# mmetcalf14/qml-cutensornet

Measured on AMD Instinct MI355X. Metric: Gram kernel entries/sec @ 60 qubits x 6 layers, higher is better.
Workload: dtype f64 (complex128)

## Files before the change

lab/qk_quad.h:

```cpp
#pragma once

__device__ __forceinline__ int qkq_qinv(const int d) {
  static constexpr int T[17] = {0, 1048576, 524288, 349526, 262144, 209716, 174763, 149797, 131072, 116509, 104858, 95326, 87382, 80660, 74899, 69906, 65536};
  return T[d];
}

struct QkqUnit {
  bool mine, a1, b1;
  int ta, tb, p;
};

template <bool A1, bool B1, typename XPtr>
__device__ __forceinline__ void qkq_p1(QkfTile (&T)[2][2], v2d (&fr)[4], v2d (&fs)[4], const bool primed, QkfStream cur, XPtr xp, unsigned x0, unsigned x1, const int nks,
                                       const QkfStream n0, const unsigned n1off) {
  v4d P[2][2][3];
  v2d fx[4], fy[4];
  if (!primed) qkf_load4(fr, cur);
  if (B1) {
#pragma unroll
    for (int i = 0; i < 4; ++i) fs[i] = qkf_ldg(cur.base + i * cur.step, cur.off + TILE);
  }
#pragma unroll
  for (int i = 0; i < 4; ++i) {
    fx[i] = qkf_ldx(xp + i * QKF_XSTEP, x0);
// ... 93 lines not shown
        p1 = __builtin_amdgcn_mfma_f64_16x16x4f64(S[1][0][i], fs[i].x, p1, 0, 0, 0);
        p2 = __builtin_amdgcn_mfma_f64_16x16x4f64(T[1][0].re[i], sp, p2, 0, 0, 0);
        p3 = __builtin_amdgcn_mfma_f64_16x16x4f64(T[1][0].im[i], sm, p3, 0, 0, 0);
        if (B1) {
          r1 = __builtin_amdgcn_mfma_f64_16x16x4f64(S[1][1][i], fs[i].x, r1, 0, 0, 0);
          r2 = __builtin_amdgcn_mfma_f64_16x16x4f64(T[1][1].re[i], sp, r2, 0, 0, 0);
          r3 = __builtin_amdgcn_mfma_f64_16x16x4f64(T[1][1].im[i], sm, r3, 0, 0, 0);
        }
      }
      if (!LAST) fs[i] = qkf_ldg(i == 0 ? b0 : i == 1 ? b1 : i == 2 ? b2 : b3, o1);
      __builtin_amdgcn_sched_barrier(0);
    }
  }
  QKF_PRIO_HI();
  {
    const v4d re = p1 - p3, im = p1 - p2;
#pragma unroll
    for (int r = 0; r < 4; ++r) {
      __hip_atomic_fetch_add(d + r * rs, re[r], __ATOMIC_RELAXED, __HIP_MEMORY_SCOPE_WORKGROUP);
      __hip_atomic_fetch_add(d + r * rs + 1, im[r], __ATOMIC_RELAXED, __HIP_MEMORY_SCOPE_WORKGROUP);
    }
  }
  if (B1) {
    const v4d re = r1 - r3, im = r1 - r2;
#pragma unroll
    for (int r = 0; r < 4; ++r) {
      __hip_atomic_fetch_add(d1 + r * rs, re[r], __ATOMIC_RELAXED, __HIP_MEMORY_SCOPE_WORKGROUP);
      __hip_atomic_fetch_add(d1 + r * rs + 1, im[r], __ATOMIC_RELAXED, __HIP_MEMORY_SCOPE_WORKGROUP);
    }
  }
}

template <bool FULL, bool A1, bool B1>
__device__ __forceinline__ void qkq_p2(const QkfTile (&T)[2][2], v2d (&fr)[4], v2d (&fs)[4], const QkfStream cur, const unsigned a1off, const int ps, const int nn, const int kmax, lds_v2d* xo,
                                       const int q, const int j, const QkfStream nxt) {
  lds_double* d = (lds_double*)(xo + q * TILE + j);
  lds_double* d1 = d + 2 * QKF_XBLOCK;
  constexpr long rs = 2 * QKF_XSTEP;
  v4d S[2][2];
#pragma unroll
  for (int u = 0; u < 2; ++u)
#pragma unroll
    for (int v = 0; v < 2; ++v) S[u][v] = ((u == 0 || A1) && (v == 0 || B1)) ? T[u][v].re + T[u][v].im : (v4d){0, 0, 0, 0};
  const v2d *const c0 = cur.base, *const c1 = cur.base + cur.step, *const c2 = cur.base + 2 * cur.step, *const c3 = cur.base + 3 * cur.step;
  unsigned o0 = cur.off, o1 = cur.off + a1off;
#pragma unroll 1
  for (int tn = 0; tn + 1 < nn; ++tn) {
    o0 += TILE, o1 += TILE;
    qkq_p2_block<FULL, A1, B1, false>(T, S, fr, fs, kmax, c0, c1, c2, c3, o0, o1, d, d1, rs);
    d += 2 * ps, d1 += 2 * ps;
  }
  qkq_p2_block<FULL, A1, B1, true>(T, S, fr, fs, kmax, nxt.base, nxt.base + nxt.step, nxt.base + 2 * nxt.step, nxt.base + 3 * nxt.step, nxt.off, 0u, d, d1, rs);
}

template <int NW, int XCAP, int WPS>
__global__ __launch_bounds__(64 * NW, WPS) void qk_sweep_fused_quad_kernel(const SweepArgs g) {
  constexpr int NT = 64 * NW;
  extern __shared__ __attribute__((aligned(16))) double lds_raw[];
  lds_v2d* const XL = (lds_v2d*)lds_raw;
  long long* const slot = reinterpret_cast<long long*>(lds_raw + 2 * XCAP);
  const v2d* const xdata = reinterpret_cast<const v2d*>(g.xdata);
  const v2d* const ydata = reinterpret_cast<const v2d*>(g.ydata);
  v2d* const G0 = reinterpret_cast<v2d*>(g.scratch) + (long long)blockIdx.x * 2 * g.x_plane;
  const int tid = threadIdx.x, lane = tid & 63;
  const int wave = __builtin_amdgcn_readfirstlane(tid >> 6);
  const int j = lane & 15, q = lane >> 4;
  const int ns = g.n_sites;
  __attribute__((address_space(3))) double* const zacc = (__attribute__((address_space(3))) double*)(slot + 2);
  lds_v4i* const rec = (lds_v4i*)(slot + 2 + 32);
  long long* const m_off = reinterpret_cast<long long*>(slot + 2 + 32) + 6 * (long long)ns;
  auto rfl = [&](const int v) __attribute__((always_inline)) { return __builtin_amdgcn_readfirstlane(v); };
  auto ldl = [&](const long long* p_) __attribute__((always_inline)) {
    const long long v = *p_;
    const unsigned lo = __builtin_amdgcn_readfirstlane((unsigned)v);
    const unsigned hi = __builtin_amdgcn_readfirstlane((unsigned)((unsigned long long)v >> 32));
    return (long long)(((unsigned long long)hi << 32) | lo);
  };
  auto site = [&](const int k) __attribute__((always_inline)) {
    const v4i r0 = rec[3 * k], r1 = rec[3 * k + 1], r2 = rec[3 * k + 2];
    QkfSite s;
    s.a = rfl(r0.x), s.a2 = rfl(r0.y), s.b = rfl(r0.z), s.b2 = rfl(r0.w);
    s.at = rfl(r1.x), s.nks = rfl(r1.y), s.W = rfl(r1.z), s.small = rfl(r1.w) != 0;
    s.inv = rfl(r2.x);
    s.ps = rfl(r2.y), s.pd = 1 << s.ps, s.next = rfl(r2.z);
    s.mt = s.a / TILE, s.nt = s.b2 / TILE, s.nn = s.a2 / TILE;
    s.Ak = xdata + ldl(m_off + 2 * k);
    s.Bk = ydata + ldl(m_off + 2 * k + 1);
    return s;
  };
  struct Pieces {
    int qa_f, qb_f, ra, rb, nA, kq, n2a, nB, nC, nD, L, qinv;
  };
  auto pieces_of = [&](const QkfSite& s, const int w) __attribute__((always_inline)) {
    Pieces pc;
    pc.qa_f = s.mt >> 1, pc.qb_f = w >> 1, pc.ra = s.mt & 1, pc.rb = w & 1;
    pc.nA = s.pd * pc.qa_f * pc.qb_f;
#if defined(QKF_QUAD_MODE) && QKF_QUAD_MODE == 0
    pc.kq = 0;
#else
    pc.kq = pc.nA - pc.nA % NW;
#endif
    pc.n2a = 2 * (pc.nA - pc.kq);
    pc.nB = s.pd * pc.ra * pc.qb_f, pc.nC = s.pd * pc.qa_f * pc.rb, pc.nD = s.pd * pc.ra * pc.rb;
    pc.L = pc.kq + pc.n2a + pc.nB + pc.nC + pc.nD;
    pc.qinv = qkq_qinv(pc.qa_f);
    return pc;
  };
  auto unit_of = [&](const QkfSite& s, const int w, const Pieces& pc, const int r0) __attribute__((always_inline)) {
    QkqUnit un;
    const int left = pc.L - r0;
    const bool cut = 2 * left <= NW;
    const int sub = cut && wave >= left ? 1 : 0;
    int i = r0 + wave - sub * left;
    un.mine = cut ? wave < 2 * left : i < pc.L;
    un.a1 = un.b1 = false, un.ta = un.tb = un.p = 0;
    auto quad = [&](const int vq) __attribute__((always_inline)) {
      const int u = vq >> s.ps, qb = (u * pc.qinv) >> 20, qa = u - qb * pc.qa_f;
      un.p = vq & (s.pd - 1), un.ta = 2 * qa, un.tb = 2 * qb;
    };
    if (i < pc.kq) {
      quad(i), un.a1 = un.b1 = true;
    } else if ((i -= pc.kq) < pc.n2a) {
      quad(pc.kq + (i >> 1)), un.ta += i & 1, un.b1 = true;
    } else if ((i -= pc.n2a) < pc.nB) {
      un.p = i & (s.pd - 1), un.ta = s.mt - 1, un.tb = 2 * (i >> s.ps), un.b1 = true;
    } else if ((i -= pc.nB) < pc.nC) {
      un.p = i & (s.pd - 1), un.ta = 2 * (i >> s.ps), un.tb = w - 1, un.a1 = true;
    } else {
      i -= pc.nC;
      un.p = i & (s.pd - 1), un.ta = s.mt - 1, un.tb = w - 1;
    }
    if (cut) {
      if (un.b1) un.tb += sub, un.b1 = false;
      else if (un.a1) un.ta += sub, un.a1 = false;
      else un.mine = un.mine && sub == 0;
    }
    return un;
  };
  auto b_stream = [&](const QkfSite& s, const int s0, const QkqUnit& un) __attribute__((always_inline)) {
    return QkfStream{s.Bk + un.p * s.b2, (unsigned)((q * s.pd) * s.b2 + (s0 + un.tb) * TILE + j), 4 * s.pd * s.b2};
  };
  auto a_stream = [&](const QkfSite& s, const QkqUnit& un) __attribute__((always_inline)) {
    return QkfStream{s.Ak + un.p * s.a2, (unsigned)(((un.ta * TILE + q) * s.pd) * s.a2 + j), 4 * s.pd * s.a2};
  };
  const int xcc = qk_xcc_id();
  if (tid == 0) qk_tail_start(g);
  for (;;) {
    if (tid == 0) *slot = qk_pull(g, xcc);
    __syncthreads();
    const long long p = *slot;
    __syncthreads();
    if (p < 0) break;
    const int xi = g.pairs[2 * p], yj = g.pairs[2 * p + 1];
    qkf_step_table<XCAP, NT>(g, xi, yj, rec, m_off, tid, [](const int pmt, const int nt) { return pmt * ((nt + 1) / 2) <= NW; });
    const int ek = g.edge_k, k_hi = ns - ek;
    const bool edges = ek > 0;
    if (!edges)
      for (int e = tid; e < TILE * TILE; e += NT) XL[e] = (v2d){e == 0 ? 1.0 : 0.0, 0.0};
    __syncthreads();
    bool xg = false;
    int cur = 0, xb = 0;
    if (edges) {
      const v4i r0 = rec[3 * ek];
      const int a_e = rfl(r0.x), b_e = rfl(r0.z);
      xg = a_e * b_e > XCAP;
      qkf_edge_prefix<NW, QKF_EDGE_PAIRS(WPS), QKF_EDGE_SETS(WPS)>(g, xi, yj, a_e, b_e, XL, G0, xg, wave, q, j);
      __syncthreads();
    }
    v2d fr[4], fs[4];
    bool primed = false;
    QkfSite sn = site(ek);
    for (int k = ek; k < k_hi;) {
      const QkfSite sc = sn;
      k = sc.next;
      if (k < k_hi) sn = site(k);
      const int a = sc.a, a2 = sc.a2, b = sc.b, nt = sc.nt, W = sc.W;
      const bool small = sc.small;
      v2d* const Gc = G0 + (long long)cur * g.x_plane;
      v2d* const Gn = G0 + (long long)(cur ^ 1) * g.x_plane;
      if (small && xg) {
        for (int e = tid; e < a * b; e += NT) XL[e] = Gc[e];
        __syncthreads();
        xg = false, xb = 0;
      } else if (!small && !xg) {
        for (int e = tid; e < a * b; e += NT) Gc[e] = XL[xb + e];
        __syncthreads();
        xg = true;
      }
      const int n_out = sc.b2 * a2;
      const bool pingpong = small && a * b + n_out <= XCAP;
      const int ob = !small ? 0 : pingpong ? (xb == 0 ? XCAP - n_out : 0) : 0;
      if (pingpong)
        for (int e = tid; e < n_out; e += NT) XL[ob + e] = (v2d){0.0, 0.0};
      for (int s0 = 0; s0 < nt; s0 += W) {
        const int w = min(W, nt - s0);
        const Pieces pc = pieces_of(sc, w);
        const int quads = pc.L;
        if (!small) {
          for (int e = tid; e < w * TILE * a2; e += NT) XL[e] = (v2d){0.0, 0.0};
          qk_lds_barrier();
        }
        for (int r0 = 0; r0 < quads; r0 += NW) {
          const QkqUnit un = unit_of(sc, w, pc, r0);
          const QkfStream as = a_stream(sc, un);
          const unsigned a1off = (unsigned)(TILE * sc.pd * a2);
          auto between = [&]() __attribute__((always_inline)) {
            if (small && r0 == 0) {
              qk_lds_barrier();
              if (!pingpong) {
                for (int e = tid; e < n_out; e += NT) XL[e] = (v2d){0.0, 0.0};
                qk_lds_barrier();
              }
            }
          };
          if (un.mine) {
            QkfTile T[2][2];
            const QkfStream bs = b_stream(sc, s0, un);
            const unsigned x0 = (unsigned)(un.ta * (b * TILE) + q * TILE + j), x1 = x0 + (unsigned)(b * TILE);
            auto go = [&](auto xbase) __attribute__((always_inline)) {
              if (un.a1) {
                if (un.b1) qkq_p1<true, true>(T, fr, fs, primed, bs, xbase, x0, x1, sc.nks, as, as.off + a1off);
                else qkq_p1<true, false>(T, fr, fs, primed, bs, xbase, x0, x1, sc.nks, as, as.off + a1off);
              } else {
                if (un.b1) qkq_p1<false, true>(T, fr, fs, primed, bs, xbase, x0, x1, sc.nks, as, as.off + a1off);
                else qkq_p1<false, false>(T, fr, fs, primed, bs, xbase, x0, x1, sc.nks, as, as.off + a1off);
              }
            };
            if (xg) go((const v2d*)Gc);
            else go((const lds_v2d*)(XL + xb));
            between();
            const int kmax = min(4, (sc.at - (un.ta + (un.a1 ? 1 : 0)) * TILE + 3) >> 2);
            QkfStream nxt = as;
            bool np1 = false;
            if (r0 + NW < quads) {
              const QkqUnit nu = unit_of(sc, w, pc, r0 + NW);
              if (nu.mine) nxt = b_stream(sc, s0, nu), np1 = true;
            } else if (s0 + W < nt) {
              const int w2 = min(W, nt - s0 - W);
              const QkqUnit nu = unit_of(sc, w2, pieces_of(sc, w2), 0);
              if (nu.mine) nxt = b_stream(sc, s0 + W, nu), np1 = true;
            } else if (k < k_hi) {
              const int w2 = min(sn.W, sn.nt);
              const QkqUnit nu = unit_of(sn, w2, pieces_of(sn, w2), 0);
              if (nu.mine) nxt = b_stream(sn, 0, nu), np1 = true;
            }
            lds_v2d* const xo = XL + ob + un.tb * QKF_XBLOCK;
            const int ps = w * QKF_XBLOCK;
            auto p2 = [&](auto a1_, auto b1_) __attribute__((always_inline)) {
              constexpr bool A1_ = decltype(a1_)::value, B1_ = decltype(b1_)::value;
              if (kmax == 4) qkq_p2<true, A1_, B1_>(T, fr, fs, as, a1off, ps, sc.nn, 4, xo, q, j, nxt);
              else qkq_p2<false, A1_, B1_>(T, fr, fs, as, a1off, ps, sc.nn, kmax, xo, q, j, nxt);
            };
            if (un.a1) {
              if (un.b1) p2(std::true_type{}, std::true_type{});
              else p2(std::true_type{}, std::false_type{});
            } else {
              if (un.b1) p2(std::false_type{}, std::true_type{});
              else p2(std::false_type{}, std::false_type{});
            }
            primed = np1;
          } else {
            between();
          }
        }
        qk_lds_barrier();
        if (!small && nt > W) {
          for (int tn = 0; tn < sc.nn; ++tn)
            for (int e = tid; e < w * QKF_XBLOCK; e += NT) Gn[(long long)tn * (sc.b2 * TILE) + s0 * QKF_XBLOCK + e] = XL[tn * w * QKF_XBLOCK + e];
          __syncthreads();
        }
      }
      if (!small) {
        if (nt > W) cur ^= 1;
        else xg = false, xb = 0;
      } else {
        xb = ob;
      }
    }
    if (edges) {
      const v4i r0 = rec[3 * (k_hi - 1)];
      const int a_e = rfl(r0.y), b_e = rfl(r0.w);
      qkf_edge_suffix<NW, QKF_EDGE_PAIRS(WPS), QKF_EDGE_SETS(WPS)>(g, xi, yj, a_e, b_e, (const lds_v2d*)(XL + xb), (const v2d*)(G0 + (long long)cur * g.x_plane), xg, zacc, wave, q, j);
      __syncthreads();
    }
    if (tid == 0) {
      v2d zz = {0.0, 0.0};
      if (edges)
        for (int w_ = 0; w_ < NW; ++w_) zz.x += zacc[2 * w_], zz.y += zacc[2 * w_ + 1];
      else zz = xg ? G0[(long long)cur * g.x_plane] : (v2d)XL[xb];
      g.values[p] = zz.x * zz.x + zz.y * zz.y;
      if (g.z) {
        g.z[2 * p] = zz.x;
        g.z[2 * p + 1] = zz.y;
      }
    }
    __syncthreads();
  }
  if (tid == 0) qk_tail_exit(g);
}
```

qml-cutensornet_amd/csrc/qk_device.h:

```cpp
#pragma once
#include <hip/hip_runtime.h>

#include <cstdint>
#include <type_traits>

static constexpr int TILE = 16;
typedef double v4d __attribute__((ext_vector_type(4)));
typedef float v4f __attribute__((ext_vector_type(4)));

struct SweepArgs {
  const double* xdata;
  const int32_t* xdims;
  const int32_t* xtrue;
  const int64_t* xoffs;
  const double* ydata;
  const int32_t* ydims;
  const int32_t* ytrue;
  const int64_t* yoffs;
  int n_sites;
  const int32_t* pairs;
  long long npairs;
  const int32_t* groups;
  long long ngroups;
  double* values;
  double* z;
  double* scratch;
  long long x_plane;
  long long t_plane;
  unsigned long long* counter;
  int nq;
  long long qstart[17];
  const double* xedge;
  const long long* xedge_offs;
  const double* yedge;
  const long long* yedge_offs;
  int edge_k;
  const double* xmg;
  const double* ymg;
  const int64_t* xmg_offs;
  const int64_t* ymg_offs;
  int merge_steps;
  int turn_ints;
  unsigned long long* tail;
  unsigned long long* err;
  unsigned long long* prof;
  unsigned long long* gang;
  int gang_n;
  int debug_flags;
  int prio_mode;
};

static constexpr int QK_QSTRIDE = 16;
static constexpr int QK_NQ_MAX = 16;

__device__ __forceinline__ int qk_xcc_id() { return __builtin_amdgcn_s_getreg((3 << 11) | 20) & 7; }

__device__ __forceinline__ long long qk_pull(const SweepArgs& g, const int xcc) {
  if (g.nq <= 1) {
    const long long p = (long long)atomicAdd(g.counter, 1ull);
    return p < g.npairs ? p : -1;
  }
  for (int s = 0; s < g.nq; ++s) {
    const int qd = ((xcc + s) & 7) + (s & 8);
    const long long n = g.qstart[qd + 1] - g.qstart[qd];
    if (n <= 0) continue;
    const long long t = (long long)atomicAdd(g.counter + QK_QSTRIDE * qd, 1ull);
    if (t < n) return g.qstart[qd] + t;
  }
  return -1;
}

__device__ __forceinline__ void qk_gang_sync(const SweepArgs& g, const int xcc, const bool have_pair, int& round) {
  if (g.gang_n <= 1) return;
  unsigned long long* const a = g.gang + QK_QSTRIDE * xcc;
  if (!have_pair) {
    __hip_atomic_store(a + 1, 1ull, __ATOMIC_RELAXED, __HIP_MEMORY_SCOPE_AGENT);
    return;
  }
  const unsigned long long target = (unsigned long long)g.gang_n * (unsigned long long)(++round);
  __hip_atomic_fetch_add(a, 1ull, __ATOMIC_RELAXED, __HIP_MEMORY_SCOPE_AGENT);
  for (int spins = 0;; ++spins) {
    if (__hip_atomic_load(a, __ATOMIC_RELAXED, __HIP_MEMORY_SCOPE_AGENT) >= target) return;
    if (__hip_atomic_load(a + 1, __ATOMIC_RELAXED, __HIP_MEMORY_SCOPE_AGENT) != 0) return;
    if (spins > 4000) {
      __hip_atomic_store(a + 1, 1ull, __ATOMIC_RELAXED, __HIP_MEMORY_SCOPE_AGENT);
      return;
    }
    __builtin_amdgcn_s_sleep(8);
  }
}

__device__ __forceinline__ void qk_tail_start(const SweepArgs& g) {
  if (g.tail) atomicMin(g.tail, (unsigned long long)__builtin_amdgcn_s_memrealtime());
}
__device__ __forceinline__ void qk_tail_exit(const SweepArgs& g) {
  if (g.tail) {
    const unsigned long long t = __builtin_amdgcn_s_memrealtime();
    atomicMin(g.tail + 1, t);
    atomicMax(g.tail + 4, t);
  }
}

__device__ __forceinline__ void qk_lds_barrier() { asm volatile("s_waitcnt lgkmcnt(0)\n\ts_barrier" ::: "memory"); }
```

qml-cutensornet_amd/csrc/qk_fused.h:

```cpp
#pragma once
#include "qk_device.h"
#include "qk_plan.h"

#define QKF_PRIO_LO() __builtin_amdgcn_s_setprio(0)
#define QKF_PRIO_HI() __builtin_amdgcn_s_setprio(2)
typedef double v2d __attribute__((ext_vector_type(2)));
typedef __attribute__((address_space(3))) v2d lds_v2d;
static constexpr int QKF_XSTEP = 4 * TILE;
static constexpr int QKF_XBLOCK = TILE * TILE;


#ifndef QKF_LDS3M
#define QKF_LDS3M 0
#endif
#ifndef QKF_P2_PROBE
#define QKF_P2_PROBE 0
#endif
#ifndef QKF_ABL
#define QKF_ABL 0
#endif
#define QKF_STEP_BARRIER()                            \
  do {                                                \
    if (QKF_ABL & 4) asm volatile("s_waitcnt lgkmcnt(0)" ::: "memory"); \
    else qk_lds_barrier();                            \
// ... 258 lines not shown
#else
#define QKF_EDGE_SETS(WPS) ((WPS) <= 3 ? 2 : 1)
#endif
__device__ __forceinline__ v2d qkf_lde(const v2d* __restrict__ base, const unsigned boff, const int col = 0) {
  return reinterpret_cast<const v2d*>(reinterpret_cast<const char*>(base) + (size_t)boff)[col];
}
template <bool HAS1, bool MORE>
__device__ __forceinline__ void qkf_edge_group(v4d (&acc)[6], v2d (&fy)[4], v2d (&fz)[4], v2d (&fx)[4], const v2d* const* const by, const v2d* const* const bx, const unsigned boy,
                                               const unsigned box) {
#pragma unroll
  for (int i = 0; i < 4; ++i) {
    const double sb = QKF_DIF(fx[i].x, fx[i].y);
    acc[0] = __builtin_amdgcn_mfma_f64_16x16x4f64(fy[i].x, fx[i].x, acc[0], 0, 0, 0);
    acc[1] = __builtin_amdgcn_mfma_f64_16x16x4f64(fy[i].y, fx[i].y, acc[1], 0, 0, 0);
    acc[2] = __builtin_amdgcn_mfma_f64_16x16x4f64(QKF_SUM(fy[i].x, fy[i].y), sb, acc[2], 0, 0, 0);
    if (HAS1) {
      acc[3] = __builtin_amdgcn_mfma_f64_16x16x4f64(fz[i].x, fx[i].x, acc[3], 0, 0, 0);
      acc[4] = __builtin_amdgcn_mfma_f64_16x16x4f64(fz[i].y, fx[i].y, acc[4], 0, 0, 0);
      acc[5] = __builtin_amdgcn_mfma_f64_16x16x4f64(QKF_SUM(fz[i].x, fz[i].y), sb, acc[5], 0, 0, 0);
    }
    if (MORE) {
      fy[i] = qkf_lde(by[i], boy);
      if (HAS1) fz[i] = qkf_lde(by[i], boy, TILE);
      fx[i] = qkf_lde(bx[i], box);
    }
    __builtin_amdgcn_sched_barrier(0);
  }
}
template <bool HAS1, int SETS>
__device__ __forceinline__ void qkf_edge_unit(QkfTile& t0, QkfTile& t1, const v2d* __restrict__ Ay, const unsigned oy, const int ldy, const v2d* __restrict__ Ax, const unsigned ox, const int ldx,
                                              const int ng) {
  static_assert(SETS == 1 || SETS == 2, "one or two groups of k-steps in flight");
  v4d acc[6];
#pragma unroll
  for (int e = 0; e < 6; ++e) acc[e] = (v4d){0, 0, 0, 0};
  v2d fy[SETS][4], fz[SETS][4], fx[SETS][4];
  const v2d *by[4 * SETS], *bx[4 * SETS];
#pragma unroll
  for (int i = 0; i < 4 * SETS; ++i) by[i] = Ay + 4 * i * ldy, bx[i] = Ax + 4 * i * ldx;
  unsigned boy = oy * 16u, box = ox * 16u;
  const unsigned sy = (unsigned)(SETS * TILE * ldy) * 16u, sx = (unsigned)(SETS * TILE * ldx) * 16u;
  const bool two = SETS == 2 && ng > 1;
#pragma unroll
  for (int s = 0; s < SETS; ++s) {
    if (s == 0 || two) {
#pragma unroll
      for (int i = 0; i < 4; ++i) {
        fy[s][i] = qkf_lde(by[4 * s + i], boy);
        if (HAS1) fz[s][i] = qkf_lde(by[4 * s + i], boy, TILE);
        fx[s][i] = qkf_lde(bx[4 * s + i], box);
      }
    }
  }
  QKF_PRIO_LO();
#pragma unroll 1
  for (int g = SETS; g < ng; g += SETS) {
    boy += sy, box += sx;
#pragma unroll
    for (int s = 0; s < SETS; ++s) qkf_edge_group<HAS1, true>(acc, fy[s], fz[s], fx[s], by + 4 * s, bx + 4 * s, boy, box);
  }
  qkf_edge_group<HAS1, false>(acc, fy[0], fz[0], fx[0], by, bx, boy, box);
  if constexpr (SETS == 2) {
    if (two) qkf_edge_group<HAS1, false>(acc, fy[1], fz[1], fx[1], by + 4, bx + 4, boy, box);
  }
  QKF_PRIO_HI();
  t0.re = acc[0] + acc[1], t0.im = acc[2] - acc[0] + acc[1];
  if (HAS1) t1.re = acc[3] + acc[4], t1.im = acc[5] - acc[3] + acc[4];
}
__device__ __forceinline__ long long qkf_uniform(const long long v) {
  const unsigned lo = __builtin_amdgcn_readfirstlane((unsigned)v);
  const unsigned hi = __builtin_amdgcn_readfirstlane((unsigned)((unsigned long long)v >> 32));
  return (long long)(((unsigned long long)hi << 32) | lo);
}

template <int NW, bool PAIRS>
__device__ __forceinline__ QkEdgeUnit qkf_edge_unit_of(const int u, const int mt, const int nt, const int inv) {
  if constexpr (PAIRS) return qk_edge_unit(u, mt, nt, NW, inv);
  const int tb = (u * inv) >> 20;
  return QkEdgeUnit{u - tb * mt, tb, false, true};
}
template <int NW, bool PAIRS, int SETS>
__device__ __forceinline__ void qkf_edge_prefix(const SweepArgs& g, const int xi, const int yj, const int a, const int b, lds_v2d* const xl, v2d* const xg, const bool to_global, const int wave,
                                                const int q, const int j) {
  const v2d* const Lx = reinterpret_cast<const v2d*>(g.xedge) + qkf_uniform(g.xedge_offs[2 * (long long)xi]);
  const v2d* const Ly = reinterpret_cast<const v2d*>(g.yedge) + qkf_uniform(g.yedge_offs[2 * (long long)yj]);
  const int mt = a / TILE, nt = b / TILE, ng = (1 << g.edge_k) >> 4, inv = qk_recip20(mt), units = PAIRS ? qk_edge_units(mt, nt, NW) : mt * nt;
  for (int u = wave; u < units; u += NW) {
    const QkEdgeUnit un = qkf_edge_unit_of<NW, PAIRS>(u, mt, nt, inv);
    if (!un.mine) continue;
    QkfTile T0, T1;
    const unsigned oy = (unsigned)(q * b + un.tb0 * TILE + j), ox = (unsigned)(q * a + un.ta * TILE + j);
    if (un.has1) qkf_edge_unit<true, 1>(T0, T1, Ly, oy, b, Lx, ox, a, ng);
    else qkf_edge_unit<false, SETS>(T0, T1, Ly, oy, b, Lx, ox, a, ng);
    const int at = un.ta * (b * TILE) + (un.tb0 * TILE + q) * TILE + j;
    if (to_global) {
#pragma unroll
      for (int r = 0; r < 4; ++r) xg[at + r * QKF_XSTEP] = (v2d){T0.re[r], T0.im[r]};
      if (un.has1) {
#pragma unroll
        for (int r = 0; r < 4; ++r) xg[at + QKF_XBLOCK + r * QKF_XSTEP] = (v2d){T1.re[r], T1.im[r]};
      }
    } else {
#pragma unroll
      for (int r = 0; r < 4; ++r) xl[at + r * QKF_XSTEP] = (v2d){T0.re[r], T0.im[r]};
      if (un.has1) {
#pragma unroll
        for (int r = 0; r < 4; ++r) xl[at + QKF_XBLOCK + r * QKF_XSTEP] = (v2d){T1.re[r], T1.im[r]};
      }
    }
  }
}

template <int NW, bool PAIRS, int SETS>
__device__ __forceinline__ void qkf_edge_suffix(const SweepArgs& g, const int xi, const int yj, const int a, const int b, const lds_v2d* const xl, const v2d* const xg, const bool from_global,
                                                __attribute__((address_space(3))) double* zacc, const int wave, const int q, const int j) {
  const v2d* const Rx = reinterpret_cast<const v2d*>(g.xedge) + qkf_uniform(g.xedge_offs[2 * (long long)xi + 1]);
  const v2d* const Ry = reinterpret_cast<const v2d*>(g.yedge) + qkf_uniform(g.yedge_offs[2 * (long long)yj + 1]);
  const int mt = a / TILE, nt = b / TILE, ng = (1 << g.edge_k) >> 4, inv = qk_recip20(mt), units = PAIRS ? qk_edge_units(mt, nt, NW) : mt * nt;
  double zr = 0, zi = 0;
  for (int u = wave; u < units; u += NW) {
    const QkEdgeUnit un = qkf_edge_unit_of<NW, PAIRS>(u, mt, nt, inv);
    if (!un.mine) continue;
    QkfTile T0, T1;
    const unsigned oy = (unsigned)(q * b + un.tb0 * TILE + j), ox = (unsigned)(q * a + un.ta * TILE + j);
    if (un.has1) qkf_edge_unit<true, 1>(T0, T1, Ry, oy, b, Rx, ox, a, ng);
    else qkf_edge_unit<false, SETS>(T0, T1, Ry, oy, b, Rx, ox, a, ng);
    const int at = un.ta * (b * TILE) + (un.tb0 * TILE + q) * TILE + j;
#pragma unroll
    for (int r = 0; r < 4; ++r) {
      const v2d x = from_global ? xg[at + r * QKF_XSTEP] : (v2d)xl[at + r * QKF_XSTEP];
      zr += x.x * T0.re[r] - x.y * T0.im[r], zi += x.x * T0.im[r] + x.y * T0.re[r];
    }
    if (un.has1) {
#pragma unroll
      for (int r = 0; r < 4; ++r) {
        const v2d x = from_global ? xg[at + QKF_XBLOCK + r * QKF_XSTEP] : (v2d)xl[at + QKF_XBLOCK + r * QKF_XSTEP];
        zr += x.x * T1.re[r] - x.y * T1.im[r], zi += x.x * T1.im[r] + x.y * T1.re[r];
      }
    }
  }
#pragma unroll
  for (int o = 32; o > 0; o >>= 1) zr += __shfl_xor(zr, o), zi += __shfl_xor(zi, o);
  if ((q | j) == 0) zacc[2 * wave] = zr, zacc[2 * wave + 1] = zi;
}

struct QkfSite {
  int a, a2, b, b2, at, nks, mt, nt, nn, W, inv, inv2, pd, ps, next;
  bool small;
  const v2d *Ak, *Bk;
};
typedef int v4i __attribute__((ext_vector_type(4)));
typedef __attribute__((address_space(3))) v4i lds_v4i;

template <int XCAP, int NT, bool ITEM_RECIPS = false, typename OneRound>
__device__ __forceinline__ void qkf_step_table(const SweepArgs& g, const int xi, const int yj, lds_v4i* const rec, long long* const m_off, const int tid, const OneRound one_round) {
  const int ns = g.n_sites, n1 = ns + 1;
  const int32_t* const xd = g.xdims + (long long)xi * n1;
  const int32_t* const yd = g.ydims + (long long)yj * n1;
  const int32_t* const xt = g.xtrue + (long long)xi * n1;
  const int32_t* const yt = g.ytrue + (long long)yj * n1;
  const v2d* const xdata = reinterpret_cast<const v2d*>(g.xdata);
  const v2d* const ydata = reinterpret_cast<const v2d*>(g.ydata);
  auto is_small = [&](const int a, const int a2, const int b, const int b2, const int pd) __attribute__((always_inline)) {
    return a * b <= XCAP && a2 * b2 <= XCAP && (one_round(pd * (a / TILE), b2 / TILE) || a * b + a2 * b2 <= XCAP);
  };
  auto put = [&](const int e, const int a, const int a2, const int b, const int b2, const int ps, const int next, const bool small, const v2d* const A, const v2d* const B)
                 __attribute__((always_inline)) {
    const int mt = a / TILE, nt = b2 / TILE;
    const int W = small ? nt : max(1, min(nt, XCAP / (TILE * a2)));
    rec[3 * e] = (v4i){a, a2, b, b2};
    rec[3 * e + 1] = (v4i){xt[e], (yt[e] + 3) >> 2, W, small ? 1 : 0};
    rec[3 * e + 2] = (v4i){qk_recip20(mt), ps, next, ITEM_RECIPS ? qk_unit_recips(nt, W, false) : 0};
    m_off[2 * e] = (long long)(((const char*)A - (const char*)xdata) / 16);
    m_off[2 * e + 1] = (long long)(((const char*)B - (const char*)ydata) / 16);
  };
  auto plain = [&](const int e, const int next) __attribute__((always_inline)) {
    const int a = xd[e], a2 = xd[e + 1], b = yd[e], b2 = yd[e + 1];
    put(e, a, a2, b, b2, 1, next, is_small(a, a2, b, b2, 2), xdata + (g.xoffs[(long long)xi * ns + e] >> 1), ydata + (g.yoffs[(long long)yj * ns + e] >> 1));
  };
  if (g.merge_steps == 0) {
    for (int e = tid; e < ns; e += NT) plain(e, e + 1);
    return;
  }
  const int ek = g.edge_k, k_hi = ns - ek;
  for (int t = tid; 2 * t < k_hi - ek; t += NT) {
    const int e = ek + 2 * t;
    if (e + 1 >= k_hi) {
      plain(e, e + 1);
      continue;
    }
    const int a = xd[e], am = xd[e + 1], a2 = xd[e + 2], b = yd[e], bm = yd[e + 1], b2 = yd[e + 2];
    const bool sm = is_small(a, a2, b, b2, 4);
    const long long work_m = 4ll * a * b2 * (b + a2), work_p = 2ll * a * bm * (b + am) + 2ll * am * b2 * (bm + a2);
    const bool merged = (sm || (!is_small(a, am, b, bm, 2) && !is_small(am, a2, bm, b2, 2))) && work_m <= work_p;
    plain(e + 1, e + 2);
    if (merged)
      put(e, a, a2, b, b2, 2, e + 2, sm, reinterpret_cast<const v2d*>(g.xmg) + (g.xmg_offs[(long long)xi * g.merge_steps + t] >> 1),
          reinterpret_cast<const v2d*>(g.ymg) + (g.ymg_offs[(long long)yj * g.merge_steps + t] >> 1));
    else plain(e, e + 1);
  }
}

#ifdef QKF_PROF
#define QKF_PROF_DECL() \
  unsigned long long pf[8] = {0, 0, 0, 0, 0, 0, 0, 0}, pt = __builtin_amdgcn_s_memtime(); \
  const unsigned long long pt0 = pt
#define QKF_STAMP(i)                                              \
  do {                                                            \
    const unsigned long long now_ = __builtin_amdgcn_s_memtime(); \
    pf[i] += now_ - pt;                                           \
    pt = now_;                                                    \
  } while (0)
#define QKF_PROF_FLUSH()                                             \
  do {                                                               \
    if (lane == 0) {                                                 \
      pf[7] = __builtin_amdgcn_s_memtime() - pt0;                    \
      for (int i_ = 0; i_ < 8; ++i_) atomicAdd(g.prof + i_, pf[i_]); \
    }                                                                \
  } while (0)
#else
#define QKF_PROF_DECL()
#define QKF_STAMP(i)
#define QKF_PROF_FLUSH()
#endif

#define QKF_PULLER(NT) ((NT) - 64)
__device__ __forceinline__ void qkf_pull_next(const SweepArgs& g, const int xcc, int& gang_round, long long* const word) {
  const long long pp = qk_pull(g, xcc);
  qk_gang_sync(g, xcc, pp >= 0, gang_round);
  *word = pp;
}

template <int NW, int S, int XCAP, int WPS, bool DET = false>
__global__ __launch_bounds__(64 * NW, WPS) void qk_sweep_fused_kernel(const SweepArgs g) {
  constexpr int NT = 64 * NW;
  extern __shared__ __attribute__((aligned(16))) double lds_raw[];
  lds_v2d* const XL = (lds_v2d*)lds_raw;
  long long* const slot = reinterpret_cast<long long*>(lds_raw + 2 * XCAP);
  const v2d* const xdata = reinterpret_cast<const v2d*>(g.xdata);
  const v2d* const ydata = reinterpret_cast<const v2d*>(g.ydata);
  v2d* const G0 = reinterpret_cast<v2d*>(g.scratch) + (long long)blockIdx.x * 2 * g.x_plane;
  const int tid = threadIdx.x, lane = tid & 63;
  const int wave = __builtin_amdgcn_readfirstlane(tid >> 6);
  const int j = lane & 15, q = lane >> 4;
  const int ns = g.n_sites;
  __attribute__((address_space(3))) double* const zacc = (__attribute__((address_space(3))) double*)(slot + 2);
  lds_v4i* const rec = (lds_v4i*)(slot + 2 + 32);
  long long* const m_off = reinterpret_cast<long long*>(slot + 2 + 32) + 6 * (long long)ns;
  lds_int* const tbroken = (lds_int*)(m_off + 2 * (long long)ns);
  lds_int* const turn0 = tbroken + 2;
  auto rfl = [&](const int v) __attribute__((always_inline)) { return __builtin_amdgcn_readfirstlane(v); };
  auto ldl = [&](const long long* p_) __attribute__((always_inline)) {
    const long long v = *p_;
    const unsigned lo = __builtin_amdgcn_readfirstlane((unsigned)v);
    const unsigned hi = __builtin_amdgcn_readfirstlane((unsigned)((unsigned long long)v >> 32));
    return (long long)(((unsigned long long)hi << 32) | lo);
  };
  auto site = [&](const int k) __attribute__((always_inline)) {
    const v4i r0 = rec[3 * k], r1 = rec[3 * k + 1], r2 = rec[3 * k + 2];
    QkfSite s;
    s.a = rfl(r0.x), s.a2 = rfl(r0.y), s.b = rfl(r0.z), s.b2 = rfl(r0.w);
    s.at = rfl(r1.x), s.nks = rfl(r1.y), s.W = rfl(r1.z), s.small = rfl(r1.w) != 0;
    s.inv = rfl(r2.x), s.inv2 = rfl(r2.w);
    s.ps = rfl(r2.y), s.pd = 1 << s.ps, s.next = rfl(r2.z);
    s.mt = s.a / TILE, s.nt = s.b2 / TILE, s.nn = s.a2 / TILE;
    s.Ak = xdata + ldl(m_off + 2 * k);
    s.Bk = ydata + ldl(m_off + 2 * k + 1);
    return s;
  };
  auto item_of = [&](const QkfSite& s, const int w, const int it) __attribute__((always_inline)) {
    return DET ? qk_unit_decode_ordered(it, s.ps, s.mt, s.inv) : qk_unit_decode(it, s.mt, w, s.inv, qk_unit_recip_of(s.inv2, w == s.W));
  };
  auto b_stream = [&](const QkfSite& s, const int s0, const int w, const int it) __attribute__((always_inline)) {
    const QkUnit un = item_of(s, w, it);
    return QkfStream{s.Bk + un.p * s.b2, (unsigned)((q * s.pd) * s.b2 + (s0 + un.tc) * TILE + j), 4 * s.pd * s.b2, min(4, s.nks)};
  };
  auto a_stream = [&](const QkfSite& s, const int w, const int it) __attribute__((always_inline)) {
    const QkUnit un = item_of(s, w, it);
    return QkfStream{s.Ak + un.p * s.a2, (unsigned)(((un.ta * TILE + q) * s.pd) * s.a2 + j), 4 * s.pd * s.a2, min(4, (s.at - un.ta * TILE + 3) >> 2)};
  };
  QKF_PROF_DECL();
  const int xcc = qk_xcc_id();
  int gang_round = 0;
  if (tid == 0) qk_tail_start(g);
  for (;;) {
    if (tid == 0) {
      const long long pp_ = qk_pull(g, xcc);
      qk_gang_sync(g, xcc, pp_ >= 0, gang_round);
      *slot = pp_;
    }
    __syncthreads();
    const long long p = *slot;
    __syncthreads();
    if (p < 0) break;
    const int xi = g.pairs[2 * p], yj = g.pairs[2 * p + 1];
    qkf_step_table<XCAP, NT, true>(g, xi, yj, rec, m_off, tid, [](const int pmt, const int nt) { return pmt * nt <= NW * S; });
    const int ek = g.edge_k, k_hi = ns - ek;
    const bool edges = ek > 0;
    if (!edges)
      for (int e = tid; e < TILE * TILE; e += NT) XL[e] = (v2d){e == 0 ? 1.0 : 0.0, 0.0};
    if constexpr (DET)
      for (int e = tid; e < 2 * g.turn_ints + 2; e += NT) tbroken[e] = 0;
    int tsel = 0;
    __syncthreads();
    bool xg = false;
    int cur = 0, xb = 0;
    if (edges) {
      const v4i r0 = rec[3 * ek];
      const int a_e = rfl(r0.x), b_e = rfl(r0.z);
      xg = a_e * b_e > XCAP;
      qkf_edge_prefix<NW, QKF_EDGE_PAIRS(WPS), QKF_EDGE_SETS(WPS)>(g, xi, yj, a_e, b_e, XL, G0, xg, wave, q, j);
      __syncthreads();
    }
    QKF_STAMP(0);
    QkfTile T[S];
    v2d fr[4];
    bool primed = false;
    QkfSite sn = site(ek);
    for (int k = ek; k < k_hi;) {
      const QkfSite sc = sn;
      k = sc.next;
      if (k < k_hi) sn = site(k);
      const int a = sc.a, a2 = sc.a2, b = sc.b, mt = sc.mt, nt = sc.nt, W = sc.W;
      const bool small = sc.small;
      v2d* const Gc = G0 + (long long)cur * g.x_plane;
      v2d* const Gn = G0 + (long long)(cur ^ 1) * g.x_plane;
      if (small && xg) {
        for (int e = tid; e < a * b; e += NT) XL[e] = Gc[e];
        __syncthreads();
        xg = false, xb = 0;
      } else if (!small && !xg) {
        for (int e = tid; e < a * b; e += NT) Gc[e] = XL[xb + e];
        __syncthreads();
        xg = true;
      }
      const int n_out = sc.b2 * a2;
      const bool pingpong = small && a * b + n_out <= XCAP;
      const int ob = !small ? 0 : pingpong ? (xb == 0 ? XCAP - n_out : 0) : 0;
      if (pingpong && !DET)
        for (int e = tid; e < n_out; e += NT) XL[ob + e] = (v2d){0.0, 0.0};
      QKF_STAMP(1);
      for (int s0 = 0; s0 < nt; s0 += W) {
        const int w = min(W, nt - s0), items = sc.pd * mt * w;
        lds_int* const tcur = turn0 + tsel * g.turn_ints;
        if constexpr (DET) {
          for (int e = tid; e < g.turn_ints; e += NT) turn0[(tsel ^ 1) * g.turn_ints + e] = 0;
        } else if (!small) {
          for (int e = tid; e < w * TILE * a2; e += NT) XL[e] = (v2d){0.0, 0.0};
          QKF_STEP_BARRIER();
        }
        QKF_STAMP(6);
        for (int r0 = 0; r0 < items; r0 += NW * S) {
          const int L = min(S, (items - r0 + NW - 1) / NW);
          const bool multi = L > 1;
          const int it0 = r0 + wave;
          auto phase1 = [&](auto xbase) __attribute__((always_inline)) {
#pragma unroll 1
            for (int s = 0; s < L; ++s) {
              if (multi) qkf_rotate<S>(T, L);
              const int it = it0 + NW * s;
              if (it < items) {
                const int ta = item_of(sc, w, it).ta;
                const bool more = s + 1 < L && it + NW < items;
                const QkfStream nxt = more ? b_stream(sc, s0, w, it + NW) : a_stream(sc, w, it0);
                qkf_p1_tile(T[S - 1], fr, primed, b_stream(sc, s0, w, it), xbase, (unsigned)(ta * (b * TILE) + q * TILE + j), sc.nks, nxt);
                primed = true;
              }
            }
          };
          if (xg) phase1((const v2d*)Gc);
          else phase1((const lds_v2d*)(XL + xb));
          QKF_STAMP(2);
          if (small && r0 == 0 && !(DET && pingpong)) {
            QKF_STEP_BARRIER();
            if (!pingpong && !DET) {
              for (int e = tid; e < n_out; e += NT) XL[e] = (v2d){0.0, 0.0};
              QKF_STEP_BARRIER();
            }
          }
          QKF_STAMP(3);
          const bool last_round = s0 + W >= nt && r0 + NW * S >= items;
#pragma unroll 1
          for (int s = 0; s < S; ++s) {
            const int it = it0 + NW * s;
            if (it >= items) break;
            if (multi) qkf_rotate<S>(T, L);
            const QkUnit un = item_of(sc, w, it);
            const int ta = un.ta, tbl = un.tc;
            const int kmax = min(4, (sc.at - ta * TILE + 3) >> 2);
            const bool more = s + 1 < S && it + NW < items;
            const int wn = min(sn.W, sn.nt);
            const bool chain = !more && last_round && k < k_hi && wave < sn.pd * sn.mt * wn;
            const QkfStream nxt = more ? a_stream(sc, w, it + NW) : chain ? b_stream(sn, 0, wn, wave) : a_stream(sc, w, it);
            const int tix = sc.pd * ta + un.p;
            const QkfTurn turn{tcur + tbl * sc.nn, tix, tbroken, g.err};
            if (kmax == 4) qkf_p2_item<true, DET>(T[S - 1], fr, primed, a_stream(sc, w, it), w * QKF_XBLOCK, sc.nn, 4, XL + ob + tbl * QKF_XBLOCK, q, j, nxt, turn);
            else qkf_p2_item<false, DET>(T[S - 1], fr, primed, a_stream(sc, w, it), w * QKF_XBLOCK, sc.nn, kmax, XL + ob + tbl * QKF_XBLOCK, q, j, nxt, turn);
            primed = more || chain;
          }
          QKF_STAMP(4);
        }
        QKF_STEP_BARRIER();
        tsel ^= 1;
        QKF_STAMP(5);
        if (!small && nt > W) {
          for (int tn = 0; tn < sc.nn; ++tn)
            for (int e = tid; e < w * QKF_XBLOCK; e += NT) Gn[(long long)tn * (sc.b2 * TILE) + s0 * QKF_XBLOCK + e] = XL[tn * w * QKF_XBLOCK + e];
          __syncthreads();
          QKF_STAMP(1);
        }
      }
      if (!small) {
        if (nt > W) cur ^= 1;
        else xg = false, xb = 0;
      } else {
        xb = ob;
      }
    }
    if (edges) {
      const v4i r0 = rec[3 * (k_hi - 1)];
      const int a_e = rfl(r0.y), b_e = rfl(r0.w);
      qkf_edge_suffix<NW, QKF_EDGE_PAIRS(WPS), QKF_EDGE_SETS(WPS)>(g, xi, yj, a_e, b_e, (const lds_v2d*)(XL + xb), (const v2d*)(G0 + (long long)cur * g.x_plane), xg, zacc, wave, q, j);
      __syncthreads();
    }
    if (tid == 0) {
      v2d zz = {0.0, 0.0};
      if (edges)
        for (int w_ = 0; w_ < NW; ++w_) zz.x += zacc[2 * w_], zz.y += zacc[2 * w_ + 1];
      else zz = xg ? G0[(long long)cur * g.x_plane] : (v2d)XL[xb];
      g.values[p] = zz.x * zz.x + zz.y * zz.y;
      if (g.z) {
        g.z[2 * p] = zz.x;
        g.z[2 * p + 1] = zz.y;
      }
    }
    __syncthreads();
  }
  if (tid == 0) qk_tail_exit(g);
  QKF_PROF_FLUSH();
}

template <bool HAS1, typename XPtr>
__device__ __forceinline__ void qkf_p1_dual(QkfTile& t0, QkfTile& t1, v2d (&fr)[4], v2d (&fs)[4], const bool primed, QkfStream cur, XPtr xp, unsigned xoff, const int nks,
                                            const QkfStream nxt) {
  v4d p1 = {0, 0, 0, 0}, p2 = {0, 0, 0, 0}, p3 = {0, 0, 0, 0}, r1 = {0, 0, 0, 0}, r2 = {0, 0, 0, 0}, r3 = {0, 0, 0, 0};
  v2d fx[4];
  if (!primed) qkf_load4(fr, cur);
  if (HAS1) {
#pragma unroll
// ... 95 lines not shown
  }
  if (HAS1) {
#pragma unroll
    for (int r = 0; r < 4; ++r) {
      __hip_atomic_fetch_add(d1 + r * rs, re1[r], __ATOMIC_RELAXED, __HIP_MEMORY_SCOPE_WORKGROUP);
      __hip_atomic_fetch_add(d1 + r * rs + 1, im1[r], __ATOMIC_RELAXED, __HIP_MEMORY_SCOPE_WORKGROUP);
    }
  }
}
template <bool FULL, bool HAS1, bool DET>
__device__ __forceinline__ void qkf_p2_dual_turn(const QkfTile& t0, const QkfTile& t1, v2d (&fr)[4], v2d (&fs)[4], QkfStream cur, const int ps, const int nn, const int kmax, lds_v2d* xo, const int q,
                                            const int j, const QkfStream nxt, const bool nxt_p1, const unsigned n1, const QkfTurn turn = QkfTurn{nullptr, 0, nullptr, nullptr}) {
  __attribute__((address_space(3))) double* d = (__attribute__((address_space(3))) double*)(xo + q * TILE + j);
#pragma unroll 1
  for (int tn = 0; tn < nn; ++tn) {
    v4d p1 = {0, 0, 0, 0}, p2 = {0, 0, 0, 0}, p3 = {0, 0, 0, 0}, r1 = {0, 0, 0, 0}, r2 = {0, 0, 0, 0}, r3 = {0, 0, 0, 0};
    const bool fin = tn + 1 == nn;
    const v2d* const rb = fin ? nxt.base : cur.base;
    const int rs = fin ? nxt.step : cur.step;
    cur.off = fin ? nxt.off : cur.off + TILE;
    QKF_PRIO_LO();
#pragma unroll
    for (int i = 0; i < 4; ++i) {
      if (FULL || i < kmax) {
        qkf_kstep<true>(p1, p2, p3, t0.re[i], t0.im[i], fr[i].x, fr[i].y);
        if (HAS1) qkf_kstep<true>(r1, r2, r3, t1.re[i], t1.im[i], fr[i].x, fr[i].y);
      }
      fr[i] = qkf_ldg_a(rb + i * rs, cur.off);
      __builtin_amdgcn_sched_barrier(0);
    }
    QKF_PRIO_HI();
    {
      const v4d re = p1 + p2, im = p3 - p1 + p2;
      if constexpr (DET) qkf_turn_add(d, (long)2 * QKF_XSTEP, re, im, turn, tn);
      else {
#pragma unroll
        for (int r = 0; r < 4; ++r) {
          __hip_atomic_fetch_add(d + r * 2 * QKF_XSTEP, re[r], __ATOMIC_RELAXED, __HIP_MEMORY_SCOPE_WORKGROUP);
          __hip_atomic_fetch_add(d + r * 2 * QKF_XSTEP + 1, im[r], __ATOMIC_RELAXED, __HIP_MEMORY_SCOPE_WORKGROUP);
        }
      }
    }
    if (HAS1) {
      const v4d re = r1 + r2, im = r3 - r1 + r2;
      __attribute__((address_space(3))) double* const d1 = d + 2 * QKF_XBLOCK;
      if constexpr (DET) qkf_turn_add(d1, (long)2 * QKF_XSTEP, re, im, QkfTurn{turn.at + nn, turn.idx, turn.broken, turn.gerr}, tn);
      else {
#pragma unroll
        for (int r = 0; r < 4; ++r) {
          __hip_atomic_fetch_add(d1 + r * 2 * QKF_XSTEP, re[r], __ATOMIC_RELAXED, __HIP_MEMORY_SCOPE_WORKGROUP);
          __hip_atomic_fetch_add(d1 + r * 2 * QKF_XSTEP + 1, im[r], __ATOMIC_RELAXED, __HIP_MEMORY_SCOPE_WORKGROUP);
        }
      }
    }
    d += 2 * ps;
  }
}

template <bool FULL, bool HAS1, bool DET = false>
__device__ __forceinline__ void qkf_p2_dual(const QkfTile& t0, const QkfTile& t1, v2d (&fr)[4], v2d (&fs)[4], QkfStream cur, const int ps, const int nn, const int kmax, lds_v2d* xo, const int q,
                                            const int j, const QkfStream nxt, const bool nxt_p1, const unsigned n1, const QkfTurn turn = QkfTurn{nullptr, 0, nullptr, nullptr}) {
  if constexpr (DET) {
    qkf_p2_dual_turn<FULL, HAS1, DET>(t0, t1, fr, fs, cur, ps, nn, kmax, xo, q, j, nxt, nxt_p1, n1, turn);
    return;
  }
  lds_double* d = (lds_double*)(xo + q * TILE + j);
  lds_double* d1 = d + 2 * QKF_XBLOCK;
  constexpr long rs = 2 * QKF_XSTEP;
  const v4d s0 = t0.re + t0.im, s1 = HAS1 ? t1.re + t1.im : s0;
  const v2d *const c0 = cur.base, *const c1 = cur.base + cur.step, *const c2 = cur.base + 2 * cur.step, *const c3 = cur.base + 3 * cur.step;
  unsigned off = cur.off;
#pragma unroll 1
  for (int tn = 0; tn + 1 < nn; ++tn) {
    off += TILE;
    qkf_p2_block<FULL, HAS1>(t0, t1, s0, s1, fr, kmax, c0, c1, c2, c3, off, d, d1, rs);
    d += 2 * ps, d1 += 2 * ps;
  }
  qkf_p2_block<FULL, HAS1>(t0, t1, s0, s1, fr, kmax, nxt.base, nxt.base + nxt.step, nxt.base + 2 * nxt.step, nxt.base + 3 * nxt.step, nxt.off, d, d1, rs);
}

template <int NW, int XCAP, int WPS, bool DET = false>
__global__ __launch_bounds__(64 * NW, WPS) void qk_sweep_fused_dual_kernel(const SweepArgs g) {
  constexpr int NT = 64 * NW;
  extern __shared__ __attribute__((aligned(16))) double lds_raw[];
  lds_v2d* const XL = (lds_v2d*)lds_raw;
  long long* const slot = reinterpret_cast<long long*>(lds_raw + 2 * XCAP);
  const v2d* const xdata = reinterpret_cast<const v2d*>(g.xdata);
  const v2d* const ydata = reinterpret_cast<const v2d*>(g.ydata);
  v2d* const G0 = reinterpret_cast<v2d*>(g.scratch) + (long long)blockIdx.x * 2 * g.x_plane;
  const int tid = threadIdx.x, lane = tid & 63;
  const int wave = __builtin_amdgcn_readfirstlane(tid >> 6);
  const int j = lane & 15, q = lane >> 4;
  const int ns = g.n_sites;
  __attribute__((address_space(3))) double* const zacc = (__attribute__((address_space(3))) double*)(slot + 2);
  lds_v4i* const rec = (lds_v4i*)(slot + 2 + 32);
  long long* const m_off = reinterpret_cast<long long*>(slot + 2 + 32) + 6 * (long long)ns;
  lds_int* const tbroken = (lds_int*)(m_off + 2 * (long long)ns);
  lds_int* const turn0 = tbroken + 2;
  auto rfl = [&](const int v) __attribute__((always_inline)) { return __builtin_amdgcn_readfirstlane(v); };
  auto ldl = [&](const long long* p_) __attribute__((always_inline)) {
    const long long v = *p_;
    const unsigned lo = __builtin_amdgcn_readfirstlane((unsigned)v);
    const unsigned hi = __builtin_amdgcn_readfirstlane((unsigned)((unsigned long long)v >> 32));
    return (long long)(((unsigned long long)hi << 32) | lo);
  };
  auto site = [&](const int k) __attribute__((always_inline)) {
    const v4i r0 = rec[3 * k], r1 = rec[3 * k + 1], r2 = rec[3 * k + 2];
    QkfSite s;
    s.a = rfl(r0.x), s.a2 = rfl(r0.y), s.b = rfl(r0.z), s.b2 = rfl(r0.w);
    s.at = rfl(r1.x), s.nks = rfl(r1.y), s.W = rfl(r1.z), s.small = rfl(r1.w) != 0;
    s.inv = rfl(r2.x);
    s.ps = rfl(r2.y), s.pd = 1 << s.ps, s.next = rfl(r2.z);
    s.mt = s.a / TILE, s.nt = s.b2 / TILE, s.nn = s.a2 / TILE;
    s.Ak = xdata + ldl(m_off + 2 * k);
    s.Bk = ydata + ldl(m_off + 2 * k + 1);
    return s;
  };
  auto pair_of = [&](const QkfSite& s, const int v) __attribute__((always_inline)) { return qk_unit_decode_ordered(v, s.ps, s.mt, s.inv); };
  auto b_stream = [&](const QkfSite& s, const int s0, const int v, const int half) __attribute__((always_inline)) {
    const QkUnit un = pair_of(s, v);
    return QkfStream{s.Bk + un.p * s.b2, (unsigned)((q * s.pd) * s.b2 + (s0 + 2 * un.tc + half) * TILE + j), 4 * s.pd * s.b2};
  };
  struct Unit {
    bool mine, has1;
    int v, half;
  };
  auto unit_of = [&](const QkfSite& s, const int w, const int units, const int r0) __attribute__((always_inline)) {
    Unit un;
    const int left = units - r0;
    const bool halves = 2 * left <= NW;
    un.half = (halves && wave >= left) ? 1 : 0;
    un.v = r0 + wave - (un.half ? left : 0);
    const int tp = pair_of(s, un.v).tc;
    const bool second = 2 * tp + 1 < w;
    un.mine = un.v < units && (un.half == 0 || second);
    un.has1 = !halves && second;
    return un;
  };
  auto a_stream = [&](const QkfSite& s, const int v) __attribute__((always_inline)) {
    const QkUnit un = pair_of(s, v);
    return QkfStream{s.Ak + un.p * s.a2, (unsigned)(((un.ta * TILE + q) * s.pd) * s.a2 + j), 4 * s.pd * s.a2};
  };
  QKF_PROF_DECL();
  const int xcc = qk_xcc_id();
  int gang_round = 0;
  if (tid == 0) qk_tail_start(g);
  if (tid == QKF_PULLER(NT)) qkf_pull_next(g, xcc, gang_round, slot);
  __syncthreads();
  long long p = slot[0];
  int psel = 0;
  auto table_of = [&](const long long pp) __attribute__((always_inline)) {
    if (pp < 0) return;
    const int xi_ = g.pairs[2 * pp], yj_ = g.pairs[2 * pp + 1];
    qkf_step_table<XCAP, NT>(g, xi_, yj_, rec, m_off, tid, [](const int pmt, const int nt) { return pmt * ((nt + 1) / 2) <= NW; });
  };
  table_of(p);
  while (p >= 0) {
    const int xi = g.pairs[2 * p], yj = g.pairs[2 * p + 1];
    const int ek = g.edge_k, k_hi = ns - ek;
    const bool edges = ek > 0;
    if (!edges)
      for (int e = tid; e < TILE * TILE; e += NT) XL[e] = (v2d){e == 0 ? 1.0 : 0.0, 0.0};
    if constexpr (DET)
      for (int e = tid; e < 2 * g.turn_ints + 2; e += NT) tbroken[e] = 0;
    int tsel = 0;
    __syncthreads();
    bool xg = false;
    int cur = 0, xb = 0;
    if (edges) {
      const v4i r0 = rec[3 * ek];
      const int a_e = rfl(r0.x), b_e = rfl(r0.z);
      xg = a_e * b_e > XCAP;
      qkf_edge_prefix<NW, QKF_EDGE_PAIRS(WPS), QKF_EDGE_SETS(WPS)>(g, xi, yj, a_e, b_e, XL, G0, xg, wave, q, j);
      __syncthreads();
    }
    QKF_STAMP(0);
    QkfTile T0, T1;
    v2d fr[4], fs[4];
    bool primed = false;
    QkfSite sn = site(ek);
    for (int k = ek; k < k_hi;) {
      const QkfSite sc = sn;
      k = sc.next;
      if (k < k_hi) sn = site(k);
      const int a = sc.a, a2 = sc.a2, b = sc.b, mt = sc.mt, nt = sc.nt, W = sc.W;
      const bool small = sc.small;
      v2d* const Gc = G0 + (long long)cur * g.x_plane;
      v2d* const Gn = G0 + (long long)(cur ^ 1) * g.x_plane;
      if (small && xg) {
        for (int e = tid; e < a * b; e += NT) XL[e] = Gc[e];
        __syncthreads();
        xg = false, xb = 0;
      } else if (!small && !xg) {
        for (int e = tid; e < a * b; e += NT) Gc[e] = XL[xb + e];
        __syncthreads();
        xg = true;
      }
      const int n_out = sc.b2 * a2;
      const bool pingpong = small && a * b + n_out <= XCAP;
      const int ob = !small ? 0 : pingpong ? (xb == 0 ? XCAP - n_out : 0) : 0;
      if (pingpong && !DET)
        for (int e = tid; e < n_out; e += NT) XL[ob + e] = (v2d){0.0, 0.0};
      QKF_STAMP(1);
      for (int s0 = 0; s0 < nt; s0 += W) {
        const int w = min(W, nt - s0), units = sc.pd * mt * ((w + 1) >> 1);
        lds_int* const tcur = turn0 + tsel * g.turn_ints;
        if constexpr (DET) {
          for (int e = tid; e < g.turn_ints; e += NT) turn0[(tsel ^ 1) * g.turn_ints + e] = 0;
        } else if (!small) {
          for (int e = tid; e < w * TILE * a2; e += NT) XL[e] = (v2d){0.0, 0.0};
          QKF_STEP_BARRIER();
        }
        for (int r0 = 0; r0 < units; r0 += NW) {
          const Unit un = unit_of(sc, w, units, r0);
          const int v = un.v;
          const bool mine = un.mine, has1 = un.has1;
          const QkUnit pr = pair_of(sc, v);
          const int tp = pr.tc, ta = pr.ta;
          if (mine) {
            const QkfStream bs = b_stream(sc, s0, v, un.half), as = a_stream(sc, v);
            const unsigned xoff = (unsigned)(ta * (b * TILE) + q * TILE + j);
            if (xg) {
              if (has1) qkf_p1_dual<true>(T0, T1, fr, fs, primed, bs, (const v2d*)Gc, xoff, sc.nks, as);
              else qkf_p1_dual<false>(T0, T1, fr, fs, primed, bs, (const v2d*)Gc, xoff, sc.nks, as);
            } else {
              if (has1) qkf_p1_dual<true>(T0, T1, fr, fs, primed, bs, (const lds_v2d*)(XL + xb), xoff, sc.nks, as);
              else qkf_p1_dual<false>(T0, T1, fr, fs, primed, bs, (const lds_v2d*)(XL + xb), xoff, sc.nks, as);
            }
          }
          QKF_STAMP(2);
          if (small && r0 == 0 && !(DET && pingpong)) {
            QKF_STEP_BARRIER();
            if (!pingpong && !DET) {
              for (int e = tid; e < n_out; e += NT) XL[e] = (v2d){0.0, 0.0};
              QKF_STEP_BARRIER();
            }
          }
          QKF_STAMP(3);
          if (mine) {
            const int kmax = min(4, (sc.at - ta * TILE + 3) >> 2);
            QkfStream nxt = a_stream(sc, v);
            bool np1 = false;
            if (r0 + NW < units) {
              const Unit nu = unit_of(sc, w, units, r0 + NW);
              if (nu.mine) nxt = b_stream(sc, s0, nu.v, nu.half), np1 = true;
            } else if (s0 + W < nt) {
              const int w2 = min(W, nt - s0 - W);
              const Unit nu = unit_of(sc, w2, sc.pd * mt * ((w2 + 1) >> 1), 0);
              if (nu.mine) nxt = b_stream(sc, s0 + W, nu.v, nu.half), np1 = true;
            } else if (k < k_hi) {
              const int w2 = min(sn.W, sn.nt);
              const Unit nu = unit_of(sn, w2, sn.pd * sn.mt * ((w2 + 1) >> 1), 0);
              if (nu.mine) nxt = b_stream(sn, 0, nu.v, nu.half), np1 = true;
            }
            const unsigned nd1 = 0;
            lds_v2d* const xo = XL + ob + (2 * tp + un.half) * QKF_XBLOCK;
            const QkfTurn tp_turn{tcur + (2 * tp + un.half) * sc.nn, sc.pd * ta + pr.p, tbroken, g.err};
            if (has1) {
              if (kmax == 4) qkf_p2_dual<true, true, DET>(T0, T1, fr, fs, a_stream(sc, v), w * QKF_XBLOCK, sc.nn, 4, xo, q, j, nxt, np1, nd1, tp_turn);
              else qkf_p2_dual<false, true, DET>(T0, T1, fr, fs, a_stream(sc, v), w * QKF_XBLOCK, sc.nn, kmax, xo, q, j, nxt, np1, nd1, tp_turn);
            } else {
              if (kmax == 4) qkf_p2_dual<true, false, DET>(T0, T1, fr, fs, a_stream(sc, v), w * QKF_XBLOCK, sc.nn, 4, xo, q, j, nxt, np1, nd1, tp_turn);
              else qkf_p2_dual<false, false, DET>(T0, T1, fr, fs, a_stream(sc, v), w * QKF_XBLOCK, sc.nn, kmax, xo, q, j, nxt, np1, nd1, tp_turn);
            }
            primed = np1;
          }
          QKF_STAMP(4);
        }
        QKF_STEP_BARRIER();
        tsel ^= 1;
        QKF_STAMP(5);
        if (!small && nt > W) {
          for (int tn = 0; tn < sc.nn; ++tn)
            for (int e = tid; e < w * QKF_XBLOCK; e += NT) Gn[(long long)tn * (sc.b2 * TILE) + s0 * QKF_XBLOCK + e] = XL[tn * w * QKF_XBLOCK + e];
          __syncthreads();
        }
      }
      if (!small) {
        if (nt > W) cur ^= 1;
        else xg = false, xb = 0;
      } else {
        xb = ob;
      }
    }
    if (tid == QKF_PULLER(NT)) qkf_pull_next(g, xcc, gang_round, slot + (psel ^ 1));
    if (edges) {
      const v4i r0 = rec[3 * (k_hi - 1)];
      const int a_e = rfl(r0.y), b_e = rfl(r0.w);
      qkf_edge_suffix<NW, QKF_EDGE_PAIRS(WPS), QKF_EDGE_SETS(WPS)>(g, xi, yj, a_e, b_e, (const lds_v2d*)(XL + xb), (const v2d*)(G0 + (long long)cur * g.x_plane), xg, zacc, wave, q, j);
    }
    __syncthreads();
    const long long pn = slot[psel ^ 1];
    if (tid == 0) {
      v2d zz = {0.0, 0.0};
      if (edges)
        for (int w_ = 0; w_ < NW; ++w_) zz.x += zacc[2 * w_], zz.y += zacc[2 * w_ + 1];
      else zz = xg ? G0[(long long)cur * g.x_plane] : (v2d)XL[xb];
      g.values[p] = zz.x * zz.x + zz.y * zz.y;
      if (g.z) {
        g.z[2 * p] = zz.x;
        g.z[2 * p + 1] = zz.y;
      }
    }
    table_of(pn);
    if (!edges) __syncthreads();
    p = pn, psel ^= 1;
    QKF_STAMP(6);
// ... 227 lines not shown
```

qml-cutensornet_amd/csrc/qk_host.h:

```cpp
#pragma once
#include "../../include/qkgram.h"
#include "qk_plan.h"

#include <hip/hip_runtime.h>

#include "qk_devmem.h"

#include <cstdint>
#include <vector>

struct QkRangeGuard {
  explicit QkRangeGuard(const char* n) { qk_range_push(n); }
  ~QkRangeGuard() { qk_range_pop(); }
};

#define HIP_TRY(expr)                                                                                 \
  do {                                                                                                \
    hipError_t e_ = (expr);                                                                           \
    if (e_ != hipSuccess) return qk_fail(QK_EDEVICE, "%s failed: %s", #expr, hipGetErrorString(e_));  \
  } while (0)
#define HIP_TRY_AS(what, expr)                              \
  do {                                                                                                          \
    hipError_t e_ = (expr);                                                                                     \
    if (e_ != hipSuccess) return qk_fail(QK_EDEVICE, "%s: %s failed: %s", what, #expr, hipGetErrorString(e_));  \
  } while (0)

struct qk_ctx {
  int device = 0;
  int num_cus = 0;
  hipStream_t own_stream = nullptr;
  hipStream_t stream = nullptr;
  bool split_pending = false;
  hipEvent_t ev0 = nullptr, ev1 = nullptr, ev_mid = nullptr;
  hipEvent_t ev_d = nullptr;
  bool ev_pending = false;
  QkGrowBuf scratch;
  QkDevBuf counter;
  bool tail_pending = false;
  QkDevBuf prof;
  QkSweepPolicy policy;
  qk_stats last{};
  QkGrowBuf build_arena, build_work;
  QkGrowBuf derive_tmp;
  QkGrowBuf local_scratch;
};

uint64_t qk_next_uid();

struct qk_mps_set {
  qk_ctx* ctx = nullptr;
  uint64_t uid = qk_next_uid();
  int n_states = 0, n_sites = 0, max_pad = 0;
  int precision = 64;
  QkDevBuf d_data;
  QkDevBuf d_il;
  QkDevBuf d_dims;
  QkDevBuf d_true;
  QkDevBuf d_offs;
  std::vector<int32_t> dims_true;
  int64_t bytes = 0;
  QkDevBuf d_edge;
  QkDevBuf d_edge_offs;
  int edge_k = 0;
  int64_t edge_bytes = 0;
  QkDevBuf d_mg;
  QkDevBuf d_mg_offs;
  QkDevBuf d_mg_units;
  std::vector<long long> h_edge_offs, h_mg_units;
  std::vector<int64_t> h_mg_offs;
  int mg_k = -1, mg_steps = 0;
  int64_t mg_bytes = 0;
};

int qk_mps_set_alloc(qk_ctx* c, int n_states, int n_sites, int64_t data_bytes, int precision, qk_mps_set** out, const char* who);

struct QkSpectraArgs {
  const double* env;
  const int32_t* dims;
  const int32_t* tru;
  const int32_t* states;
  const int32_t* pmax;
  const int64_t* sbase;
  const int64_t* roff;
  const int64_t* loff;
  const int2* tasks;
  int n_tasks;
  char* work;
  long long work_bytes;
  int qmax;
  double* out;
  int n_sites, max_values, rmul;
  int* error;
};
size_t qk_bond_spectra_work_bytes(int qmax);
int qk_bond_spectra_launch(qk_ctx* c, QkSpectraArgs a, int grid, const char* what);

struct QkCompressArgs {
  const double* planes;
  const int32_t* pad;
  const int32_t* tru;
  const int64_t* offs;
  int s0, n_batch, n_sites;
  double* stage;
  const long long* stage_offs;
  int32_t* dims_new;
  double* fidelity;
  double* discarded;
  int cap;
  double budget, zero;
  char* work;
  long long work_bytes;
  int qmax;
  int* error;
};
size_t qk_compress_work_bytes(int qmax);
int qk_compress_launch(qk_ctx* c, QkCompressArgs a, int grid, const char* what);

struct SweepArgs;
int qk_lab_init(qk_ctx* c);
int qk_lab_launch(qk_ctx* c, int variant, const SweepArgs& a, int grid, int n_sites);
int qk_lab_launch_quad(qk_ctx* c, const SweepArgs& a, int grid, int n_sites, bool f32);
```

qml-cutensornet_amd/csrc/qk_plan.h:

```cpp
#pragma once
#include "../../include/qkgram.h"

#include <algorithm>
#include <cstdint>
#include <cstdio>
#include <vector>

int qk_fail(int code, const char* fmt, ...) __attribute__((format(printf, 2, 3)));

#ifndef QKF_XCAP_ONE_V
#define QKF_XCAP_ONE_V 8192
#endif
#ifndef QKF_XCAP_TWO_V
#define QKF_XCAP_TWO_V 4608
#endif
#ifndef QKF_TWO_WGS
#define QKF_TWO_WGS 2
#endif
static constexpr int QKF_XCAP_ONE = QKF_XCAP_ONE_V, QKF_XCAP_TWO = QKF_XCAP_TWO_V;
static constexpr int QK_TILE = 16;
static inline int qk_pad16(int x) { return (x + QK_TILE - 1) / QK_TILE * QK_TILE; }
static constexpr int GMAX = 4;

#if defined(__HIPCC__)
#define QK_HD __host__ __device__
#else
#define QK_HD
#endif
struct QkUnit {
  int ta, tc, p;
};
QK_HD static inline int qk_unit_cols(const int w, const bool dual) { return dual ? (w + 1) >> 1 : w; }
QK_HD static inline int qk_recip20(const int d) { return ((1 << 20) + d - 1) / d; }
QK_HD static inline int qk_recip15(const int d) { return ((1 << 15) + d - 1) / d; }
QK_HD static inline int qk_unit_recips(const int nt, const int W, const bool dual) {
  const int wl = nt - (nt - 1) / W * W;
  return qk_recip15(qk_unit_cols(W, dual)) | (qk_recip15(qk_unit_cols(wl, dual)) << 16);
}
QK_HD static inline int qk_unit_recip_of(const int recips, const bool full_strip) { return full_strip ? (recips & 0xffff) : (int)((unsigned)recips >> 16); }
QK_HD static inline QkUnit qk_unit_decode(const int v, const int mt, const int wc, const int inv_mt, const int inv_wc) {
  const int c = (v * inv_mt) >> 20, p = (c * inv_wc) >> 15;
  return QkUnit{v - c * mt, c - p * wc, p};
}
QK_HD static inline QkUnit qk_unit_decode_ordered(const int v, const int ps, const int mt, const int inv_mt) {
  const int u = v >> ps, tc = (u * inv_mt) >> 20;
  return QkUnit{u - tc * mt, tc, v & ((1 << ps) - 1)};
}

struct QkEdgeUnit {
  int ta, tb0;
  bool has1, mine;
};
QK_HD static inline int qk_edge_units(const int mt, const int nt, const int NW) {
  const int pairs = mt * ((nt + 1) >> 1), r0 = (pairs - 1) / NW * NW, left = pairs - r0;
  return 2 * left <= NW ? r0 + 2 * left : pairs;
}
QK_HD static inline QkEdgeUnit qk_edge_unit(const int u, const int mt, const int nt, const int NW, const int inv_mt) {
  const int pairs = mt * ((nt + 1) >> 1), r0 = (pairs - 1) / NW * NW, left = pairs - r0;
  const bool halves = 2 * left <= NW, single = halves && u >= r0, half = halves && u >= r0 + left;
  const int v = u - (half ? left : 0), tp = (v * inv_mt) >> 20;
  const bool second = 2 * tp + 1 < nt;
  return QkEdgeUnit{v - tp * mt, 2 * tp + (half ? 1 : 0), !single && second, u < (halves ? r0 + 2 * left : pairs) && (!half || second)};
}

struct qk_ctx;

struct qk_plan {
  int n_sites = 0, nx = 0, ny = 0;
  bool symmetric = false;
  bool quad = false;
  int world = 1, rank = 0;
  int64_t total_pairs = 0, max_per_rank = 0;
  std::vector<int32_t> pairs;
  std::vector<int32_t> groups;
  int group = 1;
  qk_stats stats{};
  qk_stats second{};
  int64_t n_first = 0;
  int nq = 1;
  int64_t qstart[17] = {0};
  int edge_k = 0;
  bool second_wave2 = false;
  double fit_two = 1.0;
  double fit_narrow = 1.0;
  double tile_reuse_bytes = 0;
  double plan_ms = 0;
  int plan_threads = 1;
  qk_ctx* up_ctx = nullptr;
  int32_t* d_pairs = nullptr;
  int32_t* d_groups = nullptr;
};

struct QkSweepPolicy {
  int variant = 20;
  int wgs_per_cu = 2;
  bool wave_path = true;
  bool wave2_ring = true;
  bool wave2_path = true;
  bool small_path = true;
  int fused_path = 1;
  int fused_split = 1;
  int fused_wgs = 0;
  bool deterministic = false;
  bool merge_sites = true;
  bool fused_dual = true;
  bool gang = false;
};

struct QkSetShape {
  int max_pad = 0, precision = 64, n_sites = 0;
};

struct QkSweepRun {
  int kernel = QK_KERNEL_NONE;
  long long grid = 0;
  size_t lds = 0;
  long long first = 0, count = 0;
  int nq = 1, gang_n = 0;
  bool gang2 = false;
};

struct QkSweepChoice {
  int rc = QK_OK;
  char err[192] = {};
  int n_runs = 0;
  QkSweepRun run[2];
  long long launched_grid = 0;
  long long x_plane = 0, t_plane = 0;
  int turn_ints = 0;
  size_t scratch_bytes = 0;
  bool interleaved = false;
  bool fused_images = false;
  int queues = 1;
  bool tails = false;
};

static inline QkSweepChoice qk_choose_sweep(const QkSweepPolicy& p, const qk_plan& plan, const QkSetShape& x, const QkSetShape& y, const int num_cus) {
  QkSweepChoice ch;
  const long long np = (long long)plan.pairs.size() / 2;
  const bool f32 = x.precision == 32, quad = plan.quad, det = p.deterministic;
  const int n = x.n_sites, max_pad = std::max(x.max_pad, y.max_pad);
  const bool grouped = p.variant == 14 && !f32 && !quad, duo = p.variant == 16 && !f32 && !quad;
  const long long chains = quad ? 4 : (duo ? 2 : 1);
  const long long units = quad ? np / 4 : grouped ? (long long)plan.groups.size() / 2 : (duo ? (np + 1) / 2 : np);
  ch.x_plane = (grouped ? GMAX : 1) * (long long)x.max_pad * y.max_pad, ch.t_plane = 2 * ch.x_plane;
  ch.turn_ints = det ? (y.max_pad / QK_TILE) * (x.max_pad / QK_TILE) : 0;
  const size_t lds_meta = 16 + 256 + (size_t)n * (48 + 16) + (det ? (size_t)(2 * ch.turn_ints + 2) * sizeof(int) : 0);
  const bool can_one = max_pad <= QKF_XCAP_ONE / QK_TILE && (size_t)QKF_XCAP_ONE * 16 + lds_meta <= 160 * 1024;
  const bool can_two = max_pad <= QKF_XCAP_TWO / QK_TILE && (size_t)QKF_XCAP_TWO * 16 + lds_meta <= 160 * 1024 / QKF_TWO_WGS;
  const bool fused = p.variant == 20 && !f32 && !quad && p.fused_path != 0 && max_pad > (p.fused_path >= 2 ? 16 : 32) && (can_one || can_two);
  const bool second_class = fused && plan.n_first > 0 && plan.n_first < np;
  const bool split = second_class && can_one && can_two && p.fused_wgs == 0 && p.fused_split != 0 && !plan.second_wave2 && (p.fused_split == 2 || np >= 100ll * num_cus);
  const bool mixed = second_class && plan.second_wave2 && p.wave2_path && p.wave2_ring;
  const bool fused_two = fused && can_two && !split && (!can_one || p.fused_wgs == 2 || (p.fused_wgs == 0 && plan.fit_two >= 0.75 && plan.fit_narrow >= 0.5));
  const bool dual = fused && !fused_two && p.fused_dual;
  const int wgs = fused ? (fused_two ? QKF_TWO_WGS : 1) : p.wgs_per_cu;
  const long long grid = std::min(units, (long long)wgs * num_cus);
  ch.scratch_bytes = (size_t)(split ? 2ll * num_cus : grid) * (size_t)chains * 2 * (size_t)(ch.x_plane + ch.t_plane) * sizeof(double);
  const size_t site_meta = 16 + (size_t)(4 * (n + 1) + 2) * sizeof(int) + (size_t)2 * n * sizeof(long long);
  const size_t lds_ring = 3 * 16 * 1024 + site_meta;
  const size_t esz = f32 ? sizeof(float) : sizeof(double), lds_small = (size_t)(3 * 2 * (64 / esz) * 64 + 6 * 32 * 32) * esz + site_meta;
  if (lds_ring > 80 * 1024)
    return ch.rc = QK_EINVAL, snprintf(ch.err, sizeof ch.err, "qk_gram_values: %d sites need %zu bytes of LDS per workgroup (limit 80 KiB for 2 workgroups per CU)", n, lds_ring), ch;
  QkSweepRun& r = ch.run[0];
  ch.n_runs = 1, ch.launched_grid = r.grid = grid, r.count = np;
  if (quad) {
#ifdef QK_LAB
    r.kernel = QK_KERNEL_LAB;
#else
    ch.rc = QK_EINVAL, snprintf(ch.err, sizeof ch.err, "qk_gram_values: QK_PLAN_QUADS plans are swept by an experimental kernel that only libqklab.so contains");
#endif
  } else if (p.variant == 20 && p.wave_path && !f32 && max_pad <= 16) {
    r.kernel = QK_KERNEL_WAVE, ch.launched_grid = r.grid = std::min(np, 16ll * num_cus);
  } else if (!fused && p.variant == 20 && p.wave2_path && (!f32 || p.wave2_ring) && max_pad <= 32) {
    r.kernel = (f32 || p.wave2_ring) ? QK_KERNEL_WAVE2 : QK_KERNEL_WAVE2_PLAIN, ch.launched_grid = r.grid = std::min(np, 8ll * num_cus);
    ch.interleaved = ch.tails = true, ch.queues = plan.nq > 1 ? 8 : 1, r.nq = plan.nq;
  } else if (!fused && p.variant == 20 && p.small_path && max_pad <= 32 && lds_small <= 80 * 1024) {
    r.kernel = QK_KERNEL_SMALL, r.lds = lds_small;
  } else if (fused) {
    ch.interleaved = ch.fused_images = ch.tails = true, ch.queues = plan.nq > 1 ? 8 : 1, r.nq = plan.nq;
    r.kernel = fused_two ? (det ? QK_KERNEL_FUSED2_DET : QK_KERNEL_FUSED2) : dual ? (det ? QK_KERNEL_FUSED_DUAL_DET : QK_KERNEL_FUSED_DUAL) : (det ? QK_KERNEL_FUSED1_DET : QK_KERNEL_FUSED1);
    r.lds = (size_t)(fused_two ? QKF_XCAP_TWO : QKF_XCAP_ONE) * 16 + lds_meta;
    auto gang_of = [&](const long long g) { return p.gang && plan.nq > 1 && g >= 16 && g % 8 == 0 ? (int)(g / 8) : 0; };
    if (split || mixed) {
      QkSweepRun& r2 = ch.run[1];
      ch.n_runs = 2;
      r.count = plan.n_first, r2.first = plan.n_first, r2.count = np - plan.n_first;
      r.nq = r2.nq = plan.nq > 1 ? 8 : plan.nq;
      r.grid = std::min(r.count, (long long)wgs * num_cus);
      if (split) {
        r2.kernel = det ? QK_KERNEL_FUSED2_DET : QK_KERNEL_FUSED2, r2.grid = std::min(r2.count, (long long)QKF_TWO_WGS * num_cus);
        r2.lds = (size_t)QKF_XCAP_TWO * 16 + lds_meta, r2.gang_n = gang_of(r2.grid), r2.gang2 = true;
      } else {
        r2.kernel = QK_KERNEL_WAVE2, r2.grid = std::min(r2.count, 8ll * num_cus);
      }
    }
    r.gang_n = gang_of(r.grid);
  } else if (f32 || p.variant == 20) {
    r.kernel = QK_KERNEL_RING, r.lds = lds_ring;
  } else {
#ifdef QK_LAB
    r.kernel = QK_KERNEL_LAB;
#else
    ch.rc = QK_EINVAL, snprintf(ch.err, sizeof ch.err, "qk_gram_values: no kernel for this call");
#endif
  }
  return ch;
}
```

qml-cutensornet_amd/csrc/qk_planner.cpp:

```cpp
#include "qk_plan.h"

#include <sched.h>

#include <algorithm>
#include <chrono>
#include <cmath>
#include <cstdio>
#include <cstdlib>
#include <cstring>
#include <new>
#include <numeric>
#include <thread>
#include <vector>

static inline int pad16(int x) { return qk_pad16(x); }

static int plan_threads() {
  if (const char* e = std::getenv("QK_PLAN_THREADS")) return std::max(1, std::min(64, std::atoi(e)));
  cpu_set_t set;
  int n = 1;
  if (sched_getaffinity(0, sizeof set, &set) == 0) n = CPU_COUNT(&set);
  return std::max(1, std::min(16, n));
}

template <typename F>
static void par_ranges(const int threads, const int64_t n, const F& f) {
  const int t = (int)std::max<int64_t>(1, std::min<int64_t>(threads, n));
  if (t == 1) {
    f((int64_t)0, n);
    return;
  }
  std::vector<std::thread> pool;
  pool.reserve((size_t)t - 1);
  for (int w = 1; w < t; ++w) pool.emplace_back([&, w] { f(n * w / t, n * (w + 1) / t); });
  f((int64_t)0, n / t);
  for (std::thread& th : pool) th.join();
}

struct SiteTab {
  int n = 0;
  std::vector<double> t0, t1, t01, P0, P1, P01, T0, T1, TK;
  std::vector<double> bytes, weight;
  std::vector<int> max_pad;
  void build(const int n_states, const int n_sites, const int32_t* dims) {
    n = n_sites;
    const size_t tot = (size_t)n_states * n_sites;
    for (std::vector<double>* v : {&t0, &t1, &t01, &P0, &P1, &P01, &T0, &T1, &TK}) v->assign(tot, 0.0);
    bytes.assign((size_t)n_states, 0.0), weight.assign((size_t)n_states, 0.0), max_pad.assign((size_t)n_states, 0);
    for (int s = 0; s < n_states; ++s) {
      const int32_t* d = dims + (int64_t)s * (n_sites + 1);
      double by = 0, w = 0;
      int mp = 0;
      for (int k = 0; k < n_sites; ++k) {
        const size_t e = (size_t)s * n_sites + k;
        const int a0 = d[k], a1 = d[k + 1], A0 = pad16(a0), A1 = pad16(a1);
        t0[e] = a0, t1[e] = a1, t01[e] = (double)a0 * a1;
        P0[e] = A0, P1[e] = A1, P01[e] = (double)A0 * A1;
        T0[e] = A0 / 16, T1[e] = A1 / 16, TK[e] = (double)(A1 / 16) * ((a0 + 3) / 4);
        by += 16.0 * 2 * ((double)a0 * a1);
        w += (double)A0 * A1 * ((double)A0 + A1);
        mp = std::max(mp, std::max(A0, A1));
      }
      bytes[(size_t)s] = by, weight[(size_t)s] = w, max_pad[(size_t)s] = mp;
    }
  }
};

struct Pass1 {
  double c_xy, c_yx, fp_xy, fp_yx;
};
#if defined(__x86_64__)
#define QK_SIMD_CLONES __attribute__((target_clones("avx2,fma", "default")))
#else
#define QK_SIMD_CLONES
#endif
QK_SIMD_CLONES static Pass1 pair_pass1(const int n, const double* __restrict__ xT0, const double* __restrict__ xT1, const double* __restrict__ xTK, const double* __restrict__ xP0,
                                       const double* __restrict__ xP1, const double* __restrict__ xP01, const double* __restrict__ yT0, const double* __restrict__ yT1,
                                       const double* __restrict__ yTK, const double* __restrict__ yP0, const double* __restrict__ yP1, const double* __restrict__ yP01) {
  double cxy = 0, cyx = 0, fxy = 0, fyx = 0;
#pragma omp simd reduction(+ : cxy, cyx, fxy, fyx)
  for (int k = 0; k < n; ++k) {
    cxy += xT0[k] * yTK[k] + yT1[k] * xTK[k];
    cyx += yT0[k] * xTK[k] + xT1[k] * yTK[k];
    fxy += xP0[k] * yP01[k] + xP01[k] * yP1[k];
    fyx += yP0[k] * xP01[k] + yP01[k] * xP1[k];
  }
  return Pass1{6 * cxy, 6 * cyx, 16 * fxy, 16 * fyx};
}

struct Pass2 {
  double f, ft, fn;
};
QK_SIMD_CLONES static Pass2 pair_pass2(const int n, const double* __restrict__ a0, const double* __restrict__ a1, const double* __restrict__ a01, const double* __restrict__ A0,
                                       const double* __restrict__ A1, const double* __restrict__ A01, const double* __restrict__ b0, const double* __restrict__ b1,
                                       const double* __restrict__ b01, const double* __restrict__ B0, const double* __restrict__ B1, const double* __restrict__ B01, const double cap_two,
                                       const double cap_fit) {
  double f = 0, ft = 0, fn = 0;
#pragma omp simd reduction(+ : f, ft, fn)
  for (int k = 0; k < n; ++k) {
    const double f1 = a0[k] * b01[k] + a01[k] * b1[k];
    const double f2 = b0[k] * a01[k] + b01[k] * a1[k];
    f += f1 < f2 ? f1 : f2;
    const double w = A0[k] * B01[k] + A01[k] * B1[k];
    const double x0 = A0[k] * B0[k], x1 = A1[k] * B1[k];
    ft += (x0 <= cap_two && x1 <= cap_two) ? w : 0.0;
    fn += (x0 <= cap_fit && x1 <= cap_fit) ? w : 0.0;
  }
  return Pass2{16 * f, 16 * ft, 16 * fn};
}

static void pair_work(int n, const int32_t* a, const int32_t* b, const double plan_fit, double* flops, double* padded, double* bytes, double* fit_two = nullptr, double* fit_narrow = nullptr) {
  double f = 0, fp = 0, by = 0, ft = 0, fn = 0;
  for (int k = 0; k < n; ++k) {
    const double a0 = a[k], a1 = a[k + 1], b0 = b[k], b1 = b[k + 1];
    const double f1 = a0 * b0 * 2 * b1 + 2 * a0 * a1 * b1;
    const double f2 = a0 * b0 * 2 * a1 + 2 * b0 * a1 * b1;
    f += 8 * std::min(f1, f2);
    const double A0 = pad16(a[k]), A1 = pad16(a[k + 1]), B0 = pad16(b[k]), B1 = pad16(b[k + 1]);
    fp += 8 * (A0 * B0 * 2 * B1 + 2 * A0 * A1 * B1);
    if (A0 * B0 <= QKF_XCAP_TWO && A1 * B1 <= QKF_XCAP_TWO) ft += 8 * (A0 * B0 * 2 * B1 + 2 * A0 * A1 * B1);
    if (A0 * B0 <= plan_fit && A1 * B1 <= plan_fit) fn += 8 * (A0 * B0 * 2 * B1 + 2 * A0 * A1 * B1);
    by += 16.0 * 2 * (a0 * a1 + b0 * b1);
  }
  if (fit_two) *fit_two = ft;
  if (fit_narrow) *fit_narrow = fn;
  *flops = f;
  *padded = fp;
  *bytes = by + 8;
}
static double fused_cost(int n, const int32_t* a, const int32_t* b) {
  double c = 0;
  for (int k = 0; k < n; ++k) {
    const double A0 = pad16(a[k]) / 16, A1 = pad16(a[k + 1]) / 16, B1 = pad16(b[k + 1]) / 16;
    const double kb = (b[k] + 3) / 4, ka = (a[k] + 3) / 4;
    c += 6 * A0 * B1 * kb + 6 * B1 * A1 * ka;
  }
  return c;
}

static int choose_edge_k(const int n_sites, const int32_t* x_dims, const int32_t* y_dims, const std::vector<int32_t>& pairs) {
  constexpr int KMIN = 4, KMAX = 9;
  if (const char* e = std::getenv("QK_EDGE")) {
    const int v = std::atoi(e);
    if (v <= 0) return 0;
    return (v >= KMIN && v <= KMAX && n_sites >= 2 * v + 2) ? v : 0;
  }
  const int64_t np = (int64_t)pairs.size() / 2;
  if (np == 0 || n_sites < 2 * KMIN + 2) return 0;
  const int stride = n_sites + 1;
  const int64_t step = std::max<int64_t>(1, np / 512);
  const double over = 375.0;
  auto t16 = [](const int v) { return (double)((v + 15) / 16); };
  std::vector<double> total((size_t)KMAX + 1, 0.0);
  std::vector<double> site((size_t)n_sites);
  for (int64_t t = 0; t < np; t += step) {
    const int32_t* a = x_dims + (int64_t)pairs[2 * t] * stride;
    const int32_t* b = y_dims + (int64_t)pairs[2 * t + 1] * stride;
    for (int k = 0; k < n_sites; ++k)
      site[(size_t)k] = 6 * t16(a[k]) * t16(b[k + 1]) * ((b[k] + 3) / 4) + 6 * t16(b[k + 1]) * t16(a[k + 1]) * ((a[k] + 3) / 4) + over;
    double chain = 0;
    for (double v : site) chain += v;
    total[0] += chain;
    double ends = 0;
    for (int k = 1; k <= KMAX && n_sites >= 2 * k + 2; ++k) {
      ends += site[(size_t)k - 1] + site[(size_t)(n_sites - k)];
      if (k < KMIN) continue;
      const double blocks = 2.0 * 3.0 * ((1 << k) / 4) * (t16(a[k]) * t16(b[k]) + t16(a[n_sites - k]) * t16(b[n_sites - k])) + 2 * over;
      total[(size_t)k] += chain - ends + blocks;
    }
  }
  int best = 0;
  for (int k = KMIN; k <= KMAX && n_sites >= 2 * k + 2; ++k)
    if (total[(size_t)k] > 0 && total[(size_t)k] < total[(size_t)best] * 0.995) best = k;
  return best;
}

struct TiledItem {
  int32_t i, j;
  double fp;
};
struct TiledTile {
  int64_t start, count;
  double cost;
};
struct TiledGlobal {
  SiteTab xt, yt_own;
  bool sym = false;
  int n_sites = 0, nx = 0, ny = 0, world = 1;
  const int32_t *x_dims = nullptr, *y_dims = nullptr;
  std::vector<TiledItem> items;
  std::vector<TiledTile> tiles;
  std::vector<int> parent;
  std::vector<std::vector<int>> mine;
  std::vector<int64_t> per_rank;
  int64_t n_items = 0;
  const SiteTab& yt() const { return sym ? xt : yt_own; }
};

static void tiled_global(TiledGlobal& G, const int n_sites, const int nx, const int32_t* x_dims, const int ny, const int32_t* y_dims, const bool sym, const bool orient, const int world,
                         const int T, const int threads) {
  G.sym = sym, G.n_sites = n_sites, G.nx = nx, G.ny = ny, G.world = world, G.x_dims = x_dims, G.y_dims = y_dims;
  SiteTab& xt = G.xt;
  xt.build(nx, n_sites, x_dims);
  if (!sym) G.yt_own.build(ny, n_sites, y_dims);
  const SiteTab& yt = G.yt();
  typedef TiledItem Item;
  typedef TiledTile Tile;
  std::vector<Item>& items = G.items;
  std::vector<Tile>& tiles = G.tiles;
  std::vector<int>& parent = G.parent;
  auto order_of = [&](const int n, const SiteTab& tab) {
    std::vector<int> o((size_t)n);
    std::iota(o.begin(), o.end(), 0);
    std::stable_sort(o.begin(), o.end(), [&](const int u, const int v) { return tab.weight[(size_t)u] > tab.weight[(size_t)v]; });
    return o;
  };
  const std::vector<int> ox = order_of(nx, xt), oy = sym ? ox : order_of(ny, yt);
  int Tx = T, Ty = T;
  if (const char* e = std::getenv("QK_PLAN_TILE_X")) Tx = std::max(1, std::min(128, std::atoi(e)));
  if (const char* e = std::getenv("QK_PLAN_TILE_Y")) Ty = std::max(1, std::min(128, std::atoi(e)));
  const bool orient_tile = orient && std::getenv("QK_PLAN_ORIENT_TILE") && std::atoi(std::getenv("QK_PLAN_ORIENT_TILE")) != 0;
  const int nbx = (nx + Tx - 1) / Tx, nby = (ny + Ty - 1) / Ty;
  std::vector<int32_t> tile_b;
  int64_t n_items = 0;
  for (int bj = 0; bj < nby; ++bj)
    for (int bi = 0; bi < nbx; ++bi) {
      const int u0 = bi * Tx, u1 = std::min(nx, (bi + 1) * Tx), v0 = bj * Ty, v1 = std::min(ny, (bj + 1) * Ty);
      int64_t cnt = 0;
      for (int v = v0; v < v1; ++v) cnt += sym ? std::max(0, std::min(u1, v + 1) - u0) : (u1 - u0);
      if (cnt == 0) continue;
      tiles.push_back(Tile{n_items, cnt, 0.0});
      tile_b.push_back(bi), tile_b.push_back(bj);
      n_items += cnt;
    }
  items.assign((size_t)n_items, Item{0, 0, 0.0});
  G.n_items = n_items;
  par_ranges(threads, (int64_t)tiles.size(), [&](const int64_t t_lo, const int64_t t_hi) {
    for (int64_t t = t_lo; t < t_hi; ++t) {
      const int bi = tile_b[2 * (size_t)t], bj = tile_b[2 * (size_t)t + 1];
      const int64_t q0 = tiles[(size_t)t].start;
      int64_t q = q0;
      double cost = 0, cost_sw = 0, c_keep = 0, c_swap = 0;
      for (int v = bj * Ty; v < std::min(ny, (bj + 1) * Ty); ++v)
        for (int u = bi * Tx; u < std::min(nx, (bi + 1) * Tx); ++u) {
          if (sym && u > v) continue;
          int xi = ox[(size_t)u], yj = oy[(size_t)v];
          if (sym && !orient && xi > yj) std::swap(xi, yj);
          const size_t ex = (size_t)xi * n_sites, ey = (size_t)yj * n_sites;
          const Pass1 r = pair_pass1(n_sites, &xt.T0[ex], &xt.T1[ex], &xt.TK[ex], &xt.P0[ex], &xt.P1[ex], &xt.P01[ex], &yt.T0[ey], &yt.T1[ey], &yt.TK[ey], &yt.P0[ey], &yt.P1[ey], &yt.P01[ey]);
          double fp = r.fp_xy;
          if (orient_tile) c_keep += r.c_xy, c_swap += r.c_yx, cost_sw += r.fp_yx;
          else if (orient && xi != yj && r.c_yx < r.c_xy) std::swap(xi, yj), fp = r.fp_yx;
          items[(size_t)q++] = Item{xi, yj, fp};
          cost += fp;
        }
      if (orient_tile && c_swap < c_keep) {
        for (int64_t e = q0; e < q; ++e) {
          Item& it = items[(size_t)e];
          const size_t ex = (size_t)it.j * n_sites, ey = (size_t)it.i * n_sites;
          const Pass1 r = pair_pass1(n_sites, &xt.T0[ex], &xt.T1[ex], &xt.TK[ex], &xt.P0[ex], &xt.P1[ex], &xt.P01[ex], &yt.T0[ey], &yt.T1[ey], &yt.TK[ey], &yt.P0[ey], &yt.P1[ey], &yt.P01[ey]);
          std::swap(it.i, it.j), it.fp = r.fp_xy;
        }
        cost = cost_sw;
      }
      tiles[(size_t)t].cost = cost;
    }
  });
  std::vector<int> by_cost(tiles.size());
  std::iota(by_cost.begin(), by_cost.end(), 0);
  std::stable_sort(by_cost.begin(), by_cost.end(), [&](const int u, const int v) { return tiles[(size_t)u].cost > tiles[(size_t)v].cost; });
  parent.assign(tiles.size(), 0);
  std::iota(parent.begin(), parent.end(), 0);
  if (world > 1) {
    double total = 0, acc = 0;
    for (const Tile& t : tiles) total += t.cost;
    std::vector<Tile> cut;
    std::vector<int> order, par;
    for (const int t : by_cost) {
      acc += tiles[(size_t)t].cost;
      if (acc <= 0.97 * total || tiles[(size_t)t].count == 1) {
        order.push_back((int)cut.size());
        cut.push_back(tiles[(size_t)t]), par.push_back(t);
      } else {
        std::vector<int64_t> q((size_t)tiles[(size_t)t].count);
        std::iota(q.begin(), q.end(), tiles[(size_t)t].start);
        std::stable_sort(q.begin(), q.end(), [&](const int64_t u, const int64_t v) { return items[(size_t)u].fp > items[(size_t)v].fp; });
        for (const int64_t e : q) {
          order.push_back((int)cut.size());
          cut.push_back(Tile{e, 1, items[(size_t)e].fp}), par.push_back(t);
        }
      }
    }
    tiles.swap(cut), by_cost.swap(order), parent.swap(par);
    std::stable_sort(by_cost.begin(), by_cost.end(), [&](const int u, const int v) { return tiles[(size_t)u].cost > tiles[(size_t)v].cost; });
  }
  std::vector<double> load((size_t)world, 0.0);
  G.per_rank.assign((size_t)world, 0);
  G.mine.assign((size_t)world, std::vector<int>());
  for (const int t : by_cost) {
    const int r = (int)(std::min_element(load.begin(), load.end()) - load.begin());
    load[(size_t)r] += tiles[(size_t)t].cost, G.per_rank[(size_t)r] += tiles[(size_t)t].count;
    G.mine[(size_t)r].push_back(t);
  }
}
// ... 400 lines not shown
```

qml-cutensornet_amd/csrc/qkgram.hip:

```cpp
#include "qk_host.h"
#include "qk_ring.h"
#include "qk_fused.h"
#ifndef QKF_QUAD
#define QKF_QUAD 0
#endif
#if QKF_QUAD
#include "qk_quad.h"
#endif

#include <algorithm>
#include <cmath>
#include <cstdarg>
#include <cstdio>
#include <cstdlib>
#include <cstring>
#include <new>
#include <numeric>
#include <string>
#include <vector>

static thread_local std::string g_err;

int qk_fail(int code, const char* fmt, ...) {
  char buf[512];
  va_list ap;
  va_start(ap, fmt);
  vsnprintf(buf, sizeof buf, fmt, ap);
  va_end(ap);
  g_err = buf;
  return code;
}
#define fail qk_fail

extern "C" const char* qk_last_error(void) { return g_err.c_str(); }

#include <atomic>
uint64_t qk_next_uid() {
  static std::atomic<uint64_t> next{1};
  return next.fetch_add(1);
}

#include <dlfcn.h>
namespace {
struct Roctx {
  int (*push)(const char*) = nullptr;
  int (*pop)() = nullptr;
};
Roctx& roctx() {
  static Roctx r = [] {
    Roctx x;
    const char* e = std::getenv("QK_ROCTX");
    const char* pre = std::getenv("LD_PRELOAD");
    const bool attached = std::getenv("ROCP_TOOL_LIBRARIES") || (pre && std::strstr(pre, "rocprofiler"));
    if (e ? std::atoi(e) == 0 : !attached) return x;
    void* h = nullptr;
    for (const char* name : {"librocprofiler-sdk-roctx.so.1", "librocprofiler-sdk-roctx.so", "libroctx64.so.4", "libroctx64.so"})
      if ((h = dlopen(name, RTLD_NOW | RTLD_GLOBAL))) break;
    if (!h) return x;
    x.push = reinterpret_cast<int (*)(const char*)>(dlsym(h, "roctxRangePushA"));
    x.pop = reinterpret_cast<int (*)()>(dlsym(h, "roctxRangePop"));
    if (!x.push || !x.pop) x.push = nullptr, x.pop = nullptr;
    return x;
  }();
  return r;
}
}
extern "C" int qk_range_push(const char* name) {
  Roctx& r = roctx();
  return (r.push && name) ? r.push(name) : 0;
}
extern "C" int qk_range_pop(void) {
  Roctx& r = roctx();
  return r.pop ? r.pop() : 0;
}

static inline int pad16(int x) { return (x + TILE - 1) / TILE * TILE; }

extern "C" int64_t qk_pack_state_size(int32_t n_sites, const int32_t* bond_dims) {
  int64_t tot = 0;
  for (int k = 0; k < n_sites; ++k) tot += 2ll * pad16(bond_dims[k]) * 2 * pad16(bond_dims[k + 1]);
  return tot;
}

extern "C" int qk_pack_state(int32_t n_sites, const int32_t* bond_dims, const double* const* site_tensors,
                             int32_t layout, double* out, int64_t* site_offsets) {
  if (n_sites <= 0 || !bond_dims || !site_tensors || !out) return fail(QK_EINVAL, "qk_pack_state: null argument");
  if (layout != QK_LAYOUT_LPR && layout != QK_LAYOUT_LRP) return fail(QK_EINVAL, "qk_pack_state: unknown layout %d", layout);
  if (bond_dims[0] != 1 || bond_dims[n_sites] != 1) return fail(QK_EINVAL, "qk_pack_state: boundary bonds must be 1");
  int64_t off = 0;
  for (int k = 0; k < n_sites; ++k) {
    const int cl = bond_dims[k], cr = bond_dims[k + 1];
    if (cl <= 0 || cr <= 0) return fail(QK_EINVAL, "qk_pack_state: non-positive bond at site %d", k);
    const int pl = pad16(cl), pr = pad16(cr);
    const int64_t plane = (int64_t)pl * 2 * pr;
    double* re = out + off;
    double* im = re + plane;
    std::memset(re, 0, sizeof(double) * 2 * plane);
    const double* src = site_tensors[k];
    if (!src) return fail(QK_EINVAL, "qk_pack_state: null tensor at site %d", k);
    for (int l = 0; l < cl; ++l)
      for (int p = 0; p < 2; ++p)
        for (int r = 0; r < cr; ++r) {
          const int64_t s = (layout == QK_LAYOUT_LPR) ? (((int64_t)l * 2 + p) * cr + r) : (((int64_t)l * cr + r) * 2 + p);
          const int64_t d = ((int64_t)l * 2 + p) * pr + r;
          re[d] = src[2 * s];
          im[d] = src[2 * s + 1];
        }
    if (site_offsets) site_offsets[k] = off;
    off += 2 * plane;
  }
  return QK_OK;
}

#ifndef QKF_ONE_NW
#define QKF_ONE_NW 12
#define QKF_ONE_S 2
#define QKF_ONE_WPS 3
#endif
#ifndef QKF_TWO_NW
#define QKF_TWO_NW 8
#define QKF_TWO_S 1
#define QKF_TWO_WPS 4
#endif
#define QKF_KERNEL_ONE qk_sweep_fused_kernel<QKF_ONE_NW, QKF_ONE_S, QKF_XCAP_ONE, QKF_ONE_WPS>
#define QKF_KERNEL_TWO qk_sweep_fused_kernel<QKF_TWO_NW, QKF_TWO_S, QKF_XCAP_TWO, QKF_TWO_WPS>
#ifndef QKF_DUAL_NW
#define QKF_DUAL_NW 12
#define QKF_DUAL_WPS 3
#endif
#define QKF_KERNEL_DUAL qk_sweep_fused_dual_kernel<QKF_DUAL_NW, QKF_XCAP_ONE, QKF_DUAL_WPS>
#define QKF_KERNEL_ONE_DET qk_sweep_fused_kernel<QKF_ONE_NW, QKF_ONE_S, QKF_XCAP_ONE, QKF_ONE_WPS, true>
#define QKF_KERNEL_TWO_DET qk_sweep_fused_kernel<QKF_TWO_NW, QKF_TWO_S, QKF_XCAP_TWO, QKF_TWO_WPS, true>
#define QKF_KERNEL_DUAL_DET qk_sweep_fused_dual_kernel<QKF_DUAL_NW, QKF_XCAP_ONE, QKF_DUAL_WPS, true>
#if QKF_QUAD
#define QKF_QUAD_NW 8
#define QKF_KERNEL_QUAD qk_sweep_fused_quad_kernel<QKF_QUAD_NW, QKF_XCAP_ONE, 2>
#endif

extern "C" int qk_plan_destroy(qk_plan* plan) {
  if (!plan) return QK_OK;
  if (plan->d_pairs) (void)hipFree(plan->d_pairs);
  if (plan->d_groups) (void)hipFree(plan->d_groups);
  delete plan;
  return QK_OK;
}
__global__ void qk_convert_f32_kernel(const double* __restrict__ src, float* __restrict__ dst, const long long n) {
  for (long long e = (long long)blockIdx.x * blockDim.x + threadIdx.x; e < n; e += (long long)gridDim.x * blockDim.x) dst[e] = (float)src[e];
}

__global__ void qk_scatter_kernel(const int32_t* __restrict__ pairs, const double* __restrict__ vals, long long n,
                                  double* __restrict__ K, long long ld, int mirror) {
  const long long t = (long long)blockIdx.x * blockDim.x + threadIdx.x;
  if (t >= n) return;
  const int i = pairs[2 * t], j = pairs[2 * t + 1];
  if (i < 0) return;
  const double v = vals[t];
  K[(long long)j * ld + i] = v;
  if (mirror) K[(long long)i * ld + j] = v;
}

typedef double qk_v2d __attribute__((ext_vector_type(2)));

__device__ __forceinline__ void qk_ctile(QkfTile& t, const qk_v2d* __restrict__ P, const long pk, const long pm, const qk_v2d* __restrict__ Q, const long qk, const long qn, const int ks4,
                                         const int q, const int j) {
  const qk_v2d* pp = P + q * pk + j * pm;
  const qk_v2d* qq = Q + q * qk + j * qn;
  v4d p1 = {0, 0, 0, 0}, p2 = {0, 0, 0, 0}, p3 = {0, 0, 0, 0};
  qk_v2d a = pp[0], b = qq[0];
  for (int ks = 0; ks < ks4; ++ks) {
    const qk_v2d a0 = a, b0 = b;
    if (ks + 1 < ks4) a = pp[(long)4 * (ks + 1) * pk], b = qq[(long)4 * (ks + 1) * qk];
    qkf_kstep<false>(p1, p2, p3, a0.x, a0.y, b0.x, b0.y);
  }
  t.re = p1 - p2, t.im = p3 - p1 - p2;
}

__global__ __launch_bounds__(256) void qk_edge_kernel(const qk_v2d* __restrict__ il, const int32_t* __restrict__ dims, const int32_t* __restrict__ dtrue, const int64_t* __restrict__ offs,
                                                      const int n_sites, const int k, const long long n_states, qk_v2d* __restrict__ edge, const long long* __restrict__ edge_offs,
                                                      qk_v2d* __restrict__ tmp, const long long tmp_elems) {
  qk_v2d* const t0 = tmp + (long long)blockIdx.x * 2 * tmp_elems;
  qk_v2d* const t1 = t0 + tmp_elems;
  const int n1 = n_sites + 1, lane = threadIdx.x & 63, wave = threadIdx.x >> 6, nw = blockDim.x >> 6, j = lane & 15, q = lane >> 4;
  for (long long t = blockIdx.x; t < 2 * n_states; t += gridDim.x) {
    const long long st = t >> 1;
    const int right = (int)(t & 1);
    const int32_t* d = dims + st * n1;
    const int32_t* dt = dtrue + st * n1;
    qk_v2d* const dst = edge + edge_offs[t];
    for (int e = threadIdx.x; e < 256; e += blockDim.x) t0[e] = (qk_v2d){e == 0 ? 1.0 : 0.0, 0.0};
    __syncthreads();
    const qk_v2d* in = t0;
    for (int jj = 0; jj < k; ++jj) {
      const int site = right ? n_sites - 1 - jj : jj;
      const int lp = d[site], rp = d[site + 1];
      const qk_v2d* const A = il + (offs[st * n_sites + site] >> 1);
      const int ld_in = right ? rp : lp, ld_out = right ? lp : rp, rows_in = 1 << jj;
      const int ks4 = ((right ? dt[site + 1] : dt[site]) + 3) >> 2;
      qk_v2d* const out = (jj + 1 == k) ? dst : (in == t0 ? t1 : t0);
      const int nts = (rows_in + 15) >> 4, ntc = ld_out >> 4;
      for (int u = wave; u < nts * 2 * ntc; u += nw) {
        const int tc = u % ntc, pp = (u / ntc) & 1, ts = u / (2 * ntc);
        QkfTile T;
        if (right) qk_ctile(T, in + (long)(ts * 16) * ld_in, 1, ld_in, A + (long)pp * rp + (long)(tc * 16) * 2 * rp, 1, 2 * rp, ks4, q, j);
        else qk_ctile(T, in + (long)(ts * 16) * ld_in, 1, ld_in, A + (long)pp * rp + tc * 16, 2 * rp, 1, ks4, q, j);
#pragma unroll
        for (int r = 0; r < 4; ++r) {
          const int s_ = ts * 16 + q + 4 * r;
          if (s_ < rows_in) out[(long)(2 * s_ + pp) * ld_out + tc * 16 + j] = (qk_v2d){T.re[r], T.im[r]};
        }
      }
      __syncthreads();
      in = out;
    }
  }
}

__global__ __launch_bounds__(256, 2) void qk_merge_kernel(const qk_v2d* __restrict__ il, const int32_t* __restrict__ dims, const int32_t* __restrict__ dtrue, const int64_t* __restrict__ offs,
                                                          const int n_sites, const int k, const int steps, const long long n_tasks, const long long* __restrict__ unit_start,
                                                          qk_v2d* __restrict__ out, const int64_t* __restrict__ out_offs) {
  const int n1 = n_sites + 1, lane = threadIdx.x & 63, wave = threadIdx.x >> 6, nw = blockDim.x >> 6, j = lane & 15, q = lane >> 4;
  const long long n_units = unit_start[n_tasks];
  for (long long u = (long long)blockIdx.x * nw + wave; u < n_units; u += (long long)gridDim.x * nw) {
    long long lo = 0, hi = n_tasks;
    while (hi - lo > 1) {
      const long long mid = (lo + hi) >> 1;
      if (unit_start[mid] <= u) lo = mid;
      else hi = mid;
    }
    const long long t = lo, st = t / steps;
    const int step = (int)(t - st * steps), s_ = k + 2 * step, v = (int)(u - unit_start[t]);
    const int32_t* d = dims + st * n1;
    const int lp = d[s_], mp = d[s_ + 1], rp = d[s_ + 2], ntr = rp >> 4, tl = v / ntr, tr = v - tl * ntr;
    (void)lp;
    const int ks4 = (dtrue[st * n1 + s_ + 1] + 3) >> 2;
    const qk_v2d* const A1 = il + (offs[st * n_sites + s_] >> 1);
    const qk_v2d* const A2 = il + (offs[st * n_sites + s_ + 1] >> 1);
    const qk_v2d* pa = A1 + ((long)(tl * 16 + j) * 2) * mp + q;
    const qk_v2d* pb = A2 + ((long)q * 2) * rp + tr * 16 + j;
    v4d acc[4][3];
#pragma unroll
    for (int c = 0; c < 4; ++c)
#pragma unroll
      for (int e = 0; e < 3; ++e) acc[c][e] = (v4d){0, 0, 0, 0};
    qk_v2d a0 = pa[0], a1 = pa[mp], b0 = pb[0], b1 = pb[rp];
    for (int ks = 0; ks < ks4; ++ks) {
      const qk_v2d x0 = a0, x1 = a1, y0 = b0, y1 = b1;
      if (ks + 1 < ks4) {
        pa += 4, pb += (long)8 * rp;
        a0 = pa[0], a1 = pa[mp], b0 = pb[0], b1 = pb[rp];
      }
      qkf_kstep<false>(acc[0][0], acc[0][1], acc[0][2], x0.x, x0.y, y0.x, y0.y);
      qkf_kstep<false>(acc[1][0], acc[1][1], acc[1][2], x0.x, x0.y, y1.x, y1.y);
      qkf_kstep<false>(acc[2][0], acc[2][1], acc[2][2], x1.x, x1.y, y0.x, y0.y);
      qkf_kstep<false>(acc[3][0], acc[3][1], acc[3][2], x1.x, x1.y, y1.x, y1.y);
    }
    qk_v2d* const dst = out + (out_offs[t] >> 1);
#pragma unroll
    for (int c = 0; c < 4; ++c) {
      const v4d re = acc[c][0] - acc[c][1], im = acc[c][2] - acc[c][0] - acc[c][1];
#pragma unroll
      for (int r = 0; r < 4; ++r) dst[(long)(4 * (tl * 16 + q + 4 * r) + c) * rp + tr * 16 + j] = (qk_v2d){re[r], im[r]};
    }
  }
}

#ifdef QK_LAB
__global__ void qk_lab_fold_kernel(const int64_t* __restrict__ src, int64_t* __restrict__ dst, const long long n, const long long win) {
  for (long long i = blockIdx.x * (long long)blockDim.x + threadIdx.x; i < n; i += (long long)gridDim.x * blockDim.x) dst[i] = (src[i] % win) & ~1ll;
}
#endif
__global__ void qk_selftest_f32_kernel(const float* __restrict__ P, const float* __restrict__ Q, float* __restrict__ C) {
  const int lane = threadIdx.x & 63, j = lane & 15, q = lane >> 4;
  v4f acc = {0, 0, 0, 0};
  for (int ks = 0; ks < 4; ++ks) acc = __builtin_amdgcn_mfma_f32_16x16x4f32(P[(4 * ks + q) * 16 + j], Q[(4 * ks + q) * 16 + j], acc, 0, 0, 0);
  for (int r = 0; r < 4; ++r) C[(4 * q + r) * 16 + j] = acc[r];
}

__global__ void qk_selftest_kernel(const double* __restrict__ P, const double* __restrict__ Q, double* __restrict__ C) {
  const int lane = threadIdx.x & 63, j = lane & 15, q = lane >> 4;
  v4d acc = {0, 0, 0, 0};
  for (int ks = 0; ks < 4; ++ks) acc = __builtin_amdgcn_mfma_f64_16x16x4f64(P[(4 * ks + q) * 16 + j], Q[(4 * ks + q) * 16 + j], acc, 0, 0, 0);
  for (int r = 0; r < 4; ++r) C[(q + 4 * r) * 16 + j] = acc[r];
}

extern "C" int qk_device_count(void) {
  int n = 0;
  if (hipGetDeviceCount(&n) != hipSuccess) return 0;
  return n;
}

static int ctx_init(qk_ctx* c, int device_id, int num_cus);

extern "C" int qk_ctx_create(int device_id, qk_ctx** out) {
  if (!out) return fail(QK_EINVAL, "qk_ctx_create: null out");
  int n = 0;
  hipError_t e = hipGetDeviceCount(&n);
  if (e != hipSuccess || n <= 0)
    return fail(QK_EDEVICE, "qk_ctx_create: no HIP device available (%s); this engine has no CPU fallback",
                e == hipSuccess ? "device count is 0" : hipGetErrorString(e));
  if (device_id < 0 || device_id >= n) return fail(QK_EINVAL, "qk_ctx_create: device %d out of range [0,%d)", device_id, n);
  HIP_TRY(hipSetDevice(device_id));
  hipDeviceProp_t prop;
  HIP_TRY(hipGetDeviceProperties(&prop, device_id));
  if (std::strncmp(prop.gcnArchName, "gfx950", 6) != 0)
    return fail(QK_EDEVICE, "qk_ctx_create: device %d is %s; this library is built for gfx950 only", device_id, prop.gcnArchName);
  qk_ctx* c = new (std::nothrow) qk_ctx;
  if (!c) return fail(QK_ENOMEM, "qk_ctx_create: out of memory");
  const int rc_init = ctx_init(c, device_id, prop.multiProcessorCount);
  if (rc_init != QK_OK) {
    qk_ctx_destroy(c);
    return rc_init;
  }
  *out = c;
  return QK_OK;
}

static int ctx_init(qk_ctx* c, int device_id, int num_cus) {
  c->device = device_id;
  c->num_cus = num_cus;
  HIP_TRY(hipStreamCreateWithFlags(&c->own_stream, hipStreamNonBlocking));
  c->stream = c->own_stream;
  HIP_TRY(hipEventCreate(&c->ev0));
  HIP_TRY(hipEventCreate(&c->ev1));
  HIP_TRY(hipEventCreate(&c->ev_mid));
  HIP_TRY(hipEventCreate(&c->ev_d));
  HIP_TRY(c->counter.alloc((QK_NQ_MAX * QK_QSTRIDE + 8 + 2 * 8 * QK_QSTRIDE) * sizeof(unsigned long long)));
  HIP_TRY(c->prof.alloc(8 * sizeof(unsigned long long)));
  HIP_TRY(hipMemset(c->prof.get(), 0, 8 * sizeof(unsigned long long)));
  for (const void* k : {(const void*)qk_sweep_ring_kernel<float>, (const void*)qk_sweep_ring_kernel<double>, (const void*)qk_sweep_small_kernel<double>, (const void*)qk_sweep_small_kernel<float>})
    HIP_TRY(hipFuncSetAttribute(k, hipFuncAttributeMaxDynamicSharedMemorySize, 80 * 1024));
  for (const void* k : {(const void*)QKF_KERNEL_ONE, (const void*)QKF_KERNEL_DUAL, (const void*)QKF_KERNEL_ONE_DET, (const void*)QKF_KERNEL_DUAL_DET})
    HIP_TRY(hipFuncSetAttribute(k, hipFuncAttributeMaxDynamicSharedMemorySize, 160 * 1024));
  for (const void* k : {(const void*)QKF_KERNEL_TWO, (const void*)QKF_KERNEL_TWO_DET}) HIP_TRY(hipFuncSetAttribute(k, hipFuncAttributeMaxDynamicSharedMemorySize, 160 * 1024 / QKF_TWO_WGS));
#if QKF_QUAD
  HIP_TRY(hipFuncSetAttribute(reinterpret_cast<const void*>(QKF_KERNEL_QUAD), hipFuncAttributeMaxDynamicSharedMemorySize, 160 * 1024));
#endif
  QkSweepPolicy& p = c->policy;
#ifdef QK_LAB
  {
    const int rc = qk_lab_init(c);
    if (rc != QK_OK) return rc;
  }
  if (const char* v = std::getenv("QK_VARIANT")) p.variant = std::atoi(v);
#endif
  if (const char* v = std::getenv("QK_SMALL")) p.small_path = std::atoi(v) != 0;
  if (const char* v = std::getenv("QK_WAVE")) p.wave_path = std::atoi(v) != 0;
  if (const char* v = std::getenv("QK_WAVE2")) p.wave2_path = std::atoi(v) != 0, p.wave2_ring = std::atoi(v) != 2;
  if (const char* v = std::getenv("QK_FUSED")) p.fused_path = std::atoi(v);
  if (const char* v = std::getenv("QK_MERGE")) p.merge_sites = std::atoi(v) != 0;
  if (const char* v = std::getenv("QK_DETERMINISTIC"))
    if (std::atoi(v) != 0) p.deterministic = true;
  if (const char* v = std::getenv("QK_FUSED_SPLIT")) p.fused_split = std::max(0, std::min(2, std::atoi(v)));
  if (const char* v = std::getenv("QK_FUSED_WGS")) p.fused_wgs = std::max(0, std::min(2, std::atoi(v)));
  if (const char* v = std::getenv("QK_WGS_PER_CU")) p.wgs_per_cu = std::max(1, std::min(4, std::atoi(v)));
  return QK_OK;
}

extern "C" int qk_ctx_destroy(qk_ctx* c) {
  if (!c) return QK_OK;
  (void)hipSetDevice(c->device);
  if (c->stream) (void)hipStreamSynchronize(c->stream);
  if (c->ev0) (void)hipEventDestroy(c->ev0);
  if (c->ev1) (void)hipEventDestroy(c->ev1);
  if (c->ev_mid) (void)hipEventDestroy(c->ev_mid);
  if (c->ev_d) (void)hipEventDestroy(c->ev_d);
  if (c->own_stream) (void)hipStreamDestroy(c->own_stream);
  delete c;
  return QK_OK;
}

extern "C" int qk_ctx_trim(qk_ctx* c) {
  if (!c) return fail(QK_EINVAL, "qk_ctx_trim: null context");
  HIP_TRY(hipSetDevice(c->device));
  HIP_TRY(hipStreamSynchronize(c->stream));
  for (QkGrowBuf* b : {&c->scratch, &c->build_arena, &c->build_work, &c->derive_tmp, &c->local_scratch}) b->reset();
  return QK_OK;
}

extern "C" int qk_ctx_set_stream(qk_ctx* c, void* s) {
  if (!c) return fail(QK_EINVAL, "qk_ctx_set_stream: null context");
  c->stream = reinterpret_cast<hipStream_t>(s);
  return QK_OK;
}

extern "C" int qk_ctx_use_own_stream(qk_ctx* c) {
  if (!c) return fail(QK_EINVAL, "qk_ctx_use_own_stream: null context");
  c->stream = c->own_stream;
  return QK_OK;
}

extern "C" int qk_ctx_synchronize(qk_ctx* c) {
  if (!c) return fail(QK_EINVAL, "qk_ctx_synchronize: null context");
  HIP_TRY(hipSetDevice(c->device));
  HIP_TRY(hipStreamSynchronize(c->stream));
  return QK_OK;
}

int qk_mps_set_alloc(qk_ctx* c, int n_states, int n_sites, int64_t data_bytes, int precision, qk_mps_set** out, const char* who) {
  qk_mps_set* m = new (std::nothrow) qk_mps_set;
  if (!m) return fail(QK_ENOMEM, "%s: out of memory", who);
  m->ctx = c, m->n_states = n_states, m->n_sites = n_sites, m->precision = precision, m->bytes = data_bytes;
  const size_t nd = (size_t)n_states * (n_sites + 1), no = (size_t)n_states * n_sites;
  hipError_t e = m->d_data.alloc((size_t)data_bytes);
  if (e == hipSuccess) e = m->d_dims.alloc(nd * sizeof(int32_t));
  if (e == hipSuccess) e = m->d_true.alloc(nd * sizeof(int32_t));
  if (e == hipSuccess) e = m->d_offs.alloc(no * sizeof(int64_t));
  if (e != hipSuccess) {
    qk_mps_set_destroy(m);
    return fail(QK_EDEVICE, "%s: hipMalloc of a set of %lld bytes and its tables failed: %s", who, (long long)data_bytes, hipGetErrorString(e));
  }
  *out = m;
  return QK_OK;
}

extern "C" int qk_mps_set_create(qk_ctx* c, int32_t n_states, int32_t n_sites, const int32_t* bond_dims,
                                 const double* const* site_tensors, int32_t layout, qk_mps_set** out) {
  if (!c || !out || !bond_dims || !site_tensors) return fail(QK_EINVAL, "qk_mps_set_create: null argument");
  if (n_states <= 0 || n_sites <= 0) return fail(QK_EINVAL, "qk_mps_set_create: empty set (%d states, %d sites)", n_states, n_sites);
  QkRangeGuard range_("qk:upload");
  HIP_TRY(hipSetDevice(c->device));
  const int stride = n_sites + 1;
  std::vector<int32_t> pad((size_t)n_states * stride);
  std::vector<int64_t> offs((size_t)n_states * n_sites);
  std::vector<int64_t> state_off(n_states + 1, 0);
  int max_pad = 0;
  for (int s = 0; s < n_states; ++s) {
    const int32_t* d = bond_dims + (size_t)s * stride;
    if (d[0] != 1 || d[n_sites] != 1) return fail(QK_EINVAL, "qk_mps_set_create: state %d: boundary bonds must be 1", s);
    for (int k = 0; k <= n_sites; ++k) {
      if (d[k] <= 0) return fail(QK_EINVAL, "qk_mps_set_create: state %d: non-positive bond %d", s, k);
      pad[(size_t)s * stride + k] = pad16(d[k]);
      max_pad = std::max(max_pad, pad16(d[k]));
    }
    state_off[s + 1] = state_off[s] + qk_pack_state_size(n_sites, d);
  }
  qk_mps_set* m = nullptr;
  int rc = qk_mps_set_alloc(c, n_states, n_sites, state_off[n_states] * (int64_t)sizeof(double), 64, &m, "qk_mps_set_create");
  if (rc != QK_OK) return rc;
  m->max_pad = max_pad;
  m->dims_true.assign(bond_dims, bond_dims + (size_t)n_states * stride);
  hipError_t e = hipSuccess;
  std::vector<double> stage;
  std::vector<int64_t> so(n_sites);
  for (int s = 0; s < n_states; ++s) {
    const int64_t sz = state_off[s + 1] - state_off[s];
    stage.resize((size_t)sz);
    rc = qk_pack_state(n_sites, bond_dims + (size_t)s * stride, site_tensors + (size_t)s * n_sites, layout, stage.data(), so.data());
    if (rc != QK_OK) {
      qk_mps_set_destroy(m);
      return rc;
    }
    for (int k = 0; k < n_sites; ++k) offs[(size_t)s * n_sites + k] = state_off[s] + so[k];
    e = hipMemcpy(m->d_data.get<double>() + state_off[s], stage.data(), (size_t)sz * sizeof(double), hipMemcpyHostToDevice);
    if (e != hipSuccess) {
      qk_mps_set_destroy(m);
      return fail(QK_EDEVICE, "qk_mps_set_create: upload failed: %s", hipGetErrorString(e));
    }
  }
  e = hipMemcpy(m->d_dims.get(), pad.data(), pad.size() * sizeof(int32_t), hipMemcpyHostToDevice);
  if (e == hipSuccess) e = hipMemcpy(m->d_true.get(), bond_dims, pad.size() * sizeof(int32_t), hipMemcpyHostToDevice);
  if (e == hipSuccess) e = hipMemcpy(m->d_offs.get(), offs.data(), offs.size() * sizeof(int64_t), hipMemcpyHostToDevice);
  if (e != hipSuccess) {
    qk_mps_set_destroy(m);
    return fail(QK_EDEVICE, "qk_mps_set_create: table upload failed: %s", hipGetErrorString(e));
  }
  *out = m;
  return QK_OK;
}

extern "C" int qk_mps_set_destroy(qk_mps_set* m) {
  if (!m) return QK_OK;
  (void)hipSetDevice(m->ctx->device);
  (void)hipStreamSynchronize(m->ctx->stream);
  delete m;
  return QK_OK;
}

extern "C" int qk_mps_set_info(const qk_mps_set* m, int32_t* n_states, int32_t* n_sites, int32_t* max_padded_bond, int64_t* device_bytes) {
  if (!m) return fail(QK_EINVAL, "qk_mps_set_info: null set");
  if (n_states) *n_states = m->n_states;
  if (n_sites) *n_sites = m->n_sites;
  if (max_padded_bond) *max_padded_bond = m->max_pad;
  if (device_bytes) *device_bytes = m->bytes * (m->d_il ? 2 : 1) + m->edge_bytes + m->mg_bytes;
  return QK_OK;
}

extern "C" int qk_mps_set_precision(const qk_mps_set* m) { return m ? m->precision : 0; }

extern "C" int qk_mps_set_image(const qk_mps_set* m, int64_t* n_doubles, const double** planes_dev, int32_t* dims_true, int64_t* offsets) {
  if (!m) return fail(QK_EINVAL, "qk_mps_set_image: null set");
  if (m->precision != 64) return fail(QK_EINVAL, "qk_mps_set_image: only fp64 sets are exchanged");
  if (n_doubles) *n_doubles = m->bytes / (int64_t)sizeof(double);
  if (planes_dev) *planes_dev = m->d_data.get<double>();
  if (dims_true) std::memcpy(dims_true, m->dims_true.data(), m->dims_true.size() * sizeof(int32_t));
  if (offsets) {
    HIP_TRY(hipSetDevice(m->ctx->device));
    HIP_TRY(hipStreamSynchronize(m->ctx->stream));
    HIP_TRY(hipMemcpy(offsets, m->d_offs.get<int64_t>(), (size_t)m->n_states * m->n_sites * sizeof(int64_t), hipMemcpyDeviceToHost));
  }
  return QK_OK;
}

extern "C" int qk_mps_set_copy_image(const qk_mps_set* m, double* dst, int64_t n_doubles) {
  if (!m || !dst) return fail(QK_EINVAL, "qk_mps_set_copy_image: null argument");
  if (m->precision != 64) return fail(QK_EINVAL, "qk_mps_set_copy_image: only fp64 sets are exchanged");
  if (n_doubles * (int64_t)sizeof(double) < m->bytes) return fail(QK_EINVAL, "qk_mps_set_copy_image: destination holds %lld doubles, the image has %lld", (long long)n_doubles, (long long)(m->bytes / 8));
  HIP_TRY(hipSetDevice(m->ctx->device));
  HIP_TRY(hipMemcpyAsync(dst, m->d_data.get<double>(), (size_t)m->bytes, hipMemcpyDefault, m->ctx->stream));
  HIP_TRY(hipStreamSynchronize(m->ctx->stream));
  return QK_OK;
}

extern "C" int qk_mps_set_from_packed(qk_ctx* c, int32_t n_states, int32_t n_sites, const int32_t* dims_true, const int64_t* offsets,
                                      const double* planes_dev, int64_t n_doubles, qk_mps_set** out) {
  if (!c || !out || !dims_true || !offsets || !planes_dev) return fail(QK_EINVAL, "qk_mps_set_from_packed: null argument");
  if (n_states <= 0 || n_sites <= 0 || n_doubles <= 0) return fail(QK_EINVAL, "qk_mps_set_from_packed: empty set");
  const int stride = n_sites + 1;
  std::vector<int32_t> pad((size_t)n_states * stride);
  int max_pad = 0;
  for (int s = 0; s < n_states; ++s) {
    const int32_t* d = dims_true + (size_t)s * stride;
    if (d[0] != 1 || d[n_sites] != 1) return fail(QK_EINVAL, "qk_mps_set_from_packed: state %d: boundary bonds must be 1", s);
    for (int k = 0; k <= n_sites; ++k) {
      if (d[k] <= 0) return fail(QK_EINVAL, "qk_mps_set_from_packed: state %d: non-positive bond %d", s, k);
      pad[(size_t)s * stride + k] = pad16(d[k]);
      max_pad = std::max(max_pad, pad16(d[k]));
    }
    for (int k = 0; k < n_sites; ++k) {
      const int64_t off = offsets[(size_t)s * n_sites + k], sz = 2ll * pad[(size_t)s * stride + k] * 2 * pad[(size_t)s * stride + k + 1];
      if (off < 0 || (off & 1) || off + sz > n_doubles) return fail(QK_EINVAL, "qk_mps_set_from_packed: state %d site %d: tensor [%lld, %lld) outside the %lld-double image", s, k, (long long)off, (long long)(off + sz), (long long)n_doubles);
    }
  }
  HIP_TRY(hipSetDevice(c->device));
  qk_mps_set* m = nullptr;
  const int rc = qk_mps_set_alloc(c, n_states, n_sites, n_doubles * (int64_t)sizeof(double), 64, &m, "qk_mps_set_from_packed");
  if (rc != QK_OK) return rc;
  m->max_pad = max_pad;
  m->dims_true.assign(dims_true, dims_true + (size_t)n_states * stride);
  hipError_t e = hipMemcpyAsync(m->d_data.get(), planes_dev, (size_t)m->bytes, hipMemcpyDefault, c->stream);
  if (e == hipSuccess) e = hipMemcpyAsync(m->d_dims.get(), pad.data(), pad.size() * sizeof(int32_t), hipMemcpyHostToDevice, c->stream);
  if (e == hipSuccess) e = hipMemcpyAsync(m->d_true.get(), dims_true, pad.size() * sizeof(int32_t), hipMemcpyHostToDevice, c->stream);
  if (e == hipSuccess) e = hipMemcpyAsync(m->d_offs.get(), offsets, (size_t)n_states * n_sites * sizeof(int64_t), hipMemcpyHostToDevice, c->stream);
  if (e == hipSuccess) e = hipStreamSynchronize(c->stream);
  if (e != hipSuccess) {
    qk_mps_set_destroy(m);
    return fail(QK_EDEVICE, "qk_mps_set_from_packed: %s", hipGetErrorString(e));
  }
  *out = m;
  return QK_OK;
}

extern "C" int qk_mps_set_to_f32(qk_ctx* c, const qk_mps_set* src, qk_mps_set** out) {
  if (!c || !src || !out) return fail(QK_EINVAL, "qk_mps_set_to_f32: null argument");
  if (src->ctx != c) return fail(QK_EINVAL, "qk_mps_set_to_f32: the set belongs to another context");
  if (src->precision != 64) return fail(QK_EINVAL, "qk_mps_set_to_f32: the source set is not fp64");
  HIP_TRY(hipSetDevice(c->device));
  const long long n = src->bytes / (long long)sizeof(double);
  qk_mps_set* m = nullptr;
  const int rc = qk_mps_set_alloc(c, src->n_states, src->n_sites, n * (long long)sizeof(float), 32, &m, "qk_mps_set_to_f32");
  if (rc != QK_OK) return rc;
  m->max_pad = src->max_pad;
  m->dims_true = src->dims_true;
  const size_t nd = (size_t)src->n_states * (src->n_sites + 1), no = (size_t)src->n_states * src->n_sites;
  hipError_t e = hipMemcpyAsync(m->d_dims.get(), src->d_dims.get(), nd * sizeof(int32_t), hipMemcpyDeviceToDevice, c->stream);
  if (e == hipSuccess) e = hipMemcpyAsync(m->d_true.get(), src->d_true.get(), nd * sizeof(int32_t), hipMemcpyDeviceToDevice, c->stream);
  if (e == hipSuccess) e = hipMemcpyAsync(m->d_offs.get(), src->d_offs.get(), no * sizeof(int64_t), hipMemcpyDeviceToDevice, c->stream);
  if (e == hipSuccess) {
    qk_convert_f32_kernel<<<dim3(4 * c->num_cus), dim3(256), 0, c->stream>>>(src->d_data.get<double>(), m->d_data.get<float>(), n);
    e = hipGetLastError();
  }
  if (e == hipSuccess) e = hipStreamSynchronize(c->stream);
  if (e != hipSuccess) {
    qk_mps_set_destroy(m);
    return fail(QK_EDEVICE, "qk_mps_set_to_f32: %s", hipGetErrorString(e));
  }
  *out = m;
  return QK_OK;
}

static int ensure_interleaved(qk_ctx* c, qk_mps_set* m) {
  if (m->d_il) return QK_OK;
  QkDevBuf il;
  HIP_TRY(il.alloc((size_t)m->bytes));
  const long long nt = (long long)m->n_states * m->n_sites;
  const dim3 grid((unsigned)std::min<long long>(nt, 64ll * c->num_cus));
  if (m->precision == 64) qk_interleave_kernel<double><<<grid, dim3(256), 0, c->stream>>>(m->d_data.get<double>(), il.get<double>(), m->d_dims.get<int32_t>(), m->d_offs.get<int64_t>(), m->n_sites, nt);
  else
    qk_interleave_kernel<float><<<grid, dim3(256), 0, c->stream>>>(m->d_data.get<float>(), il.get<float>(), m->d_dims.get<int32_t>(), m->d_offs.get<int64_t>(), m->n_sites, nt);
  HIP_TRY(hipGetLastError());
  m->d_il = std::move(il);
  return QK_OK;
}

static int ensure_edges(qk_ctx* c, qk_mps_set* m, const int k) {
  if (k <= 0 || (m->d_edge && m->edge_k == k)) return QK_OK;
  if (m->d_edge || m->d_edge_offs) HIP_TRY(hipStreamSynchronize(c->stream));
  m->d_edge.reset(), m->d_edge_offs.reset(), m->edge_k = 0, m->edge_bytes = 0;
  const int n = m->n_sites, stride = n + 1;
  std::vector<long long>& offs = m->h_edge_offs;
  offs.assign((size_t)m->n_states * 2, 0);
  long long total = 0;
  int maxld = 16;
  for (int s_ = 0; s_ < m->n_states; ++s_) {
    const int32_t* d = m->dims_true.data() + (size_t)s_ * stride;
    offs[(size_t)2 * s_] = total;
    total += (long long)(1 << k) * pad16(d[k]);
    offs[(size_t)2 * s_ + 1] = total;
    total += (long long)(1 << k) * pad16(d[n - k]);
    for (int jj = 0; jj <= k; ++jj) maxld = std::max(maxld, std::max(pad16(d[jj]), pad16(d[n - jj])));
  }
  const long long tmp_elems = (long long)std::max(1 << (k - 1), 16) * maxld;
  const int grid = (int)std::min<long long>(2ll * m->n_states, 4ll * c->num_cus);
  const size_t tmp_bytes = (size_t)grid * 2 * tmp_elems * 2 * sizeof(double);
  if (tmp_bytes > c->derive_tmp.bytes) HIP_TRY(hipStreamSynchronize(c->stream));
  HIP_TRY(c->derive_tmp.ensure(tmp_bytes));
  QkDevBuf eb, ob;
  HIP_TRY(eb.alloc((size_t)total * 2 * sizeof(double)));
  HIP_TRY(ob.alloc(offs.size() * sizeof(long long)));
  HIP_TRY(hipMemcpyAsync(ob.get(), offs.data(), offs.size() * sizeof(long long), hipMemcpyHostToDevice, c->stream));
  qk_edge_kernel<<<dim3(grid), dim3(256), 0, c->stream>>>(m->d_il.get<qk_v2d>(), m->d_dims.get<int32_t>(), m->d_true.get<int32_t>(), m->d_offs.get<int64_t>(), n, k, m->n_states, eb.get<qk_v2d>(),
                                                          ob.get<long long>(), c->derive_tmp.get<qk_v2d>(), tmp_elems);
  HIP_TRY(hipGetLastError());
  m->d_edge = std::move(eb), m->d_edge_offs = std::move(ob);
  m->edge_k = k, m->edge_bytes = total * 2 * (long long)sizeof(double);
  return QK_OK;
}

static void free_merged(qk_mps_set* m) {
  m->d_mg.reset(), m->d_mg_offs.reset(), m->d_mg_units.reset(), m->mg_k = -1, m->mg_steps = 0, m->mg_bytes = 0;
}

static int ensure_merged(qk_ctx* c, qk_mps_set* m, const int k) {
  if (m->d_mg && m->mg_k == k) return QK_OK;
  if (m->d_mg) HIP_TRY(hipStreamSynchronize(c->stream));
  free_merged(m);
  const int n = m->n_sites, stride = n + 1, steps = (n - 2 * k) / 2;
  if (steps < 1) return fail(QK_EINVAL, "ensure_merged: a chain of %d sites", n - 2 * k);
  std::vector<int64_t>& mo = m->h_mg_offs;
  std::vector<long long>& us = m->h_mg_units;
  mo.assign((size_t)m->n_states * steps, 0);
  us.assign((size_t)m->n_states * steps + 1, 0);
  long long total = 0, units = 0;
  for (int s_ = 0; s_ < m->n_states; ++s_) {
    const int32_t* d = m->dims_true.data() + (size_t)s_ * stride;
    for (int t = 0; t < steps; ++t) {
      const long long lp = pad16(d[k + 2 * t]), rp = pad16(d[k + 2 * t + 2]);
      mo[(size_t)s_ * steps + t] = 2 * total;
      us[(size_t)s_ * steps + t] = units;
      total += 4ll * lp * rp;
      units += (lp / 16) * (rp / 16);
    }
  }
  us.back() = units;
  QkDevBuf ib, ob, ub;
  HIP_TRY(ib.alloc((size_t)total * 2 * sizeof(double)));
  HIP_TRY(ob.alloc(mo.size() * sizeof(int64_t)));
  HIP_TRY(ub.alloc(us.size() * sizeof(long long)));
  HIP_TRY(hipMemcpyAsync(ob.get(), mo.data(), mo.size() * sizeof(int64_t), hipMemcpyHostToDevice, c->stream));
  HIP_TRY(hipMemcpyAsync(ub.get(), us.data(), us.size() * sizeof(long long), hipMemcpyHostToDevice, c->stream));
  const long long tasks = (long long)m->n_states * steps;
  const unsigned grid = (unsigned)std::min<long long>((units + 3) / 4, 4ll * c->num_cus);
  qk_merge_kernel<<<dim3(grid), dim3(256), 0, c->stream>>>(m->d_il.get<qk_v2d>(), m->d_dims.get<int32_t>(), m->d_true.get<int32_t>(), m->d_offs.get<int64_t>(), n, k, steps, tasks, ub.get<long long>(),
                                                          ib.get<qk_v2d>(), ob.get<int64_t>());
  HIP_TRY(hipGetLastError());
  m->d_mg = std::move(ib), m->d_mg_offs = std::move(ob), m->d_mg_units = std::move(ub);
  m->mg_k = k, m->mg_steps = steps, m->mg_bytes = total * 2 * (long long)sizeof(double);
  return QK_OK;
}

static int ensure_plan_uploaded(qk_ctx* c, qk_plan* p) {
  if (p->d_pairs && p->up_ctx == c) return QK_OK;
  if (p->d_pairs) (void)hipFree(p->d_pairs);
  if (p->d_groups) (void)hipFree(p->d_groups);
  p->d_pairs = nullptr, p->d_groups = nullptr, p->up_ctx = nullptr;
  if (p->pairs.empty()) return QK_OK;
  QkDevBuf pairs, groups;
  HIP_TRY(pairs.alloc(p->pairs.size() * sizeof(int32_t)));
  HIP_TRY(hipMemcpy(pairs.get(), p->pairs.data(), p->pairs.size() * sizeof(int32_t), hipMemcpyHostToDevice));
  HIP_TRY(groups.alloc(p->groups.size() * sizeof(int32_t)));
  HIP_TRY(hipMemcpy(groups.get(), p->groups.data(), p->groups.size() * sizeof(int32_t), hipMemcpyHostToDevice));
  p->d_pairs = static_cast<int32_t*>(pairs.release()), p->d_groups = static_cast<int32_t*>(groups.release()), p->up_ctx = c;
  return QK_OK;
}

static int derive_fused_images(qk_ctx* c, const qk_mps_set* xs, const qk_mps_set* ys, const qk_plan* plan, const bool merge_sites, SweepArgs& a) {
  int ek = plan->edge_k, rc = QK_OK;
  if (ek > 0) {
    if (xs->edge_k > 0 && (ys == xs || ys->edge_k == 0 || ys->edge_k == xs->edge_k)) ek = xs->edge_k;
    else if (xs->edge_k == 0 && ys->edge_k > 0) ek = ys->edge_k;
    for (const qk_mps_set* m : {xs, ys})
      if ((rc = ensure_edges(c, const_cast<qk_mps_set*>(m), ek)) != QK_OK) return rc;
    a.xedge = xs->d_edge.get<double>(), a.xedge_offs = xs->d_edge_offs.get<long long>(), a.yedge = ys->d_edge.get<double>(), a.yedge_offs = ys->d_edge_offs.get<long long>(), a.edge_k = ek;
  }
  if (merge_sites && xs->n_sites - 2 * ek >= 2) {
    for (const qk_mps_set* m : {xs, ys})
      if ((rc = ensure_merged(c, const_cast<qk_mps_set*>(m), ek)) != QK_OK) return rc;
    a.xmg = xs->d_mg.get<double>(), a.xmg_offs = xs->d_mg_offs.get<int64_t>(), a.ymg = ys->d_mg.get<double>(), a.ymg_offs = ys->d_mg_offs.get<int64_t>(), a.merge_steps = xs->mg_steps;
  }
#ifdef QK_LAB
  if (const char* v = std::getenv("QK_DEBUG_ALIAS")) {
    const long long win = std::atoll(v);
    if (win > 0) {
      auto fold = [&](const int64_t* src, const long long n) -> const int64_t* {
        QkDevBuf buf;
        if (buf.alloc((size_t)n * sizeof(int64_t)) != hipSuccess) return src;
        int64_t* dst = static_cast<int64_t*>(buf.release());
        qk_lab_fold_kernel<<<dim3(256), dim3(256), 0, c->stream>>>(src, dst, n, win);
        return dst;
      };
      a.xoffs = fold(a.xoffs, (long long)xs->n_states * xs->n_sites), a.yoffs = fold(a.yoffs, (long long)ys->n_states * ys->n_sites);
      if (a.merge_steps > 0)
        a.xmg_offs = fold(a.xmg_offs, (long long)xs->n_states * xs->mg_steps), a.ymg_offs = fold(a.ymg_offs, (long long)ys->n_states * ys->mg_steps);
    }
  }
#endif
  return QK_OK;
}

static int launch_sweep(const int kernel, const bool f32, const long long grid_, const size_t lds, const hipStream_t s, const SweepArgs& a) {
  const dim3 grid((unsigned)grid_);
  switch (kernel) {
    case QK_KERNEL_WAVE: qk_sweep_wave_kernel<0><<<grid, dim3(64), lds, s>>>(a); break;
    case QK_KERNEL_WAVE2: if (f32) qk_sweep_wave2_kernel<3, float><<<grid, dim3(64), lds, s>>>(a); else qk_sweep_wave2_kernel<3, double><<<grid, dim3(64), lds, s>>>(a); break;
    case QK_KERNEL_WAVE2_PLAIN: qk_sweep_wave2_kernel<0, double><<<grid, dim3(64), lds, s>>>(a); break;
    case QK_KERNEL_SMALL: if (f32) qk_sweep_small_kernel<float><<<grid, dim3(512), lds, s>>>(a); else qk_sweep_small_kernel<double><<<grid, dim3(512), lds, s>>>(a); break;
    case QK_KERNEL_RING: if (f32) qk_sweep_ring_kernel<float><<<grid, dim3(512), lds, s>>>(a); else qk_sweep_ring_kernel<double><<<grid, dim3(512), lds, s>>>(a); break;
    case QK_KERNEL_FUSED1: QKF_KERNEL_ONE<<<grid, dim3(64 * QKF_ONE_NW), lds, s>>>(a); break;
    case QK_KERNEL_FUSED1_DET: QKF_KERNEL_ONE_DET<<<grid, dim3(64 * QKF_ONE_NW), lds, s>>>(a); break;
    case QK_KERNEL_FUSED2: QKF_KERNEL_TWO<<<grid, dim3(64 * QKF_TWO_NW), lds, s>>>(a); break;
    case QK_KERNEL_FUSED2_DET: QKF_KERNEL_TWO_DET<<<grid, dim3(64 * QKF_TWO_NW), lds, s>>>(a); break;
#if QKF_QUAD
    case QK_KERNEL_FUSED_DUAL: QKF_KERNEL_QUAD<<<grid, dim3(64 * QKF_QUAD_NW), lds, s>>>(a); break;
#else
    case QK_KERNEL_FUSED_DUAL: QKF_KERNEL_DUAL<<<grid, dim3(64 * QKF_DUAL_NW), lds, s>>>(a); break;
#endif
    case QK_KERNEL_FUSED_DUAL_DET: QKF_KERNEL_DUAL_DET<<<grid, dim3(64 * QKF_DUAL_NW), lds, s>>>(a); break;
    default: return fail(QK_EINVAL, "qk_gram_values: no kernel for this call");
  }
  return QK_OK;
}

extern "C" int qk_gram_values(qk_ctx* c, const qk_mps_set* xs, const qk_mps_set* ys, const qk_plan* plan_c, double* values_dev, double* z_dev) {
  if (!c || !xs || !plan_c || !values_dev) return fail(QK_EINVAL, "qk_gram_values: null argument");
  qk_plan* plan = const_cast<qk_plan*>(plan_c);
  if (!ys) ys = xs;
  if (xs->ctx != c || ys->ctx != c) return fail(QK_EINVAL, "qk_gram_values: sets belong to another context");
  if (xs->n_sites != ys->n_sites || xs->n_sites != plan->n_sites) return fail(QK_EINVAL, "qk_gram_values: site counts differ (%d, %d, plan %d)", xs->n_sites, ys->n_sites, plan->n_sites);
  if (plan->nx != xs->n_states || plan->ny != ys->n_states) return fail(QK_EINVAL, "qk_gram_values: plan is for %dx%d states, sets hold %dx%d", plan->nx, plan->ny, xs->n_states, ys->n_states);
  QkRangeGuard range_("qk:sweep");
  HIP_TRY(hipSetDevice(c->device));
  const long long np = (long long)plan->pairs.size() / 2;
  c->last = plan->stats;
  c->split_pending = c->tail_pending = false;
  c->last.max_bond = std::max(xs->max_pad, ys->max_pad);
  c->last.kernel_ms = 0, c->last.grid = 0, c->last.kernel = QK_KERNEL_NONE, c->last.precision = xs->precision;
  if (np == 0) return QK_OK;
  int rc = ensure_plan_uploaded(c, plan);
  if (rc != QK_OK) return rc;
  if (xs->precision != ys->precision) return fail(QK_EINVAL, "qk_gram_values: the two sets differ in precision (fp%d, fp%d)", xs->precision, ys->precision);
  const bool f32 = (xs->precision == 32);
  if (f32) c->last.bytes *= 0.5;

  QkSweepPolicy pol = c->policy;
  if (const char* v = std::getenv("QK_FUSED_DUAL")) pol.fused_dual = std::atoi(v) != 0;
  if (const char* v = std::getenv("QK_GANG")) pol.gang = std::atoi(v) != 0;
  const QkSweepChoice ch = qk_choose_sweep(pol, *plan, {xs->max_pad, xs->precision, xs->n_sites}, {ys->max_pad, ys->precision, ys->n_sites}, c->num_cus);
  if (ch.rc != QK_OK) return fail(ch.rc, "%s", ch.err);
  c->last.queues = ch.queues, c->last.tail_frac = c->last.second_tail_frac = 0;
  if (ch.scratch_bytes > c->scratch.bytes) HIP_TRY(hipStreamSynchronize(c->stream));
  HIP_TRY(c->scratch.ensure(ch.scratch_bytes));
  SweepArgs a{};
  a.xdata = xs->d_data.get<double>(), a.xdims = xs->d_dims.get<int32_t>(), a.xtrue = xs->d_true.get<int32_t>(), a.xoffs = xs->d_offs.get<int64_t>();
  a.ydata = ys->d_data.get<double>(), a.ydims = ys->d_dims.get<int32_t>(), a.ytrue = ys->d_true.get<int32_t>(), a.yoffs = ys->d_offs.get<int64_t>();
  a.n_sites = xs->n_sites;
  a.pairs = plan->d_pairs, a.npairs = np;
  a.groups = plan->d_groups, a.ngroups = (long long)plan->groups.size() / 2;
  a.values = values_dev, a.z = z_dev;
  a.scratch = c->scratch.get<double>(), a.x_plane = ch.x_plane, a.t_plane = ch.t_plane, a.turn_ints = ch.turn_ints;
  unsigned long long* const counter = c->counter.get<unsigned long long>();
  a.counter = counter, a.prof = c->prof.get<unsigned long long>();
  for (int s_ = 0; s_ <= QK_NQ_MAX; ++s_) a.qstart[s_] = plan->nq > 1 ? plan->qstart[s_] : (s_ == 0 ? 0 : np);
  a.tail = counter + QK_NQ_MAX * QK_QSTRIDE, a.err = a.tail + 7, a.gang = a.tail + 8;
#ifdef QK_LAB
  if (const char* v = std::getenv("QK_DEBUG_FLAGS")) a.debug_flags = std::atoi(v);
  if (const char* v = std::getenv("QK_PRIO")) a.prio_mode = std::atoi(v);
#endif
  HIP_TRY(hipEventRecord(c->ev_d, c->stream));
  HIP_TRY(hipMemsetAsync(counter, 0, (QK_NQ_MAX * QK_QSTRIDE + 8 + 2 * 8 * QK_QSTRIDE) * sizeof(unsigned long long), c->stream));
  HIP_TRY(hipMemsetAsync(a.tail, 0xFF, 4 * sizeof(unsigned long long), c->stream));
  if (ch.interleaved) {
    for (const qk_mps_set* m : {xs, ys})
      if ((rc = ensure_interleaved(c, const_cast<qk_mps_set*>(m))) != QK_OK) return rc;
    a.xdata = xs->d_il.get<double>(), a.ydata = ys->d_il.get<double>();
  }
  if (ch.fused_images && (rc = derive_fused_images(c, xs, ys, plan, pol.merge_sites, a)) != QK_OK) return rc;
  HIP_TRY(hipEventRecord(c->ev0, c->stream));
  for (int i = 0; i < ch.n_runs; ++i) {
    const QkSweepRun& r = ch.run[i];
    SweepArgs ar = a;
    ar.npairs = r.count, ar.nq = r.nq, ar.gang_n = r.gang_n;
    if (i == 1) {
      HIP_TRY(hipEventRecord(c->ev_mid, c->stream));
      ar.pairs = a.pairs + 2 * r.first, ar.values = a.values + r.first, ar.z = a.z ? a.z + 2 * r.first : nullptr;
      ar.counter = counter + 8 * QK_QSTRIDE, ar.tail = a.tail + 2;
      if (plan->nq > 1)
        for (int s_ = 0; s_ <= 8; ++s_) ar.qstart[s_] = plan->qstart[8 + s_] - r.first;
      if (r.gang2) ar.gang = a.gang + 8 * QK_QSTRIDE;
      c->last.second_pairs = plan->second.pairs, c->last.second_flops = plan->second.flops, c->last.second_padded_flops = plan->second.padded_flops;
      c->last.second_bytes = plan->second.bytes, c->last.second_kernel = r.kernel;
      c->split_pending = true;
    }
#ifdef QK_LAB
    if (r.kernel == QK_KERNEL_LAB) rc = plan->quad ? qk_lab_launch_quad(c, ar, (int)r.grid, xs->n_sites, f32) : qk_lab_launch(c, pol.variant, ar, (int)r.grid, xs->n_sites);
    else
#endif
      rc = launch_sweep(r.kernel, f32, r.grid, r.lds, c->stream, ar);
    if (rc != QK_OK) return rc;
  }
  HIP_TRY(hipGetLastError());
  HIP_TRY(hipEventRecord(c->ev1, c->stream));
  c->ev_pending = true;
  c->last.kernel = ch.run[0].kernel, c->last.grid = (int)ch.launched_grid;
  c->tail_pending = ch.tails;
  return QK_OK;
}

extern "C" int qk_gram_values_host(qk_ctx* c, const qk_mps_set* xs, const qk_mps_set* ys, const qk_plan* plan, double* values_host, double* z_host) {
  if (!c || !plan || !values_host) return fail(QK_EINVAL, "qk_gram_values_host: null argument");
  const int64_t np = qk_plan_num_pairs(plan);
  if (np == 0) return QK_OK;
  HIP_TRY(hipSetDevice(c->device));
  QkDevBuf vals, z;
  HIP_TRY(vals.alloc((size_t)np * sizeof(double)));
  if (z_host) HIP_TRY(z.alloc((size_t)np * 2 * sizeof(double)));
  const int rc = qk_gram_values(c, xs, ys, plan, vals.get<double>(), z.get<double>());
  if (rc != QK_OK) return rc;
  HIP_TRY(hipMemcpyAsync(values_host, vals.get(), (size_t)np * sizeof(double), hipMemcpyDeviceToHost, c->stream));
  if (z_host) HIP_TRY(hipMemcpyAsync(z_host, z.get(), (size_t)np * 2 * sizeof(double), hipMemcpyDeviceToHost, c->stream));
  HIP_TRY(hipStreamSynchronize(c->stream));
  return QK_OK;
}

extern "C" int qk_scatter(qk_ctx* c, const int32_t* pairs_dev, const double* values_dev, int64_t n, double* k_dev, int64_t ld, int32_t mirror) {
  if (!c || !pairs_dev || !values_dev || !k_dev) return fail(QK_EINVAL, "qk_scatter: null argument");
  if (n <= 0) return QK_OK;
  QkRangeGuard range_("qk:scatter");
  HIP_TRY(hipSetDevice(c->device));
  const int bs = 256;
  hipLaunchKernelGGL(qk_scatter_kernel, dim3((unsigned)((n + bs - 1) / bs)), dim3(bs), 0, c->stream, pairs_dev, values_dev, (long long)n, k_dev, (long long)ld, (int)mirror);
  HIP_TRY(hipGetLastError());
  return QK_OK;
}

extern "C" const char* qk_kernel_name(int32_t kernel, int32_t precision) {
  const bool f32 = precision == 32;
  switch (kernel) {
    case QK_KERNEL_WAVE: return "qk_sweep_wave_kernel<0>";
    case QK_KERNEL_SMALL: return f32 ? "qk_sweep_small_kernel<float>" : "qk_sweep_small_kernel<double>";
    case QK_KERNEL_FUSED1: return "qk_sweep_fused_kernel<12, 2, 8192, 3, false>";
    case QK_KERNEL_FUSED2: return "qk_sweep_fused_kernel<8, 1, 4608, 4, false>";
    case QK_KERNEL_FUSED1_DET: return "qk_sweep_fused_kernel<12, 2, 8192, 3, true>";
    case QK_KERNEL_FUSED2_DET: return "qk_sweep_fused_kernel<8, 1, 4608, 4, true>";
    case QK_KERNEL_FUSED_DUAL_DET: return "qk_sweep_fused_dual_kernel<12, 8192, 3, true>";
    case QK_KERNEL_RING: return f32 ? "qk_sweep_ring_kernel<float>" : "qk_sweep_ring_kernel<double>";
    case QK_KERNEL_WAVE2: return precision == 32 ? "qk_sweep_wave2_kernel<3, float>" : "qk_sweep_wave2_kernel<3, double>";
    case QK_KERNEL_WAVE2_PLAIN: return "qk_sweep_wave2_kernel<0, double>";
    case QK_KERNEL_FUSED_DUAL: return "qk_sweep_fused_dual_kernel<12, 8192, 3, false>";
    case QK_KERNEL_LAB: return "(lab kernel)";
    default: return "(none)";
  }
}
#ifndef QKF_EXPERIMENT
static_assert(QKF_ONE_NW == 12 && QKF_ONE_S == 2 && QKF_ONE_WPS == 3 && QKF_TWO_NW == 8 && QKF_TWO_S == 1 && QKF_TWO_WPS == 4 && QKF_XCAP_ONE == 8192 && QKF_XCAP_TWO == 4608,
              "qk_kernel_name spells the fused sweep's template arguments");
#endif

extern "C" int qk_get_stats(qk_ctx* c, qk_stats* out) {
  if (!c || !out) return fail(QK_EINVAL, "qk_get_stats: null argument");
  if (c->ev_pending) {
    HIP_TRY(hipSetDevice(c->device));
    HIP_TRY(hipEventSynchronize(c->ev1));
    float ms = 0;
    HIP_TRY(hipEventElapsedTime(&ms, c->ev0, c->ev1));
    c->last.kernel_ms = ms;
    HIP_TRY(hipEventElapsedTime(&ms, c->ev_d, c->ev0));
    c->last.derive_ms = ms;
    if (c->tail_pending) {
      unsigned long long t[8];
      HIP_TRY(hipMemcpy(t, c->counter.get<unsigned long long>() + QK_NQ_MAX * QK_QSTRIDE, sizeof t, hipMemcpyDeviceToHost));
      auto frac = [](const unsigned long long start, const unsigned long long first_exit, const unsigned long long last_exit) {
        return (last_exit > start && first_exit <= last_exit && first_exit >= start) ? (double)(last_exit - first_exit) / (double)(last_exit - start) : 0.0;
      };
      if (t[7] != 0) return fail(QK_EDEVICE, "qk_get_stats: the ordered accumulation of the last sweep ran out of patience (a bug: please report); its results are not valid");
      c->last.tail_frac = frac(t[0], t[1], t[4]);
      if (c->split_pending) c->last.second_tail_frac = frac(t[2], t[3], t[6]);
      c->tail_pending = false;
    }
    if (c->split_pending) {
      HIP_TRY(hipEventElapsedTime(&ms, c->ev_mid, c->ev1));
      c->last.second_ms = ms;
      c->split_pending = false;
    }
    c->ev_pending = false;
#ifdef QKF_PROF
    {
      unsigned long long pf[8];
      HIP_TRY(hipMemcpy(pf, c->prof.get(), sizeof pf, hipMemcpyDeviceToHost));
      HIP_TRY(hipMemset(c->prof.get(), 0, sizeof pf));
      const double tot = pf[7] > 0 ? (double)pf[7] : 1.0;
      fprintf(stderr, "[qkf_prof] pair set-up %.3f  step set-up %.3f  phase1 %.3f  wait1 %.3f  phase2 %.3f  wait2 %.3f  tail %.3f  (of %.3e wave cycles)\n", pf[0] / tot, pf[1] / tot, pf[2] / tot,
              pf[3] / tot, pf[4] / tot, pf[5] / tot, pf[6] / tot, tot);
    }
#endif
  }
  *out = c->last;
  return QK_OK;
}

static int plan_for_sets(const qk_mps_set* xs, const qk_mps_set* ys, qk_plan** plan) {
  const bool sym = (ys == nullptr || ys == xs);
  return qk_plan_create(xs->n_sites, xs->n_states, xs->dims_true.data(), sym ? xs->n_states : ys->n_states,
                        sym ? nullptr : ys->dims_true.data(), sym ? (QK_PLAN_SYMMETRIC | QK_PLAN_ORIENT) : 0u, 1, 0, 0, plan);
}

struct PlanGuard {
  qk_plan* p = nullptr;
  ~PlanGuard() { qk_plan_destroy(p); }
};

extern "C" int qk_gram_host(qk_ctx* c, const qk_mps_set* xs, const qk_mps_set* ys, double* out, int64_t ld) {
  if (!c || !xs || !out) return fail(QK_EINVAL, "qk_gram_host: null argument");
  const bool sym = (ys == nullptr || ys == xs);
  const int nx = xs->n_states, ny = sym ? nx : ys->n_states;
  if (ld < nx) return fail(QK_EINVAL, "qk_gram_host: ld %lld < %d columns", (long long)ld, nx);
  PlanGuard plan;
  int rc = plan_for_sets(xs, ys, &plan.p);
  if (rc != QK_OK) return rc;
  const int64_t np = qk_plan_num_pairs(plan.p);
  QkDevBuf vals, k;
  HIP_TRY(hipSetDevice(c->device));
  HIP_TRY(vals.alloc((size_t)np * sizeof(double)));
  HIP_TRY(k.alloc((size_t)ny * nx * sizeof(double)));
  HIP_TRY(hipMemsetAsync(k.get(), 0, (size_t)ny * nx * sizeof(double), c->stream));
  rc = qk_gram_values(c, xs, ys, plan.p, vals.get<double>(), nullptr);
  if (rc == QK_OK) rc = qk_scatter(c, plan.p->d_pairs, vals.get<double>(), np, k.get<double>(), nx, sym ? 1 : 0);
  if (rc != QK_OK) return rc;
  HIP_TRY(hipMemcpy2DAsync(out, (size_t)ld * sizeof(double), k.get(), (size_t)nx * sizeof(double), (size_t)nx * sizeof(double), (size_t)ny, hipMemcpyDeviceToHost, c->stream));
  HIP_TRY(hipStreamSynchronize(c->stream));
  return QK_OK;
}

extern "C" int qk_overlaps_host(qk_ctx* c, const qk_mps_set* xs, const qk_mps_set* ys, double* out) {
  if (!c || !xs || !out) return fail(QK_EINVAL, "qk_overlaps_host: null argument");
  if (!ys) ys = xs;
  const int nx = xs->n_states, ny = ys->n_states;
  PlanGuard plan;
// ... 69 lines not shown
```

Before: 746,300.

## Choose per-pair site-merge segmentation by dynamic programming with merged images at every offset

Replaces the fixed even-aligned pairwise site merging with a per-pair segmentation mask computed on the device by a dynamic program over an instruction-count cost model. Merged two-site images are now precomputed at every starting offset (stride 1) instead of only even offsets, so the DP can pick merges at either parity. If that doesn't fit in memory, it falls back to stride 2. The aim is fewer or cheaper contraction steps per Gram entry, at the cost of more merged-image memory and an extra segment kernel launch, cached per plan.

```diff
diff --git a/lab/qk_quad.h b/lab/qk_quad.h
--- a/lab/qk_quad.h
+++ b/lab/qk_quad.h
@@ -269,7 +269,7 @@
     __syncthreads();
     if (p < 0) break;
     const int xi = g.pairs[2 * p], yj = g.pairs[2 * p + 1];
-    qkf_step_table<XCAP, NT>(g, xi, yj, rec, m_off, tid, [](const int pmt, const int nt) { return pmt * ((nt + 1) / 2) <= NW; });
+    qkf_step_table<XCAP, NT>(g, xi, yj, p, rec, m_off, tid, QkSegRule{XCAP, NW, true});
     const int ek = g.edge_k, k_hi = ns - ek;
     const bool edges = ek > 0;
     if (!edges)
diff --git a/qml-cutensornet_amd/csrc/qk_device.h b/qml-cutensornet_amd/csrc/qk_device.h
--- a/qml-cutensornet_amd/csrc/qk_device.h
+++ b/qml-cutensornet_amd/csrc/qk_device.h
@@ -40,6 +40,7 @@
   const int64_t* xmg_offs;
   const int64_t* ymg_offs;
   int merge_steps;
+  const unsigned long long* seg;
   int turn_ints;
   unsigned long long* tail;
   unsigned long long* err;
diff --git a/qml-cutensornet_amd/csrc/qk_fused.h b/qml-cutensornet_amd/csrc/qk_fused.h
--- a/qml-cutensornet_amd/csrc/qk_fused.h
+++ b/qml-cutensornet_amd/csrc/qk_fused.h
@@ -434,8 +434,8 @@
 typedef int v4i __attribute__((ext_vector_type(4)));
 typedef __attribute__((address_space(3))) v4i lds_v4i;
 
-template <int XCAP, int NT, bool ITEM_RECIPS = false, typename OneRound>
-__device__ __forceinline__ void qkf_step_table(const SweepArgs& g, const int xi, const int yj, lds_v4i* const rec, long long* const m_off, const int tid, const OneRound one_round) {
+template <int XCAP, int NT, bool ITEM_RECIPS = false>
+__device__ __forceinline__ void qkf_step_table(const SweepArgs& g, const int xi, const int yj, const long long pair, lds_v4i* const rec, long long* const m_off, const int tid, const QkSegRule rule) {
   const int ns = g.n_sites, n1 = ns + 1;
   const int32_t* const xd = g.xdims + (long long)xi * n1;
   const int32_t* const yd = g.ydims + (long long)yj * n1;
@@ -443,9 +443,6 @@
   const int32_t* const yt = g.ytrue + (long long)yj * n1;
   const v2d* const xdata = reinterpret_cast<const v2d*>(g.xdata);
   const v2d* const ydata = reinterpret_cast<const v2d*>(g.ydata);
-  auto is_small = [&](const int a, const int a2, const int b, const int b2, const int pd) __attribute__((always_inline)) {
-    return a * b <= XCAP && a2 * b2 <= XCAP && (one_round(pd * (a / TILE), b2 / TILE) || a * b + a2 * b2 <= XCAP);
-  };
   auto put = [&](const int e, const int a, const int a2, const int b, const int b2, const int ps, const int next, const bool small, const v2d* const A, const v2d* const B)
                  __attribute__((always_inline)) {
     const int mt = a / TILE, nt = b2 / TILE;
@@ -458,28 +455,21 @@
   };
   auto plain = [&](const int e, const int next) __attribute__((always_inline)) {
     const int a = xd[e], a2 = xd[e + 1], b = yd[e], b2 = yd[e + 1];
-    put(e, a, a2, b, b2, 1, next, is_small(a, a2, b, b2, 2), xdata + (g.xoffs[(long long)xi * ns + e] >> 1), ydata + (g.yoffs[(long long)yj * ns + e] >> 1));
-  };
-  if (g.merge_steps == 0) {
+    put(e, a, a2, b, b2, 1, next, qk_seg_small(rule, a, a2, b, b2, 2), xdata + (g.xoffs[(long long)xi * ns + e] >> 1), ydata + (g.yoffs[(long long)yj * ns + e] >> 1));
+  };
+  if (g.seg == nullptr) {
     for (int e = tid; e < ns; e += NT) plain(e, e + 1);
     return;
   }
   const int ek = g.edge_k, k_hi = ns - ek;
-  for (int t = tid; 2 * t < k_hi - ek; t += NT) {
-    const int e = ek + 2 * t;
-    if (e + 1 >= k_hi) {
-      plain(e, e + 1);
-      continue;
-    }
-    const int a = xd[e], am = xd[e + 1], a2 = xd[e + 2], b = yd[e], bm = yd[e + 1], b2 = yd[e + 2];
-    const bool sm = is_small(a, a2, b, b2, 4);
-    const long long work_m = 4ll * a * b2 * (b + a2), work_p = 2ll * a * bm * (b + am) + 2ll * am * b2 * (bm + a2);
-    const bool merged = (sm || (!is_small(a, am, b, bm, 2) && !is_small(am, a2, bm, b2, 2))) && work_m <= work_p;
-    plain(e + 1, e + 2);
-    if (merged)
-      put(e, a, a2, b, b2, 2, e + 2, sm, reinterpret_cast<const v2d*>(g.xmg) + (g.xmg_offs[(long long)xi * g.merge_steps + t] >> 1),
-          reinterpret_cast<const v2d*>(g.ymg) + (g.ymg_offs[(long long)yj * g.merge_steps + t] >> 1));
-    else plain(e, e + 1);
+  const unsigned long long w0 = g.seg[2 * pair], w1 = g.seg[2 * pair + 1];
+  for (int e = ek + tid; e < k_hi; e += NT) {
+    const int i = e - ek;
+    if (qk_seg_bit(w0, w1, i) && e + 1 < k_hi) {
+      const int a = xd[e], a2 = xd[e + 2], b = yd[e], b2 = yd[e + 2];
+      put(e, a, a2, b, b2, 2, e + 2, qk_seg_small(rule, a, a2, b, b2, 4), reinterpret_cast<const v2d*>(g.xmg) + (g.xmg_offs[(long long)xi * g.merge_steps + i] >> 1),
+          reinterpret_cast<const v2d*>(g.ymg) + (g.ymg_offs[(long long)yj * g.merge_steps + i] >> 1));
+    } else plain(e, e + 1);
   }
 }
 
@@ -576,7 +566,7 @@
     __syncthreads();
     if (p < 0) break;
     const int xi = g.pairs[2 * p], yj = g.pairs[2 * p + 1];
-    qkf_step_table<XCAP, NT, true>(g, xi, yj, rec, m_off, tid, [](const int pmt, const int nt) { return pmt * nt <= NW * S; });
+    qkf_step_table<XCAP, NT, true>(g, xi, yj, p, rec, m_off, tid, QkSegRule{XCAP, NW * S, false});
     const int ek = g.edge_k, k_hi = ns - ek;
     const bool edges = ek > 0;
     if (!edges)
@@ -978,7 +968,7 @@
   auto table_of = [&](const long long pp) __attribute__((always_inline)) {
     if (pp < 0) return;
     const int xi_ = g.pairs[2 * pp], yj_ = g.pairs[2 * pp + 1];
-    qkf_step_table<XCAP, NT>(g, xi_, yj_, rec, m_off, tid, [](const int pmt, const int nt) { return pmt * ((nt + 1) / 2) <= NW; });
+    qkf_step_table<XCAP, NT>(g, xi_, yj_, pp, rec, m_off, tid, QkSegRule{XCAP, NW, true});
   };
   table_of(p);
   while (p >= 0) {
diff --git a/qml-cutensornet_amd/csrc/qk_host.h b/qml-cutensornet_amd/csrc/qk_host.h
--- a/qml-cutensornet_amd/csrc/qk_host.h
+++ b/qml-cutensornet_amd/csrc/qk_host.h
@@ -68,7 +68,8 @@
   QkDevBuf d_mg_units;
   std::vector<long long> h_edge_offs, h_mg_units;
   std::vector<int64_t> h_mg_offs;
-  int mg_k = -1, mg_steps = 0;
+  int mg_k = -1, mg_steps = 0, mg_stride = 0;
+  bool mg_full_failed = false;
   int64_t mg_bytes = 0;
 };
 
diff --git a/qml-cutensornet_amd/csrc/qk_plan.h b/qml-cutensornet_amd/csrc/qk_plan.h
--- a/qml-cutensornet_amd/csrc/qk_plan.h
+++ b/qml-cutensornet_amd/csrc/qk_plan.h
@@ -61,6 +61,64 @@
   const int v = u - (half ? left : 0), tp = (v * inv_mt) >> 20;
   const bool second = 2 * tp + 1 < nt;
   return QkEdgeUnit{v - tp * mt, 2 * tp + (half ? 1 : 0), !single && second, u < (halves ? r0 + 2 * left : pairs) && (!half || second)};
+}
+
+static constexpr int QK_STEP_PRICE = 375;
+static constexpr int QK_SEG_BITS = 128;
+struct QkSegRule {
+  int xcap, cap;
+  bool dual;
+};
+struct QkSegMask {
+  unsigned long long w[2];
+};
+QK_HD static inline bool qk_seg_bit(const unsigned long long w0, const unsigned long long w1, const int i) { return i < QK_SEG_BITS && (((i < 64 ? w0 : w1) >> (i & 63)) & 1ull) != 0; }
+QK_HD static inline bool qk_seg_one_round(const QkSegRule& r, const int pmt, const int nt) { return pmt * (r.dual ? (nt + 1) / 2 : nt) <= r.cap; }
+QK_HD static inline bool qk_seg_small(const QkSegRule& r, const int a, const int a2, const int b, const int b2, const int pd) {
+  return a * b <= r.xcap && a2 * b2 <= r.xcap && (qk_seg_one_round(r, pd * (a / QK_TILE), b2 / QK_TILE) || a * b + a2 * b2 <= r.xcap);
+}
+QK_HD static inline long long qk_step_instr(const int pd, const int a, const int a2, const int b, const int b2, const int at, const int bt) {
+  return 3ll * pd * (b2 / QK_TILE) * ((long long)(a / QK_TILE) * ((bt + 3) >> 2) + (long long)(a2 / QK_TILE) * ((at + 3) >> 2));
+}
+QK_HD static inline bool qk_merge_admissible(const QkSegRule& r, const int32_t* const xd, const int32_t* const yd, const int e) {
+  const int a = xd[e], am = xd[e + 1], a2 = xd[e + 2], b = yd[e], bm = yd[e + 1], b2 = yd[e + 2];
+  const long long work_m = 4ll * a * b2 * (b + a2), work_p = 2ll * a * bm * (b + am) + 2ll * am * b2 * (bm + a2);
+  return (qk_seg_small(r, a, a2, b, b2, 4) || (!qk_seg_small(r, a, am, b, bm, 2) && !qk_seg_small(r, am, a2, bm, b2, 2))) && work_m <= work_p;
+}
+QK_HD static inline QkSegMask qk_segment_chain(const int32_t* const xd, const int32_t* const xt, const int32_t* const yd, const int32_t* const yt, const int n_sites, const int ek,
+                                               const QkSegRule& rule, const int parities, const bool greedy, long long* const objective = nullptr, int* const steps = nullptr) {
+  const int m = n_sites - 2 * ek;
+  auto may = [&](const int i) { return i + 1 < m && i < QK_SEG_BITS && ((parities >> (i & 1)) & 1) != 0 && qk_merge_admissible(rule, xd, yd, ek + i); };
+  auto plain_cost = [&](const int i) { return qk_step_instr(2, xd[ek + i], xd[ek + i + 1], yd[ek + i], yd[ek + i + 1], xt[ek + i], yt[ek + i]) + QK_STEP_PRICE; };
+  auto merged_cost = [&](const int i) { return qk_step_instr(4, xd[ek + i], xd[ek + i + 2], yd[ek + i], yd[ek + i + 2], xt[ek + i], yt[ek + i]) + QK_STEP_PRICE; };
+  QkSegMask take{{0ull, 0ull}};
+  if (greedy) {
+    for (int i = 0; i < m && i < QK_SEG_BITS; ++i)
+      if (may(i)) take.w[i >> 6] |= 1ull << (i & 63);
+  } else {
+    long long c1 = 0, c2 = 0;
+    int s1 = 0, s2 = 0;
+    for (int i = m - 1; i >= 0; --i) {
+      long long c = plain_cost(i) + c1;
+      int s = s1 + 1;
+      if (may(i)) {
+        const long long cm = merged_cost(i) + c2;
+        const int sm = s2 + 1;
+        if (cm < c || (cm == c && (sm < s || (sm == s && (i & 1) == 0)))) c = cm, s = sm, take.w[i >> 6] |= 1ull << (i & 63);
+      }
+      c2 = c1, s2 = s1, c1 = c, s1 = s;
+    }
+  }
+  QkSegMask out{{0ull, 0ull}};
+  long long obj = 0;
+  int n_steps = 0;
+  for (int i = 0; i < m; ++n_steps) {
+    if (qk_seg_bit(take.w[0], take.w[1], i)) out.w[i >> 6] |= 1ull << (i & 63), obj += merged_cost(i), i += 2;
+    else obj += plain_cost(i), i += 1;
+  }
+  if (objective) *objective = obj;
+  if (steps) *steps = n_steps;
+  return out;
 }
 
 struct qk_ctx;
@@ -89,6 +147,8 @@
   qk_ctx* up_ctx = nullptr;
   int32_t* d_pairs = nullptr;
   int32_t* d_groups = nullptr;
+  unsigned long long* d_seg = nullptr;
+  unsigned long long seg_key[8] = {0};
 };
 
 struct QkSweepPolicy {
@@ -102,7 +162,7 @@
   int fused_split = 1;
   int fused_wgs = 0;
   bool deterministic = false;
-  bool merge_sites = true;
+  int merge_mode = 2;
   bool fused_dual = true;
   bool gang = false;
 };
diff --git a/qml-cutensornet_amd/csrc/qk_planner.cpp b/qml-cutensornet_amd/csrc/qk_planner.cpp
--- a/qml-cutensornet_amd/csrc/qk_planner.cpp
+++ b/qml-cutensornet_amd/csrc/qk_planner.cpp
@@ -149,7 +149,7 @@
   if (np == 0 || n_sites < 2 * KMIN + 2) return 0;
   const int stride = n_sites + 1;
   const int64_t step = std::max<int64_t>(1, np / 512);
-  const double over = 375.0;
+  const double over = QK_STEP_PRICE;
   auto t16 = [](const int v) { return (double)((v + 15) / 16); };
   std::vector<double> total((size_t)KMAX + 1, 0.0);
   std::vector<double> site((size_t)n_sites);
diff --git a/qml-cutensornet_amd/csrc/qkgram.hip b/qml-cutensornet_amd/csrc/qkgram.hip
--- a/qml-cutensornet_amd/csrc/qkgram.hip
+++ b/qml-cutensornet_amd/csrc/qkgram.hip
@@ -141,6 +141,7 @@
   if (!plan) return QK_OK;
   if (plan->d_pairs) (void)hipFree(plan->d_pairs);
   if (plan->d_groups) (void)hipFree(plan->d_groups);
+  if (plan->d_seg) (void)hipFree(plan->d_seg);
   delete plan;
   return QK_OK;
 }
@@ -216,7 +217,7 @@
 }
 
 __global__ __launch_bounds__(256, 2) void qk_merge_kernel(const qk_v2d* __restrict__ il, const int32_t* __restrict__ dims, const int32_t* __restrict__ dtrue, const int64_t* __restrict__ offs,
-                                                          const int n_sites, const int k, const int steps, const long long n_tasks, const long long* __restrict__ unit_start,
+                                                          const int n_sites, const int k, const int steps, const int stride, const int n_starts, const long long n_tasks, const long long* __restrict__ unit_start,
                                                           qk_v2d* __restrict__ out, const int64_t* __restrict__ out_offs) {
   const int n1 = n_sites + 1, lane = threadIdx.x & 63, wave = threadIdx.x >> 6, nw = blockDim.x >> 6, j = lane & 15, q = lane >> 4;
   const long long n_units = unit_start[n_tasks];
@@ -228,7 +229,7 @@
       else hi = mid;
     }
     const long long t = lo, st = t / steps;
-    const int step = (int)(t - st * steps), s_ = k + 2 * step, v = (int)(u - unit_start[t]);
+    const int step = (int)(t - st * steps), s_ = k + stride * step, v = (int)(u - unit_start[t]);
     const int32_t* d = dims + st * n1;
     const int lp = d[s_], mp = d[s_ + 1], rp = d[s_ + 2], ntr = rp >> 4, tl = v / ntr, tr = v - tl * ntr;
     (void)lp;
@@ -254,7 +255,7 @@
       qkf_kstep<false>(acc[2][0], acc[2][1], acc[2][2], x1.x, x1.y, y0.x, y0.y);
       qkf_kstep<false>(acc[3][0], acc[3][1], acc[3][2], x1.x, x1.y, y1.x, y1.y);
     }
-    qk_v2d* const dst = out + (out_offs[t] >> 1);
+    qk_v2d* const dst = out + (out_offs[st * n_starts + stride * step] >> 1);
 #pragma unroll
     for (int c = 0; c < 4; ++c) {
       const v4d re = acc[c][0] - acc[c][1], im = acc[c][2] - acc[c][0] - acc[c][1];
@@ -262,6 +263,16 @@
       for (int r = 0; r < 4; ++r) dst[(long)(4 * (tl * 16 + q + 4 * r) + c) * rp + tr * 16 + j] = (qk_v2d){re[r], im[r]};
     }
   }
+}
+
+__global__ __launch_bounds__(256) void qk_segment_kernel(const int32_t* __restrict__ xdims, const int32_t* __restrict__ xtrue, const int32_t* __restrict__ ydims, const int32_t* __restrict__ ytrue,
+                                                         const int n_sites, const int ek, const int32_t* __restrict__ pairs, const long long npairs, const QkSegRule rule, const int parities,
+                                                         const bool greedy, unsigned long long* __restrict__ seg) {
+  const long long p = (long long)blockIdx.x * blockDim.x + threadIdx.x;
+  if (p >= npairs) return;
+  const long long xo = (long long)pairs[2 * p] * (n_sites + 1), yo = (long long)pairs[2 * p + 1] * (n_sites + 1);
+  const QkSegMask m = qk_segment_chain(xdims + xo, xtrue + xo, ydims + yo, ytrue + yo, n_sites, ek, rule, parities, greedy);
+  seg[2 * p] = m.w[0], seg[2 * p + 1] = m.w[1];
 }
 
 #ifdef QK_LAB
@@ -347,7 +358,7 @@
   if (const char* v = std::getenv("QK_WAVE")) p.wave_path = std::atoi(v) != 0;
   if (const char* v = std::getenv("QK_WAVE2")) p.wave2_path = std::atoi(v) != 0, p.wave2_ring = std::atoi(v) != 2;
   if (const char* v = std::getenv("QK_FUSED")) p.fused_path = std::atoi(v);
-  if (const char* v = std::getenv("QK_MERGE")) p.merge_sites = std::atoi(v) != 0;
+  if (const char* v = std::getenv("QK_MERGE")) p.merge_mode = std::max(0, std::min(2, std::atoi(v)));
   if (const char* v = std::getenv("QK_DETERMINISTIC"))
     if (std::atoi(v) != 0) p.deterministic = true;
   if (const char* v = std::getenv("QK_FUSED_SPLIT")) p.fused_split = std::max(0, std::min(2, std::atoi(v)));
@@ -627,44 +638,53 @@
 }
 
 static void free_merged(qk_mps_set* m) {
-  m->d_mg.reset(), m->d_mg_offs.reset(), m->d_mg_units.reset(), m->mg_k = -1, m->mg_steps = 0, m->mg_bytes = 0;
-}
-
-static int ensure_merged(qk_ctx* c, qk_mps_set* m, const int k) {
-  if (m->d_mg && m->mg_k == k) return QK_OK;
+  m->d_mg.reset(), m->d_mg_offs.reset(), m->d_mg_units.reset(), m->mg_k = -1, m->mg_steps = 0, m->mg_stride = 0, m->mg_bytes = 0;
+}
+
+static int ensure_merged(qk_ctx* c, qk_mps_set* m, const int k, int stride) {
+  if (m->mg_full_failed) stride = 2;
+  if (m->d_mg && m->mg_k == k && m->mg_stride <= stride) return QK_OK;
   if (m->d_mg) HIP_TRY(hipStreamSynchronize(c->stream));
   free_merged(m);
-  const int n = m->n_sites, stride = n + 1, steps = (n - 2 * k) / 2;
-  if (steps < 1) return fail(QK_EINVAL, "ensure_merged: a chain of %d sites", n - 2 * k);
+  const int n = m->n_sites, n1 = n + 1, starts = n - 2 * k - 1;
+  if (starts < 1) return fail(QK_EINVAL, "ensure_merged: a chain of %d sites", n - 2 * k);
   std::vector<int64_t>& mo = m->h_mg_offs;
   std::vector<long long>& us = m->h_mg_units;
-  mo.assign((size_t)m->n_states * steps, 0);
-  us.assign((size_t)m->n_states * steps + 1, 0);
+  QkDevBuf ib, ob, ub;
+  int steps = 0;
   long long total = 0, units = 0;
-  for (int s_ = 0; s_ < m->n_states; ++s_) {
-    const int32_t* d = m->dims_true.data() + (size_t)s_ * stride;
-    for (int t = 0; t < steps; ++t) {
-      const long long lp = pad16(d[k + 2 * t]), rp = pad16(d[k + 2 * t + 2]);
-      mo[(size_t)s_ * steps + t] = 2 * total;
-      us[(size_t)s_ * steps + t] = units;
-      total += 4ll * lp * rp;
-      units += (lp / 16) * (rp / 16);
-    }
-  }
-  us.back() = units;
-  QkDevBuf ib, ob, ub;
-  HIP_TRY(ib.alloc((size_t)total * 2 * sizeof(double)));
+  for (;; stride = 2) {
+    steps = (starts + stride - 1) / stride;
+    mo.assign((size_t)m->n_states * starts, 0);
+    us.assign((size_t)m->n_states * steps + 1, 0);
+    total = units = 0;
+    for (int s_ = 0; s_ < m->n_states; ++s_) {
+      const int32_t* d = m->dims_true.data() + (size_t)s_ * n1;
+      for (int t = 0; t < steps; ++t) {
+        const long long lp = pad16(d[k + stride * t]), rp = pad16(d[k + stride * t + 2]);
+        mo[(size_t)s_ * starts + stride * t] = 2 * total;
+        us[(size_t)s_ * steps + t] = units;
+        total += 4ll * lp * rp;
+        units += (lp / 16) * (rp / 16);
+      }
+    }
+    us.back() = units;
+    if (ib.alloc((size_t)total * 2 * sizeof(double)) == hipSuccess) break;
+    (void)hipGetLastError();
+    if (stride == 2) return fail(QK_EDEVICE, "ensure_merged: no device memory for %lld bytes of merged steps", total * 2 * (long long)sizeof(double));
+    m->mg_full_failed = true;
+  }
   HIP_TRY(ob.alloc(mo.size() * sizeof(int64_t)));
   HIP_TRY(ub.alloc(us.size() * sizeof(long long)));
   HIP_TRY(hipMemcpyAsync(ob.get(), mo.data(), mo.size() * sizeof(int64_t), hipMemcpyHostToDevice, c->stream));
   HIP_TRY(hipMemcpyAsync(ub.get(), us.data(), us.size() * sizeof(long long), hipMemcpyHostToDevice, c->stream));
   const long long tasks = (long long)m->n_states * steps;
   const unsigned grid = (unsigned)std::min<long long>((units + 3) / 4, 4ll * c->num_cus);
-  qk_merge_kernel<<<dim3(grid), dim3(256), 0, c->stream>>>(m->d_il.get<qk_v2d>(), m->d_dims.get<int32_t>(), m->d_true.get<int32_t>(), m->d_offs.get<int64_t>(), n, k, steps, tasks, ub.get<long long>(),
-                                                          ib.get<qk_v2d>(), ob.get<int64_t>());
+  qk_merge_kernel<<<dim3(grid), dim3(256), 0, c->stream>>>(m->d_il.get<qk_v2d>(), m->d_dims.get<int32_t>(), m->d_true.get<int32_t>(), m->d_offs.get<int64_t>(), n, k, steps, stride, starts, tasks,
+                                                          ub.get<long long>(), ib.get<qk_v2d>(), ob.get<int64_t>());
   HIP_TRY(hipGetLastError());
   m->d_mg = std::move(ib), m->d_mg_offs = std::move(ob), m->d_mg_units = std::move(ub);
-  m->mg_k = k, m->mg_steps = steps, m->mg_bytes = total * 2 * (long long)sizeof(double);
+  m->mg_k = k, m->mg_steps = starts, m->mg_stride = stride, m->mg_bytes = total * 2 * (long long)sizeof(double);
   return QK_OK;
 }
 
@@ -672,7 +692,8 @@
   if (p->d_pairs && p->up_ctx == c) return QK_OK;
   if (p->d_pairs) (void)hipFree(p->d_pairs);
   if (p->d_groups) (void)hipFree(p->d_groups);
-  p->d_pairs = nullptr, p->d_groups = nullptr, p->up_ctx = nullptr;
+  if (p->d_seg) (void)hipFree(p->d_seg);
+  p->d_pairs = nullptr, p->d_groups = nullptr, p->d_seg = nullptr, p->up_ctx = nullptr;
   if (p->pairs.empty()) return QK_OK;
   QkDevBuf pairs, groups;
   HIP_TRY(pairs.alloc(p->pairs.size() * sizeof(int32_t)));
@@ -683,7 +704,7 @@
   return QK_OK;
 }
 
-static int derive_fused_images(qk_ctx* c, const qk_mps_set* xs, const qk_mps_set* ys, const qk_plan* plan, const bool merge_sites, SweepArgs& a) {
+static int derive_fused_images(qk_ctx* c, const qk_mps_set* xs, const qk_mps_set* ys, const qk_plan* plan, const int merge_mode, SweepArgs& a) {
   int ek = plan->edge_k, rc = QK_OK;
   if (ek > 0) {
     if (xs->edge_k > 0 && (ys == xs || ys->edge_k == 0 || ys->edge_k == xs->edge_k)) ek = xs->edge_k;
@@ -692,9 +713,9 @@
       if ((rc = ensure_edges(c, const_cast<qk_mps_set*>(m), ek)) != QK_OK) return rc;
     a.xedge = xs->d_edge.get<double>(), a.xedge_offs = xs->d_edge_offs.get<long long>(), a.yedge = ys->d_edge.get<double>(), a.yedge_offs = ys->d_edge_offs.get<long long>(), a.edge_k = ek;
   }
-  if (merge_sites && xs->n_sites - 2 * ek >= 2) {
+  if (merge_mode > 0 && xs->n_sites - 2 * ek >= 2) {
     for (const qk_mps_set* m : {xs, ys})
-      if ((rc = ensure_merged(c, const_cast<qk_mps_set*>(m), ek)) != QK_OK) return rc;
+      if ((rc = ensure_merged(c, const_cast<qk_mps_set*>(m), ek, merge_mode >= 2 ? 1 : 2)) != QK_OK) return rc;
     a.xmg = xs->d_mg.get<double>(), a.xmg_offs = xs->d_mg_offs.get<int64_t>(), a.ymg = ys->d_mg.get<double>(), a.ymg_offs = ys->d_mg_offs.get<int64_t>(), a.merge_steps = xs->mg_steps;
   }
 #ifdef QK_LAB
@@ -714,6 +735,57 @@
     }
   }
 #endif
+  return QK_OK;
+}
+
+static QkSegRule seg_rule_of(const int kernel) {
+  switch (kernel) {
+    case QK_KERNEL_FUSED1: case QK_KERNEL_FUSED1_DET: return {QKF_XCAP_ONE, QKF_ONE_NW * QKF_ONE_S, false};
+    case QK_KERNEL_FUSED2: case QK_KERNEL_FUSED2_DET: return {QKF_XCAP_TWO, QKF_TWO_NW * QKF_TWO_S, false};
+#if QKF_QUAD
+    case QK_KERNEL_FUSED_DUAL: return {QKF_XCAP_ONE, QKF_QUAD_NW, true};
+#else
+    case QK_KERNEL_FUSED_DUAL: return {QKF_XCAP_ONE, QKF_DUAL_NW, true};
+#endif
+    case QK_KERNEL_FUSED_DUAL_DET: return {QKF_XCAP_ONE, QKF_DUAL_NW, true};
+    default: return {0, 0, false};
+  }
+}
+
+static int ensure_segments(qk_ctx* c, const qk_mps_set* xs, const qk_mps_set* ys, qk_plan* plan, const QkSweepChoice& ch, const int merge_mode, SweepArgs& a) {
+  const long long np = (long long)plan->pairs.size() / 2;
+  const bool both = merge_mode >= 2 && xs->mg_stride == 1 && ys->mg_stride == 1;
+  const unsigned long long key[8] = {1ull,
+                                     xs->uid,
+                                     ys->uid,
+                                     (unsigned long long)a.edge_k,
+                                     both ? 3ull : 1ull,
+                                     merge_mode == 1 ? 1ull : 0ull,
+                                     (unsigned long long)ch.run[0].kernel | ((unsigned long long)(ch.n_runs > 1 ? ch.run[1].kernel : 0) << 32),
+                                     (unsigned long long)ch.run[0].count};
+  if (plan->d_seg && std::equal(key, key + 8, plan->seg_key)) return a.seg = plan->d_seg, QK_OK;
+  if (plan->d_seg) {
+    HIP_TRY(hipStreamSynchronize(c->stream));
+    (void)hipFree(plan->d_seg), plan->d_seg = nullptr;
+  }
+  QkDevBuf seg;
+  HIP_TRY(seg.alloc((size_t)np * 2 * sizeof(unsigned long long)));
+  unsigned long long* const d = seg.get<unsigned long long>();
+  for (int i = 0; i < ch.n_runs; ++i) {
+    const QkSweepRun& r = ch.run[i];
+    const QkSegRule rule = seg_rule_of(r.kernel);
+    if (r.count <= 0) continue;
+    if (rule.cap == 0) {
+      HIP_TRY(hipMemsetAsync(d + 2 * r.first, 0, (size_t)r.count * 2 * sizeof(unsigned long long), c->stream));
+      continue;
+    }
+    qk_segment_kernel<<<dim3((unsigned)((r.count + 255) / 256)), dim3(256), 0, c->stream>>>(a.xdims, a.xtrue, a.ydims, a.ytrue, a.n_sites, a.edge_k, a.pairs + 2 * r.first, r.count, rule, both ? 3 : 1,
+                                                                                            merge_mode == 1, d + 2 * r.first);
+  }
+  HIP_TRY(hipGetLastError());
+  plan->d_seg = static_cast<unsigned long long*>(seg.release());
+  std::copy(key, key + 8, plan->seg_key);
+  a.seg = plan->d_seg;
   return QK_OK;
 }
 
@@ -793,7 +865,8 @@
       if ((rc = ensure_interleaved(c, const_cast<qk_mps_set*>(m))) != QK_OK) return rc;
     a.xdata = xs->d_il.get<double>(), a.ydata = ys->d_il.get<double>();
   }
-  if (ch.fused_images && (rc = derive_fused_images(c, xs, ys, plan, pol.merge_sites, a)) != QK_OK) return rc;
+  if (ch.fused_images && (rc = derive_fused_images(c, xs, ys, plan, pol.merge_mode, a)) != QK_OK) return rc;
+  if (a.merge_steps > 0 && (rc = ensure_segments(c, xs, ys, plan, ch, pol.merge_mode, a)) != QK_OK) return rc;
   HIP_TRY(hipEventRecord(c->ev0, c->stream));
   for (int i = 0; i < ch.n_runs; ++i) {
     const QkSweepRun& r = ch.run[i];
@@ -801,7 +874,7 @@
     ar.npairs = r.count, ar.nq = r.nq, ar.gang_n = r.gang_n;
     if (i == 1) {
       HIP_TRY(hipEventRecord(c->ev_mid, c->stream));
-      ar.pairs = a.pairs + 2 * r.first, ar.values = a.values + r.first, ar.z = a.z ? a.z + 2 * r.first : nullptr;
+      ar.pairs = a.pairs + 2 * r.first, ar.values = a.values + r.first, ar.z = a.z ? a.z + 2 * r.first : nullptr, ar.seg = a.seg ? a.seg + 2 * r.first : nullptr;
       ar.counter = counter + 8 * QK_QSTRIDE, ar.tail = a.tail + 2;
       if (plan->nq > 1)
         for (int s_ = 0; s_ <= 8; ++s_) ar.qstart[s_] = plan->qstart[8 + s_] - r.first;
```

New measurement: 762,700, median of 6. +2.2%, better.
